# zgchen33/MCGaze

Measured on AMD Instinct MI355X. Metric: clips/sec (7x3x224x224), higher is better.
Workload: dtype f16x3; 1 GPU; full multiclue_gaze_r50 forward (R-50 + FPN + 4 decoder stages + gaze head), 64 clips/GPU x 7 frames x 3x224x224, 64 clips/step; clips_per_gpu=64, clip_length=7, global_clips=64, chunk_frames=0, parallelism=single GPU, trunk_streams=2

## Files before the change

### include/mcgaze_hip.h

```cpp
#ifndef MCGAZE_HIP_H
#define MCGAZE_HIP_H

#include <stddef.h>
#include <stdint.h>

#ifdef __cplusplus
extern "C" {
#endif

#define MCG_ABI_VERSION 14

enum { MCG_OK = 0, MCG_ERR_ARG = 1, MCG_ERR_HIP = 2, MCG_ERR_UNSUPPORTED = 3, MCG_ERR_WORKSPACE = 4 };
typedef enum { MCG_F32 = 0, MCG_BF16 = 1, MCG_F16X3 = 2, MCG_F16 = 3 } mcg_dtype;
#define MCG_ELEM_BYTES(dt) (((dt) == MCG_BF16 || (dt) == MCG_F16) ? 2 : 4)
typedef void* mcg_stream;

int mcg_abi_version(void);
const char* mcg_build_id(void);
const char* mcg_last_error(void);
int mcg_device_info(int* cu_count, size_t* hbm_bytes, char* arch, int arch_len);

int mcg_nchw_to_nhwc(mcg_stream s, mcg_dtype dt, const float* src, void* dst, int N, int C, int H, int W);
int mcg_nhwc_to_nchw(mcg_stream s, mcg_dtype dt, const void* src, float* dst, int N, int C, int H, int W);

enum { MCG_RES_NONE = 0, MCG_RES_ADD = 1, MCG_RES_UPSAMPLE_ADD = 2 };
enum {
  MCG_FLAG_STAGED_GEMM = 1,
  MCG_FLAG_NO_SPECIALISED = 2,
  MCG_FLAG_NO_ATTN_BLOCK = 4
};
typedef struct {
  const void* x;
  const void* w;
  const float* bias;
  const void* residual;
  void* y;
  int N, H, W, Cin, Cout, KH, KW, stride, pad;
  int relu;
  int residual_mode;
  int Hr, Wr;
  const void* x2;
  int Cin2, stride2, H2, W2;
  int tile;
  int flags;
  float wscale;
} mcg_conv_desc;
int mcg_conv2d(mcg_stream s, mcg_dtype dt, const mcg_conv_desc* d);

int mcg_bottleneck_x3(mcg_stream s, const float* x, const float* src2, const void* wstream, const float* bias, float* y, float* z,
                      int frames, int H, int W, int cm, int nsrc, int cn, void* trace);

size_t mcg_conv3x3_wino_x3_weight_bytes(int Cin, int Cout, int g);
int mcg_conv3x3_wino_x3(mcg_stream s, const float* x, const void* u, const float* bias, float* y, int frames, int H, int W,
                        int Cin, int Cout, int relu, int tile, float wscale, int g);

size_t mcg_stem_workspace_bytes(mcg_dtype dt, int N, int H, int W);
int mcg_stem_forward(mcg_stream s, mcg_dtype dt, const float* img, const void* w_stem, const float* bias,
                     void* y, int N, int H, int W, void* ws, size_t ws_bytes, int flags);

int mcg_roi_align(mcg_stream s, mcg_dtype dt, const void* const feats[4], const int feat_h[4], const int feat_w[4],
                  const int strides[4], int C, const float* boxes, int num_boxes, int boxes_per_frame,
                  void* out, int32_t* levels_out);
int mcg_roi_align_indexed(mcg_stream s, mcg_dtype dt, const void* const feats[4], const int feat_h[4], const int feat_w[4],
                          const int strides[4], int C, const float* boxes, int num_boxes, int boxes_per_frame,
                          const int32_t* frame_of, int pyramid_frames, void* out, int32_t* levels_out);

enum {
  MCG_SW_IN_PROJ_W = 0, MCG_SW_IN_PROJ_B, MCG_SW_OUT_PROJ_W, MCG_SW_OUT_PROJ_B, MCG_SW_ATTN_LN_G, MCG_SW_ATTN_LN_B,
  MCG_SW_DYN_W,
  MCG_SW_DYN_B,
  MCG_SW_NORM_IN_G, MCG_SW_NORM_IN_B, MCG_SW_NORM_OUT_G, MCG_SW_NORM_OUT_B,
  MCG_SW_FC_W, MCG_SW_FC_B, MCG_SW_FC_LN_G, MCG_SW_FC_LN_B, MCG_SW_IIC_LN_G, MCG_SW_IIC_LN_B,
  MCG_SW_FFN1_W, MCG_SW_FFN1_B, MCG_SW_FFN2_W, MCG_SW_FFN2_B, MCG_SW_FFN_LN_G, MCG_SW_FFN_LN_B,
  MCG_SW_CLS_FC_W, MCG_SW_CLS_LN_G, MCG_SW_CLS_LN_B,
  MCG_SW_REG_FC_W,
  MCG_SW_REG_LN_G,
  MCG_SW_REG_LN_B,
  MCG_SW_HEAD_CLS_W,
  MCG_SW_HEAD_CLS_B,
  MCG_SW_HEAD_REG_W,
  MCG_SW_HEAD_REG_B,
  MCG_SW_OUT_PROJ_WF, MCG_SW_CLS_FC_WF,
  MCG_SW_REG_FC_WF,
  MCG_SW_IN_PROJ_WF,
  MCG_SW_DYN_WF,
  MCG_SW_COUNT
};
enum {
  MCG_GW_FC_W = 0,
  MCG_GW_LN_G,
  MCG_GW_LN_B,
  MCG_GW_OUT_W,
  MCG_GW_OUT_B,
  MCG_GW_FUSE_W,
  MCG_GW_FUSE_B,
  MCG_GW_COUNT
};

size_t mcg_stage_workspace_bytes(mcg_dtype dt, int num_frames);
int mcg_stage_forward(mcg_stream s, mcg_dtype dt, const void* const weights[MCG_SW_COUNT], const void* roi_feat,
                      const void* obj_in, const float* boxes_in, int num_frames, int clip_length,
                      void* obj_out, float* boxes_out, float* cls_out, const float bbox_stds[4],
                      void* ws, size_t ws_bytes, int flags);

size_t mcg_gaze_head_workspace_bytes(mcg_dtype dt, int num_frames);
int mcg_gaze_head(mcg_stream s, mcg_dtype dt, const void* const weights[MCG_GW_COUNT], const void* obj,
                  int num_frames, float* gaze_out, void* ws, size_t ws_bytes);

typedef struct {
  const void* w;
  const float* bias;
  int cin, cout, k, stride, pad;
  const void* wf;
  float wscale;
  const void* wf4;
} mcg_conv_weights;

typedef struct {
  const void* wstream;
  const float* bias;
  int conv2_index;
  int cm, c, cn;
  int nsrc;
} mcg_fused_block;

typedef struct {
  int blocks[4];
  mcg_conv_weights stem;
  const mcg_conv_weights* convs;
  int num_convs;
  mcg_conv_weights lateral[4];
  mcg_conv_weights fpn_out[4];
  mcg_conv_weights c3_ds[4];
  const float* init_boxes;
  const void* init_feats;
  int num_stages;
  const void* const* stage_weights;
  const void* const* gaze_weights;
  float bbox_stds[4];
  const mcg_fused_block* fused;
  int num_fused;
} mcg_model_weights;

typedef struct mcg_engine mcg_engine;
int mcg_engine_create(mcg_engine** out, const mcg_model_weights* w, mcg_dtype dt);
void mcg_engine_destroy(mcg_engine* e);
int mcg_engine_set_option(mcg_engine* e, const char* name, int value);
int mcg_engine_range_audit(mcg_engine* e, unsigned long long* counts, const char** names, int capacity, int* n_out);
size_t mcg_engine_workspace_bytes(const mcg_engine* e, int num_frames, int H, int W, int chunk_frames);
int mcg_backbone_fpn_forward(mcg_engine* e, mcg_stream s, const float* img, int num_frames, int H, int W,
                             int chunk_frames, void* const pyramid[4], void* ws, size_t ws_bytes);
size_t mcg_trunk_workspace_bytes(const mcg_engine* e, int num_frames, int H, int W, int chunk_frames);
size_t mcg_decoder_workspace_bytes(const mcg_engine* e, int num_frames);
int mcg_decoder_forward(mcg_engine* e, mcg_stream s, const void* const pyramid[4], int num_frames, int clip_length, int H, int W,
                        const int* img_hw, float* gaze_out, float* boxes_out, float* scores_out, void* ws, size_t ws_bytes);
int mcg_decoder_forward_indexed(mcg_engine* e, mcg_stream s, const void* const pyramid[4], int pyramid_frames, const int32_t* frame_of,
                                int num_frames, int clip_length, int H, int W, const int* img_hw, float* gaze_out, float* boxes_out,
                                float* scores_out, void* ws, size_t ws_bytes);
int mcg_clip_forward(mcg_engine* e, mcg_stream s, const float* img, int num_frames, int clip_length, int H, int W,
                     const int* img_hw, int chunk_frames, float* gaze_out, float* boxes_out, float* scores_out,
                     void* ws, size_t ws_bytes);

typedef struct mcg_frame_desc {
  const void* src;
  int src_h, src_w, src_pitch;
  int crop_y, crop_x, crop_h, crop_w;
  int out_h, out_w;
} mcg_frame_desc;
int mcg_preprocess_frames(mcg_stream stream, const mcg_frame_desc* frames_dev, int num_frames, float* dst, int pad_h, int pad_w,
                          const float mean[3], const float stdinv[3], int to_rgb);

int mcg_engine_profile_start(mcg_engine* e, int capacity);
int mcg_engine_profile_stop(mcg_engine* e, int* count, float* ms, double* flops, double* algo_bytes, int* cfg, int* shape_mnk, int capacity);
int mcg_bench_backbone_forward(mcg_engine* e, mcg_stream s, const float* img, int num_frames, int H, int W, void* ws, size_t ws_bytes);
int mcg_bench_backbone_levels(const mcg_engine* e, void* ws, int num_frames, int H, int W, void* levels[4]);

#ifdef __cplusplus
}
#endif
#endif
```

### mcgaze_amd/csrc/check_resources.py

```python
#!/usr/bin/env python3
import re
import sys

RULES = {
    'wino_x3w_kernel': dict(scratch=0, vgpr_spill=0, unit='engine'),
}


def parse(path):
    kernels, cur = [], None
    for line in open(path, errors='replace'):
        m = re.search(r'remark: (?:\s*)Function Name: (\S+)', line)
        if m:
            cur = dict(name=m.group(1))
            kernels.append(cur)
            continue
        m = re.search(r'remark:\s+([A-Za-z \[\]/]+): (\S+) \[-Rpass-analysis', line)
        if m and cur is not None:
            cur[m.group(1).strip()] = m.group(2)
    return kernels


def main():
    path = sys.argv[1]
    kernels = parse(path)
    other = [l.rstrip() for l in open(path, errors='replace') if 'Rpass-analysis=kernel-resource-usage' not in l and not re.match(r'\s+\d* *\|', l) and l.strip()
             and not l.startswith('In file included from') and not re.match(r'\d+ (warning|remark)s? generated', l.strip())]
    for l in other:
        print(l, file=sys.stderr)
    bad = []
    import os
    unit = os.path.basename(path).split('.')[0]
    for prefix, lim in RULES.items():
        if lim.get('unit') == unit and not any(prefix in k['name'] and 'VGPRs Spill' in k and 'ScratchSize [bytes/lane]' in k for k in kernels):
            bad.append(f'{prefix}: no resource remarks found in {path} (expected -Rpass-analysis=kernel-resource-usage output for it)')
    for k in kernels:
        for prefix, lim in RULES.items():
            if prefix in k['name']:
                scratch = int(k.get('ScratchSize [bytes/lane]', '0'))
                spill = int(k.get('VGPRs Spill', '0'))
                if scratch > lim['scratch'] or spill > lim['vgpr_spill']:
                    bad.append(f"{k['name']}: scratch {scratch} B/lane, {spill} spilled VGPRs (limits {lim['scratch']}, {lim['vgpr_spill']})")
    if '--table' in sys.argv:
        print('| kernel | VGPRs | AGPRs | SGPRs | scratch B/lane | VGPR spill | waves/SIMD |\n|---|---|---|---|---|---|---|')
        for k in kernels:
            print(f"| `{k['name']}` | {k.get('VGPRs')} | {k.get('AGPRs')} | {k.get('TotalSGPRs')} | {k.get('ScratchSize [bytes/lane]')} | {k.get('VGPRs Spill')} | {k.get('Occupancy [waves/SIMD]')} |")
    if bad:
        print('check_resources: kernels with hand-issued loads must not spill:\n  ' + '\n  '.join(bad), file=sys.stderr)
        return 1
    return 0


if __name__ == '__main__':
    sys.exit(main())
```

### mcgaze_amd/csrc/engine.hip

```cpp
#include "igemm.hpp"
#include "pw_pair.hpp"
#include "pw_single.hpp"
#include "bneck_x3.hpp"
#include "pw_single_x3.hpp"
#include "wino_x3.hpp"

#include <stdlib.h>
#include <string.h>

#include <map>
#include <mutex>
#include <string>
#include <vector>

int launch_roi_align(hipStream_t s, mcg_dtype dt, const void* const feats[4], const int feat_h[4], const int feat_w[4],
                     const int strides[4], int C, const float* boxes, int num_boxes, int boxes_per_frame, const int32_t* frame_of,
                     int pyramid_frames, void* out, int32_t* levels_out);
int launch_init_queries(hipStream_t s, mcg_dtype dt, const float* init_boxes, const void* init_feats, const int* img_hw,
                        const int32_t* frame_of, int pyramid_frames, int H, int W, float* boxes, void* obj, int N);

struct mcg_engine {
  mcg_dtype dt;
  int blocks[4];
  mcg_conv_weights stem;
  std::vector<mcg_conv_weights> convs;
  mcg_conv_weights lateral[4], fpn_out[4], c3_ds[4];
  std::vector<mcg_fused_block> fused;
  bool bneck_fused = true;
  bool bneck_blocked = true;
  int winograd = 1;
  int wino_tile = -1;
  static constexpr int kAuditCap = 256;
  unsigned long long* audit_dev = nullptr;
  std::vector<std::string> audit_names;
  const float* init_boxes;
  const void* init_feats;
  int num_stages;
  std::vector<const void*> stage_w;
  const void* gaze_w[MCG_GW_COUNT];
  float stds[4];
  static constexpr int kMaxSplit = 4, kCandidates = 8;
  struct StreamPool* pool = nullptr;
  hipStream_t* cand = nullptr;
  hipEvent_t ev_fork = nullptr, ev_join[kMaxSplit - 1] = {};
  McgCtx ctx;
  Prof prof;
  int trunk_streams = 2;
  int max_range_frames = 0;
  bool pw_single = true;
  bool pw_pair = true;
  std::mutex mu;
};
struct StreamPool {
  hipStream_t cand[mcg_engine::kCandidates] = {};
  hipEvent_t ev_probe[3] = {};
  std::map<hipStream_t, std::vector<int>> side_of;
  std::mutex mu;
  bool ok = false;
};
static StreamPool* stream_pool_for_current_device() {
  static std::mutex g_mu;
  static std::map<int, StreamPool*> g_pools;
  int dev = 0;
  if (hipGetDevice(&dev) != hipSuccess) return nullptr;
  std::lock_guard<std::mutex> lock(g_mu);
  auto it = g_pools.find(dev);
  if (it != g_pools.end()) return it->second;
  StreamPool* p = new StreamPool();
  bool ok = true;
  for (int i = 0; i < mcg_engine::kCandidates; ++i) ok = ok && hipStreamCreateWithFlags(&p->cand[i], hipStreamNonBlocking) == hipSuccess;
  for (int i = 0; i < 3; ++i) ok = ok && hipEventCreate(&p->ev_probe[i]) == hipSuccess;
  p->ok = ok;
  g_pools[dev] = p;
  return p;
}
__global__ void probe_spin_kernel(long long ticks) {
  const long long t0 = wall_clock64();
  while (wall_clock64() - t0 < ticks) {}
}
static const std::vector<int>& side_streams_for(mcg_engine* e, hipStream_t s) {
  StreamPool* p = e->pool;
  std::lock_guard<std::mutex> lock(p->mu);
  auto it = p->side_of.find(s);
  if (it != p->side_of.end()) return it->second;
  std::vector<int> good, rest;
  const long long ticks = 15000;
  for (int c = 0; c < mcg_engine::kCandidates; ++c) {
    bool concurrent = false;
    if (hipEventRecord(p->ev_probe[0], s) == hipSuccess) {
      hipLaunchKernelGGL(probe_spin_kernel, dim3(1), dim3(64), 0, s, ticks);
      hipLaunchKernelGGL(probe_spin_kernel, dim3(1), dim3(64), 0, p->cand[c], ticks);
      float ms = 0.f;
      if (hipEventRecord(p->ev_probe[1], s) == hipSuccess && hipEventRecord(p->ev_probe[2], p->cand[c]) == hipSuccess &&
          hipEventSynchronize(p->ev_probe[1]) == hipSuccess && hipEventSynchronize(p->ev_probe[2]) == hipSuccess &&
          hipEventElapsedTime(&ms, p->ev_probe[0], p->ev_probe[2]) == hipSuccess)
        concurrent = ms < 0.15f * 1.6f;
    }
    (concurrent ? good : rest).push_back(c);
  }
  (void)hipGetLastError();
  good.insert(good.end(), rest.begin(), rest.end());
  return p->side_of.emplace(s, good).first->second;
}
static int range_frame_cap(const mcg_engine* e, int H, int W) {
  const long long per_frame = (long long)(H / 4) * (W / 4) * 256 * (mcg_is16(e->dt) ? 2 : 4);
  long long cap = 0x7FFFFF00ll / (per_frame > 0 ? per_frame : 1);
  if (e->max_range_frames > 0 && e->max_range_frames < cap) cap = e->max_range_frames;
  return cap < 1 ? 1 : (cap > 0x7fffffff ? 0x7fffffff : (int)cap);
}
static const int kMinFramesPerRange = 56;
static int trunk_ranges(const mcg_engine* e, int frames) {
  int k = e->trunk_streams;
  if (k > mcg_engine::kMaxSplit) k = mcg_engine::kMaxSplit;
  while (k > 1 && frames / k < kMinFramesPerRange) --k;
  return k < 1 ? 1 : k;
}

static inline size_t al256(size_t b) { return (b + 255) / 256 * 256; }
static inline size_t esize(mcg_dtype dt) { return mcg_is16(dt) ? 2 : 4; }

extern "C" void mcg_engine_destroy(mcg_engine* e);
extern "C" int mcg_engine_create(mcg_engine** out, const mcg_model_weights* w, mcg_dtype dt) {
  MCG_CHECK_ARG(out && w, "mcg_engine_create: null pointer");
  MCG_CHECK_ARG(dt == MCG_F32 || dt == MCG_BF16 || dt == MCG_F16X3 || dt == MCG_F16, "mcg_engine_create: unknown dtype %d", (int)dt);
  int expect = 0;
  for (int l = 0; l < 4; ++l) {
    MCG_CHECK_ARG(w->blocks[l] > 0, "mcg_engine_create: blocks[%d]=%d", l, w->blocks[l]);
    expect += 3 * w->blocks[l] + 1;
  }
  MCG_CHECK_ARG(w->num_convs == expect && w->convs, "mcg_engine_create: expected %d bottleneck convs, got %d", expect, w->num_convs);
  MCG_CHECK_ARG(w->num_stages > 0 && w->stage_weights && w->gaze_weights && w->init_boxes && w->init_feats, "mcg_engine_create: decoder tables missing");
  for (int i = 0; i < w->num_convs; ++i)
    MCG_CHECK_ARG(w->convs[i].w && w->convs[i].bias, "mcg_engine_create: conv %d has a null pointer", i);
  mcg_engine* e = new mcg_engine();
  e->dt = dt;
  memcpy(e->blocks, w->blocks, sizeof(e->blocks));
  e->stem = w->stem;
  e->convs.assign(w->convs, w->convs + w->num_convs);
  memcpy(e->lateral, w->lateral, sizeof(e->lateral));
  memcpy(e->fpn_out, w->fpn_out, sizeof(e->fpn_out));
  memcpy(e->c3_ds, w->c3_ds, sizeof(e->c3_ds));
  if (w->fused && w->num_fused > 0 && dt == MCG_F16X3) e->fused.assign(w->fused, w->fused + w->num_fused);
  e->init_boxes = w->init_boxes;
  e->init_feats = w->init_feats;
  e->num_stages = w->num_stages;
  e->stage_w.assign(w->stage_weights, w->stage_weights + (size_t)w->num_stages * MCG_SW_COUNT);
  memcpy(e->gaze_w, w->gaze_weights, sizeof(e->gaze_w));
  memcpy(e->stds, w->bbox_stds, sizeof(e->stds));
  bool ok = hipEventCreateWithFlags(&e->ev_fork, hipEventDisableTiming) == hipSuccess;
  e->pool = stream_pool_for_current_device();
  ok = ok && e->pool && e->pool->ok;
  if (e->pool) e->cand = e->pool->cand;
  for (int i = 0; i < mcg_engine::kMaxSplit - 1; ++i) ok = ok && hipEventCreateWithFlags(&e->ev_join[i], hipEventDisableTiming) == hipSuccess;
  if (!ok) {
    mcg_engine_destroy(e);
    mcg_set_error("mcg_engine_create: could not create the side streams / events");
    return MCG_ERR_HIP;
  }
  *out = e;
  return MCG_OK;
}

extern "C" int mcg_engine_set_option(mcg_engine* e, const char* name, int value) {
  MCG_CHECK_ARG(e && name, "mcg_engine_set_option: null pointer");
  std::lock_guard<std::mutex> lock(e->mu);
  if (!strcmp(name, "trunk_streams")) { MCG_CHECK_ARG(value >= 1 && value <= mcg_engine::kMaxSplit, "trunk_streams must be 1..%d", mcg_engine::kMaxSplit); e->trunk_streams = value; }
  else if (!strcmp(name, "max_range_frames")) { MCG_CHECK_ARG(value >= 0, "max_range_frames must be >= 0"); e->max_range_frames = value; }
  else if (!strcmp(name, "tile")) e->ctx.tile = value > 0 ? value : -1;
  else if (!strcmp(name, "staged_gemm")) e->ctx.staged = value != 0;
  else if (!strcmp(name, "conv3x3_c64")) e->ctx.c64 = value != 0;
  else if (!strcmp(name, "stem_fused")) e->ctx.stem_fused = value != 0;
  else if (!strcmp(name, "decoder_chain")) e->ctx.chain = value != 0;
  else if (!strcmp(name, "decoder_attn_block")) e->ctx.attn_block = value != 0;
  else if (!strcmp(name, "pointwise_pair")) e->pw_pair = value != 0;
  else if (!strcmp(name, "pointwise_stream")) e->pw_single = value != 0;
  else if (!strcmp(name, "bottleneck_fused")) e->bneck_fused = value != 0;
  else if (!strcmp(name, "bottleneck_blocked")) e->bneck_blocked = value != 0;
  else if (!strcmp(name, "winograd")) { MCG_CHECK_ARG(value >= 0 && value <= 2, "winograd must be 0, 1 or 2"); e->winograd = value; }
  else if (!strcmp(name, "wino_tile")) { MCG_CHECK_ARG(value >= -1 && value <= 3, "wino_tile must be -1 (by grid size) .. 3"); e->wino_tile = value; }
  else if (!strcmp(name, "range_audit")) {
    MCG_CHECK_ARG(!mcg_is16(e->dt) || !value, "range_audit: f32-storage engines only (MCG_F32, MCG_F16X3)");
    if (value && !e->audit_dev) {
      if (hipMalloc((void**)&e->audit_dev, sizeof(unsigned long long) * 2 * mcg_engine::kAuditCap) != hipSuccess) { e->audit_dev = nullptr; mcg_set_error("range_audit: hipMalloc failed"); return MCG_ERR_HIP; }
    }
    if (value && hipMemset(e->audit_dev, 0, sizeof(unsigned long long) * 2 * mcg_engine::kAuditCap) != hipSuccess) { mcg_set_error("range_audit: hipMemset failed"); return MCG_ERR_HIP; }
    if (!value && e->audit_dev) { (void)hipFree(e->audit_dev); e->audit_dev = nullptr; }
    e->audit_names.clear();
  }
  else { mcg_set_error("mcg_engine_set_option: unknown option '%s'", name); return MCG_ERR_ARG; }
  return MCG_OK;
}

extern "C" int mcg_engine_profile_start(mcg_engine* e, int capacity) {
  MCG_CHECK_ARG(e, "mcg_engine_profile_start: null engine");
  std::lock_guard<std::mutex> lock(e->mu);
  if (e->prof.recs) { mcg_set_error("mcg_engine_profile_start: already armed"); return MCG_ERR_ARG; }
  MCG_CHECK_ARG(capacity > 0 && capacity <= (1 << 20), "mcg_engine_profile_start: bad capacity %d", capacity);
  e->prof.recs = new ProfRec[capacity];
  for (int i = 0; i < capacity; ++i) { e->prof.recs[i].a = nullptr; e->prof.recs[i].b = nullptr; }
  for (int i = 0; i < capacity; ++i) {
    if (hipEventCreate(&e->prof.recs[i].a) != hipSuccess || hipEventCreate(&e->prof.recs[i].b) != hipSuccess) {
      for (int j = 0; j <= i; ++j) {
        if (e->prof.recs[j].a) (void)hipEventDestroy(e->prof.recs[j].a);
        if (e->prof.recs[j].b) (void)hipEventDestroy(e->prof.recs[j].b);
      }
      delete[] e->prof.recs;
      e->prof = Prof();
      mcg_set_error("mcg_engine_profile_start: hipEventCreate failed");
      return MCG_ERR_HIP;
    }
  }
  e->prof.cap = capacity; e->prof.n = 0;
  e->ctx.prof = &e->prof;
  return MCG_OK;
}
extern "C" int mcg_engine_profile_stop(mcg_engine* e, int* count, float* ms, double* flops, double* bytes, int* cfg, int* shape, int capacity) {
  MCG_CHECK_ARG(e, "mcg_engine_profile_stop: null engine");
  std::lock_guard<std::mutex> lock(e->mu);
  if (!e->prof.recs) { mcg_set_error("mcg_engine_profile_stop: not armed"); return MCG_ERR_ARG; }
  const int n = e->prof.n;
  int rc = MCG_OK;
  for (int i = 0; i < n; ++i) {
    const ProfRec& r = e->prof.recs[i];
    float t = 0.f;
    if (hipEventSynchronize(r.b) != hipSuccess || hipEventElapsedTime(&t, r.a, r.b) != hipSuccess) rc = MCG_ERR_HIP;
    if (i < capacity) {
      if (ms) ms[i] = t;
      if (flops) flops[i] = r.flops;
      if (bytes) bytes[i] = r.bytes;
      if (cfg) cfg[i] = r.cfg;
      if (shape) { shape[3 * i] = r.shape[0]; shape[3 * i + 1] = r.shape[1]; shape[3 * i + 2] = r.shape[2]; }
    }
  }
  for (int i = 0; i < e->prof.cap; ++i) { (void)hipEventDestroy(e->prof.recs[i].a); (void)hipEventDestroy(e->prof.recs[i].b); }
  delete[] e->prof.recs;
  e->prof = Prof();
  e->ctx.prof = nullptr;
  if (count) *count = n < capacity ? n : capacity;
  if (rc != MCG_OK) mcg_set_error("mcg_engine_profile_stop: event query failed");
  return rc;
}
extern "C" void mcg_engine_destroy(mcg_engine* e) {
  if (!e) return;
  if (e->ev_fork) (void)hipEventDestroy(e->ev_fork);
  for (int i = 0; i < mcg_engine::kMaxSplit - 1; ++i)
    if (e->ev_join[i]) (void)hipEventDestroy(e->ev_join[i]);
  if (e->prof.recs) {
    for (int i = 0; i < e->prof.cap; ++i) { (void)hipEventDestroy(e->prof.recs[i].a); (void)hipEventDestroy(e->prof.recs[i].b); }
    delete[] e->prof.recs;
  }
  if (e->audit_dev) (void)hipFree(e->audit_dev);
  delete e;
}

__global__ void range_audit_kernel(const float* __restrict__ x, long long n, unsigned long long* __restrict__ cnt) {
  unsigned long long big = 0, bad = 0;
  for (long long i = (long long)blockIdx.x * blockDim.x + threadIdx.x; i < n; i += (long long)gridDim.x * blockDim.x) {
    const float v = x[i];
    if (!(fabsf(v) <= 3.4028235e38f)) ++bad;
    else if (fabsf(v) > 65504.f) ++big;
  }
  big = (unsigned long long)wave_sum((float)big) ;
  bad = (unsigned long long)wave_sum((float)bad);
  if ((threadIdx.x & 63) == 0) {
    if (big) atomicAdd(cnt, big);
    if (bad) atomicAdd(cnt + 1, bad);
  }
}
struct AuditCursor { mcg_engine* e; hipStream_t s; int idx; bool naming; };
static void audit_tensor(AuditCursor& a, const char* name, const void* p, long long elements) {
  if (!a.e->audit_dev || a.idx >= mcg_engine::kAuditCap) return;
  if (a.naming) a.e->audit_names.push_back(name);
  const long long per_thread = 16;
  long long blocks = (elements + 256 * per_thread - 1) / (256 * per_thread);
  if (blocks > 4096) blocks = 4096;
  if (blocks < 1) blocks = 1;
  hipLaunchKernelGGL(range_audit_kernel, dim3((int)blocks), dim3(256), 0, a.s, (const float*)p, elements, a.e->audit_dev + 2 * a.idx);
  ++a.idx;
}

struct TrunkWs {
  char *stem_ws, *x0, *xa, *xb, *o1, *o2, *ds, *c[4], *l[4];
  size_t stem_bytes, total;
};
static TrunkWs trunk_layout(mcg_dtype dt, int n, int H, int W, char* base) {
  const size_t es = esize(dt);
  const size_t h2 = H / 4, w2 = W / 4;
  TrunkWs t;
  size_t off = 0;
  auto take = [&](size_t bytes) { char* p = base ? base + off : nullptr; off += al256(bytes); return p; };
  t.stem_bytes = mcg_stem_workspace_bytes(dt, n, H, W);
  t.stem_ws = take(t.stem_bytes);
  const size_t big = (size_t)n * h2 * w2 * 256 * es;
  t.x0 = take((size_t)n * h2 * w2 * 64 * es);
  t.xa = take(big); t.xb = take(big);
  t.o1 = take(big / 2); t.o2 = take(big / 2);
  t.ds = take(big);
  for (int i = 0; i < 4; ++i) {
    const size_t hi = (H / 4) >> i, wi = (W / 4) >> i;
    t.c[i] = take((size_t)n * hi * wi * (256u << i) * es);
    t.l[i] = take((size_t)n * hi * wi * 256 * es);
  }
  t.total = off;
  return t;
}

static int conv_call(const mcg_engine* e, hipStream_t s, mcg_dtype dt, const mcg_conv_weights& cw, const void* x, int n, int h, int w, void* y,
                     int relu, const void* res, int res_mode, int hr, int wr) {
  mcg_conv_desc d;
  memset(&d, 0, sizeof(d));
  d.x = x; d.w = cw.w; d.bias = cw.bias; d.residual = res; d.y = y;
  d.N = n; d.H = h; d.W = w; d.Cin = cw.cin; d.Cout = cw.cout; d.KH = cw.k; d.KW = cw.k; d.stride = cw.stride; d.pad = cw.pad;
  d.relu = relu; d.residual_mode = res_mode; d.Hr = hr; d.Wr = wr;
  d.wscale = dt == MCG_F16X3 ? cw.wscale : 0.f;
  const long long M = (long long)n * h * w;
  const int rm = res ? res_mode : MCG_RES_NONE;
  if (mcg_is16(dt) && e->pw_single && e->ctx.tile < 0 && !e->ctx.staged && cw.wf && cw.bias && cw.k == 1 && cw.stride == 1 && cw.pad == 0 &&
      pw_single_applicable(cw.cin, cw.cout, rm, M, rm == MCG_RES_UPSAMPLE_ADD ? (long long)n * hr * wr : M) && M < 0x7fffffffll) {
    PwSingleParams pp;
    memset(&pp, 0, sizeof(pp));
    pp.a = x; pp.res = res; pp.wf = cw.wf; pp.bias = cw.bias; pp.y = y;
    pp.M = (int)M; pp.relu = relu; pp.Ho = h; pp.Wo = w;
    if (rm == MCG_RES_UPSAMPLE_ADD) { pp.Hr = hr; pp.Wr = wr; pp.rscale_h = (float)hr / (float)h; pp.rscale_w = (float)wr / (float)w; }
    const double res_rows = rm == MCG_RES_NONE ? 0.0 : (rm == MCG_RES_ADD ? (double)M : (double)n * hr * wr);
    ProfRec* rec = prof_begin(e->ctx, s, 61, pp.M, cw.cout, cw.cin, 2.0 * M * cw.cin * cw.cout,
                              2.0 * ((double)M * (cw.cin + cw.cout) + res_rows * cw.cout + (double)cw.cin * cw.cout));
    const int prc = launch_pw_single(s, pp, cw.cin, cw.cout, rm == MCG_RES_NONE ? 0 : (rm == MCG_RES_ADD ? 1 : 2), dt == MCG_F16);
    prof_end(rec, s);
    if (prc) { mcg_set_error("pw_single launch failed"); return MCG_ERR_HIP; }
    return MCG_OK;
  }
  if (dt == MCG_F16X3 && e->pw_single && e->ctx.tile < 0 && cw.wf && cw.bias && cw.k == 1 && cw.stride == 1 && cw.pad == 0 &&
      pw_single_x3_applicable(cw.cin, cw.cout, rm, M, rm == MCG_RES_UPSAMPLE_ADD ? (long long)n * hr * wr : M) && M < 0x7fffffffll) {
    PwSingleParams pp;
    memset(&pp, 0, sizeof(pp));
    pp.a = x; pp.res = res; pp.wf = cw.wf; pp.bias = cw.bias; pp.y = y;
    pp.M = (int)M; pp.relu = relu; pp.Ho = h; pp.Wo = w; pp.wscale = cw.wscale;
    if (rm == MCG_RES_UPSAMPLE_ADD) { pp.Hr = hr; pp.Wr = wr; pp.rscale_h = (float)hr / (float)h; pp.rscale_w = (float)wr / (float)w; }
    const double res_rows = rm == MCG_RES_NONE ? 0.0 : (rm == MCG_RES_ADD ? (double)M : (double)n * hr * wr);
    ProfRec* rec = prof_begin(e->ctx, s, 71, pp.M, cw.cout, cw.cin, 2.0 * M * cw.cin * cw.cout,
                              4.0 * ((double)M * (cw.cin + cw.cout) + res_rows * cw.cout + (double)cw.cin * cw.cout));
    const int prc = launch_pw_single_x3(s, pp, cw.cout, rm == MCG_RES_NONE ? 0 : (rm == MCG_RES_ADD ? 1 : 2));
    prof_end(rec, s);
    if (prc) { mcg_set_error("pw_single_x3 launch failed"); return MCG_ERR_HIP; }
    return MCG_OK;
  }
  const int wg = (dt == MCG_F16X3 && e->winograd && e->ctx.tile < 0 && cw.k == 3 && cw.stride == 1 && cw.pad == 1 && rm == MCG_RES_NONE)
                     ? ((cw.wf4 && e->winograd >= 2 && wino_x3_applicable(n, h, w, cw.cin, cw.cout, 4)) ? 4 : ((cw.wf && wino_x3_applicable(n, h, w, cw.cin, cw.cout, 2)) ? 2 : 0))
                     : 0;
  if (wg) {
    WinoParams wp;
    memset(&wp, 0, sizeof(wp));
    wp.x = (const float*)x; wp.u = wg == 4 ? cw.wf4 : cw.wf; wp.bias = cw.bias; wp.y = (float*)y;
    wp.H = h; wp.W = w; wp.frames = n; wp.Cin = cw.cin; wp.Cout = cw.cout; wp.relu = relu; wp.wscale = cw.wscale;
    ProfRec* rec = prof_begin(e->ctx, s, 73, (int)M, cw.cout, 9 * cw.cin, 2.0 * M * 9.0 * cw.cin * cw.cout,
                              4.0 * ((double)M * (cw.cin + cw.cout) + 9.0 * cw.cin * cw.cout));
    const int wrc = launch_wino_x3(s, wp, e->wino_tile, wg);
    prof_end(rec, s);
    if (wrc) { mcg_set_error("wino_x3 launch failed"); return MCG_ERR_HIP; }
    return MCG_OK;
  }
  return conv2d_ctx(s, dt, &d, e->ctx);
}

static int trunk_chunk(mcg_engine* e, hipStream_t s, const float* img, int f0, int n, int H, int W, void* const pyr[4], char* wsbase,
                       bool backbone_only = false) {
  const mcg_dtype dt = e->dt;
  const size_t es = esize(dt);
  TrunkWs t = trunk_layout(dt, n, H, W, wsbase);
  MCG_TRY(stem_forward_ctx(s, dt, img + (size_t)f0 * 3 * H * W, e->stem.w, e->stem.bias, t.x0, n, H, W, t.stem_ws, t.stem_bytes, e->ctx));
  AuditCursor au{e, s, 0, e->audit_dev != nullptr && e->audit_names.empty()};
  char aname[64];
  audit_tensor(au, "stem", t.x0, (long long)n * (H / 4) * (W / 4) * 64);
  const void* x = t.x0;
  int h = H / 4, w = W / 4, ci = 0;
  bool x_blocked = false;
  bool o1_ready = false;
  char *o1 = t.o1, *o2 = t.o2;
  for (int l = 0; l < 4; ++l) {
    for (int b = 0; b < e->blocks[l]; ++b) {
      const mcg_conv_weights& c1 = e->convs[ci], &c2 = e->convs[ci + 1], &c3 = e->convs[ci + 2];
      const bool has_ds = b == 0;
      const int ho = (h + 2 * c2.pad - c2.k) / c2.stride + 1, wo = (w + 2 * c2.pad - c2.k) / c2.stride + 1;
      void* y = (b == e->blocks[l] - 1) ? (void*)t.c[l] : (x == t.xa ? (void*)t.xb : (void*)t.xa);
      if (!o1_ready) {
        MCG_TRY(conv_call(e, s, dt, c1, x, n, h, w, o1, 1, nullptr, MCG_RES_NONE, 0, 0));
        snprintf(aname, sizeof(aname), "layer%d.%d.conv1", l + 1, b);
        audit_tensor(au, aname, o1, (long long)n * h * w * c1.cout);
      }
      o1_ready = false;
      auto fused_at = [&](int cj, int bj) -> const mcg_fused_block* {
        if (!(dt == MCG_F16X3 && e->bneck_fused && e->ctx.tile < 0) || cj + 2 >= (int)e->convs.size()) return nullptr;
        const mcg_fused_block* f = nullptr;
        for (const mcg_fused_block& q : e->fused)
          if (q.conv2_index == cj + 1) f = &q;
        if (!f) return nullptr;
        const bool ds = bj == 0;
        const mcg_conv_weights &d2 = e->convs[cj + 1], &d3 = e->convs[cj + 2];
        const int kk = ds ? e->convs[cj + 3].cin : 0, ss = ds ? e->convs[cj + 3].stride : 1;
        const int cn_i = cj + (ds ? 4 : 3);
        const bool nx = f->cn == 0 || (cn_i < (int)e->convs.size() && e->convs[cn_i].k == 1 && e->convs[cn_i].stride == 1 && e->convs[cn_i].cout == f->cn && e->convs[cn_i].cin == f->c);
        return (d2.k == 3 && d2.stride == 1 && d2.pad == 1 && d2.cin == f->cm && d2.cout == f->cm && d3.cout == f->c && f->nsrc == (ds ? 2 : 1) && nx &&
                bneck_x3_applicable(f->cm, f->c, f->cn, f->nsrc, kk, ss)) ? f : nullptr;
      };
      const mcg_fused_block* fb = fused_at(ci, b);
      if (x_blocked && !(fb && fb->nsrc == 1)) { mcg_set_error("trunk: a blocked tensor reached a kernel that does not read that layout"); return MCG_ERR_UNSUPPORTED; }
      if (fb) {
        const int k2 = has_ds ? e->convs[ci + 3].cin : 0;
        const int ci_nx = ci + (has_ds ? 4 : 3);
        {
          BneckParams bp;
          memset(&bp, 0, sizeof(bp));
          bp.x = (const float*)o1; bp.res = (const float*)x; bp.wstream = (const char*)fb->wstream; bp.bias = fb->bias;
          bp.y = (float*)y; bp.z = (float*)o2; bp.H = h; bp.W = w;
          const long long blk_bytes = (long long)n * ((h + bnx::TH - 1) / bnx::TH) * ((w + bnx::TW - 1) / bnx::TW) * bnx::NPIX * fb->c * (long long)es;
          const mcg_fused_block* fnext = (b + 1 < e->blocks[l]) ? fused_at(ci_nx, b + 1) : nullptr;
          bp.res_blocked = x_blocked ? 1 : 0;
          bp.y_blocked = (e->bneck_blocked && !e->audit_dev && y != (void*)t.c[l] && fb->cn > 0 && fnext && fnext->nsrc == 1 && fnext->c == fb->c &&
                          blk_bytes <= (long long)((size_t)n * (H / 4) * (W / 4) * 256 * es)) ? 1 : 0;
          const double M = (double)n * h * w;
          ProfRec* rec = prof_begin(e->ctx, s, 70, n * h * w, fb->c + fb->cn, 9 * fb->cm + fb->cm + k2 + fb->c,
                                    2.0 * M * (9.0 * fb->cm * fb->cm + (double)(fb->cm + k2) * fb->c + (double)fb->c * fb->cn),
                                    4.0 * (M * (fb->cm + (has_ds ? k2 : fb->c) + fb->c + fb->cn) + 9.0 * fb->cm * fb->cm + (double)(fb->cm + k2) * fb->c + (double)fb->c * fb->cn));
          const int frc = launch_bneck_x3(s, bp, n, fb->cm, fb->nsrc, fb->cn);
          prof_end(rec, s);
          if (frc) { mcg_set_error("bneck_x3 launch failed"); return MCG_ERR_HIP; }
          snprintf(aname, sizeof(aname), "layer%d.%d.out (fused tail)", l + 1, b);
          audit_tensor(au, aname, y, (long long)n * h * w * fb->c);
          if (fb->cn > 0) {
            snprintf(aname, sizeof(aname), "layer%d.%d.next_conv1 (fused tail)", l + 1, b);
            audit_tensor(au, aname, o2, (long long)n * h * w * fb->cn);
          }
          if (fb->cn > 0) { char* tmp = o1; o1 = o2; o2 = tmp; o1_ready = true; }
          x = y; h = ho; w = wo;
          x_blocked = bp.y_blocked != 0;
          ci = ci_nx;
          continue;
        }
      }
      MCG_TRY(conv_call(e, s, dt, c2, o1, n, h, w, o2, 1, nullptr, MCG_RES_NONE, 0, 0));
      snprintf(aname, sizeof(aname), "layer%d.%d.conv2", l + 1, b);
      audit_tensor(au, aname, o2, (long long)n * ho * wo * c2.cout);
      const int ci_next = ci + (has_ds ? 4 : 3);
      const mcg_conv_weights* c3w = has_ds ? (e->c3_ds[l].w ? &e->c3_ds[l] : nullptr) : &c3;
      const mcg_conv_weights* c1n = ci_next < (int)e->convs.size() ? &e->convs[ci_next] : nullptr;
      const int k2 = has_ds ? e->convs[ci + 3].cin : 0;
      if (mcg_is16(dt) && e->pw_pair && l == 0 && c3w && c1n && c3w->wf && c1n->wf && c3w->bias && c1n->bias && c1n->k == 1 && c1n->stride == 1 &&
          c1n->cin == c3.cout && pw_pair_applicable(c3.cin, k2, has_ds ? e->convs[ci + 3].stride : 1, c3.cout, c1n->cout, (long long)n * ho * wo) && (long long)n * ho * wo < 0x7fffffffll) {
        PwPairParams pp;
        memset(&pp, 0, sizeof(pp));
        pp.a1 = o2; pp.K1 = c3.cin;
        if (has_ds) { pp.a2 = x; pp.K2 = k2; pp.stride2 = e->convs[ci + 3].stride; pp.H2 = h; pp.W2 = w; }
        else pp.res = x;
        pp.w3f = c3w->wf; pp.b3 = c3w->bias; pp.y = y;
        pp.w1f = c1n->wf; pp.b1 = c1n->bias; pp.z = o1;
        pp.M = n * ho * wo; pp.C = c3.cout; pp.C2 = c1n->cout; pp.Ho = ho; pp.Wo = wo;
        ProfRec* rec = prof_begin(e->ctx, s, 60, pp.M, pp.C + pp.C2, pp.K1 + pp.K2, 2.0 * pp.M * ((double)(pp.K1 + pp.K2) * pp.C + (double)pp.C * pp.C2),
                                  2.0 * ((double)pp.M * (pp.K1 + pp.K2 + (has_ds ? 0 : pp.C) + pp.C + pp.C2) + (double)(pp.K1 + pp.K2) * pp.C + (double)pp.C * pp.C2));
        const int prc = launch_pw_pair(s, pp, dt == MCG_F16);
        prof_end(rec, s);
        if (prc) { mcg_set_error("pw_pair launch failed"); return MCG_ERR_HIP; }
        o1_ready = true;
        x = y; h = ho; w = wo;
        ci = ci_next;
        continue;
      }
      if (has_ds && e->c3_ds[l].w) {
        const mcg_conv_weights& f = e->c3_ds[l];
        mcg_conv_desc d;
        memset(&d, 0, sizeof(d));
        d.x = o2; d.w = f.w; d.bias = f.bias; d.y = y;
        d.wscale = dt == MCG_F16X3 ? f.wscale : 0.f;
        d.N = n; d.H = ho; d.W = wo; d.Cin = c3.cin; d.Cout = c3.cout; d.KH = 1; d.KW = 1; d.stride = 1; d.pad = 0; d.relu = 1;
        d.x2 = x; d.Cin2 = e->convs[ci + 3].cin; d.stride2 = e->convs[ci + 3].stride; d.H2 = h; d.W2 = w;
        MCG_TRY(conv2d_ctx(s, dt, &d, e->ctx));
      } else {
        const void* identity = x;
        if (has_ds) {
          MCG_TRY(conv_call(e, s, dt, e->convs[ci + 3], x, n, h, w, t.ds, 0, nullptr, MCG_RES_NONE, 0, 0));
          identity = t.ds;
        }
        MCG_TRY(conv_call(e, s, dt, c3, o2, n, ho, wo, y, 1, identity, MCG_RES_ADD, 0, 0));
      }
      snprintf(aname, sizeof(aname), "layer%d.%d.out", l + 1, b);
      audit_tensor(au, aname, y, (long long)n * ho * wo * c3.cout);
      x = y; h = ho; w = wo;
      ci += has_ds ? 4 : 3;
    }
  }
  if (backbone_only) return MCG_OK;
  int hs[4], wsz[4];
  for (int i = 0; i < 4; ++i) { hs[i] = (H / 4) >> i; wsz[i] = (W / 4) >> i; }
  for (int i = 3; i >= 0; --i) {
    const void* res = i == 3 ? nullptr : t.l[i + 1];
    MCG_TRY(conv_call(e, s, dt, e->lateral[i], t.c[i], n, hs[i], wsz[i], t.l[i], 0, res, res ? MCG_RES_UPSAMPLE_ADD : MCG_RES_NONE,
                      i == 3 ? 0 : hs[i + 1], i == 3 ? 0 : wsz[i + 1]));
    snprintf(aname, sizeof(aname), "fpn.lateral%d (+ top-down)", i);
    audit_tensor(au, aname, t.l[i], (long long)n * hs[i] * wsz[i] * 256);
  }
  for (int i = 0; i < 4; ++i) {
    char* dst = (char*)pyr[i] + (size_t)f0 * hs[i] * wsz[i] * 256 * es;
    MCG_TRY(conv_call(e, s, dt, e->fpn_out[i], t.l[i], n, hs[i], wsz[i], dst, 0, nullptr, MCG_RES_NONE, 0, 0));
    snprintf(aname, sizeof(aname), "fpn.P%d", i + 2);
    audit_tensor(au, aname, dst, (long long)n * hs[i] * wsz[i] * 256);
  }
  return MCG_OK;
}

extern "C" int mcg_engine_range_audit(mcg_engine* e, unsigned long long* counts, const char** names, int capacity, int* n_out) {
  MCG_CHECK_ARG(e && counts && n_out && capacity > 0, "mcg_engine_range_audit: bad argument");
  std::lock_guard<std::mutex> lock(e->mu);
  if (!e->audit_dev) { mcg_set_error("mcg_engine_range_audit: the range_audit option is off"); return MCG_ERR_ARG; }
  const int n = (int)e->audit_names.size() < capacity ? (int)e->audit_names.size() : capacity;
  if (hipDeviceSynchronize() != hipSuccess ||
      hipMemcpy(counts, e->audit_dev, sizeof(unsigned long long) * 2 * n, hipMemcpyDeviceToHost) != hipSuccess ||
      hipMemset(e->audit_dev, 0, sizeof(unsigned long long) * 2 * mcg_engine::kAuditCap) != hipSuccess) {
    mcg_set_error("mcg_engine_range_audit: device read failed");
    return MCG_ERR_HIP;
  }
  if (names) for (int i = 0; i < n; ++i) names[i] = e->audit_names[i].c_str();
  *n_out = n;
  return MCG_OK;
}

struct DecWs {
  char *roi, *obj_a, *obj_b, *stage_ws, *gaze_ws;
  float *boxes_a, *boxes_b, *cls;
  size_t stage_bytes, gaze_bytes, total;
};
static DecWs dec_layout(mcg_dtype dt, int N, char* base) {
  const size_t es = esize(dt), R = (size_t)N * 3;
  DecWs c;
  memset(&c, 0, sizeof(c));
  size_t off = 0;
  auto take = [&](size_t bytes) { char* p = base ? base + off : nullptr; off += al256(bytes); return p; };
  c.roi = take(R * 49 * 256 * es);
  c.obj_a = take(R * 256 * es); c.obj_b = take(R * 256 * es);
  c.boxes_a = (float*)take(R * 4 * 4); c.boxes_b = (float*)take(R * 4 * 4); c.cls = (float*)take(R * 4);
  c.stage_bytes = mcg_stage_workspace_bytes(dt, N); c.stage_ws = take(c.stage_bytes);
  c.gaze_bytes = mcg_gaze_head_workspace_bytes(dt, N); c.gaze_ws = take(c.gaze_bytes);
  c.total = off;
  return c;
}
static size_t pyramid_bytes(mcg_dtype dt, int N, int H, int W, int level) {
  return al256((size_t)N * ((H / 4) >> level) * ((W / 4) >> level) * 256 * esize(dt));
}

extern "C" size_t mcg_trunk_workspace_bytes(const mcg_engine* e, int N, int H, int W, int chunk) {
  if (!e || N <= 0) return 0;
  if (chunk <= 0 || chunk > N) chunk = N;
  if (chunk < N) return trunk_layout(e->dt, chunk, H, W, nullptr).total;
  size_t total = 0;
  const int cap = range_frame_cap(e, H, W);
  for (int k = 1; k <= mcg_engine::kMaxSplit; ++k) {
    const int per = (N + k - 1) / k < cap ? (N + k - 1) / k : cap;
    const size_t t = (size_t)k * al256(trunk_layout(e->dt, per, H, W, nullptr).total);
    if (t > total) total = t;
  }
  return total;
}
extern "C" size_t mcg_decoder_workspace_bytes(const mcg_engine* e, int N) {
  if (!e || N <= 0) return 0;
  return dec_layout(e->dt, N, nullptr).total;
}
extern "C" size_t mcg_engine_workspace_bytes(const mcg_engine* e, int N, int H, int W, int chunk) {
  if (!e || N <= 0) return 0;
  size_t total = mcg_trunk_workspace_bytes(e, N, H, W, chunk) + mcg_decoder_workspace_bytes(e, N);
  for (int i = 0; i < 4; ++i) total += pyramid_bytes(e->dt, N, H, W, i);
  return total;
}

static int check_shape(int N, int H, int W) {
  MCG_CHECK_ARG(N > 0, "num_frames must be positive (got %d)", N);
  MCG_CHECK_ARG(H >= 32 && W >= 32 && H % 32 == 0 && W % 32 == 0, "frame size %dx%d must be a multiple of 32 (Pad(size_divisor=32))", H, W);
  return MCG_OK;
}

static int trunk_forward(mcg_engine* e, mcg_stream s_, const float* img, int N, int H, int W, int chunk,
                         void* const pyramid[4], void* ws, size_t ws_bytes, bool backbone_only) {
  MCG_CHECK_ARG(e && img && (pyramid || backbone_only) && ws, "mcg_backbone_fpn_forward: null pointer");
  MCG_TRY(check_shape(N, H, W));
  std::lock_guard<std::mutex> lock(e->mu);
  if (chunk <= 0 || chunk > N) chunk = N;
  const size_t need = mcg_trunk_workspace_bytes(e, N, H, W, chunk);
  if (ws_bytes < need) { mcg_set_error("mcg_backbone_fpn_forward: workspace too small (%zu < %zu)", ws_bytes, need); return MCG_ERR_WORKSPACE; }
  hipStream_t s = (hipStream_t)s_;
  if (chunk < N) {
    for (int f0 = 0; f0 < N; f0 += chunk) MCG_TRY(trunk_chunk(e, s, img, f0, (N - f0) < chunk ? (N - f0) : chunk, H, W, pyramid, (char*)ws, backbone_only));
    return MCG_OK;
  }
  const int k = trunk_ranges(e, N);
  const int cap = range_frame_cap(e, H, W);
  const int per = (N + k - 1) / k < cap ? (N + k - 1) / k : cap;
  if (k == 1) {
    for (int f0 = 0; f0 < N; f0 += per) MCG_TRY(trunk_chunk(e, s, img, f0, (N - f0) < per ? (N - f0) : per, H, W, pyramid, (char*)ws, backbone_only));
    return MCG_OK;
  }
  const std::vector<int>& sides = side_streams_for(e, s);
  const size_t part_ws = al256(trunk_layout(e->dt, per, H, W, nullptr).total);
  if (hipEventRecord(e->ev_fork, s) != hipSuccess) { mcg_set_error("mcg_backbone_fpn_forward: hipEventRecord failed"); return MCG_ERR_HIP; }
  int rc = MCG_OK;
  for (int i = 1; i < k; ++i)
    if (hipStreamWaitEvent(e->cand[sides[i - 1]], e->ev_fork, 0) != hipSuccess) { mcg_set_error("mcg_backbone_fpn_forward: hipStreamWaitEvent failed"); return MCG_ERR_HIP; }
  for (int f0 = 0, i = 0; f0 < N && rc == MCG_OK; f0 += per, i = (i + 1) % k) {
    hipStream_t si = i == 0 ? s : e->cand[sides[i - 1]];
    rc = trunk_chunk(e, si, img, f0, (N - f0) < per ? (N - f0) : per, H, W, pyramid, (char*)ws + (size_t)i * part_ws, backbone_only);
  }
  for (int i = 1; i < k; ++i) {
    hipStream_t si = e->cand[sides[i - 1]];
    if (hipEventRecord(e->ev_join[i - 1], si) != hipSuccess || hipStreamWaitEvent(s, e->ev_join[i - 1], 0) != hipSuccess) {
      mcg_set_error("mcg_backbone_fpn_forward: join failed");
      rc = rc == MCG_OK ? MCG_ERR_HIP : rc;
    }
  }
  return rc;
}

extern "C" int mcg_bottleneck_x3(mcg_stream s, const float* x, const float* src2, const void* wstream, const float* bias, float* y, float* z,
                                 int frames, int H, int W, int cm, int nsrc, int cn, void* trace) {
  MCG_CHECK_ARG(x && src2 && wstream && bias && y && (z || cn == 0), "mcg_bottleneck_x3: null pointer");
  MCG_CHECK_ARG(frames > 0 && H > 0 && W > 0, "mcg_bottleneck_x3: empty problem");
  MCG_CHECK_ARG(bneck_x3_applicable(cm, 4 * cm, cn, nsrc, 64, 1), "mcg_bottleneck_x3: unsupported shape (cm=%d nsrc=%d cn=%d)", cm, nsrc, cn);
  BneckParams bp;
  memset(&bp, 0, sizeof(bp));
  bp.x = x; bp.res = src2; bp.wstream = (const char*)wstream; bp.bias = bias; bp.y = y; bp.z = z; bp.H = H; bp.W = W; bp.trace = (unsigned long long*)trace;
  if (launch_bneck_x3((hipStream_t)s, bp, frames, cm, nsrc, cn)) { mcg_set_error("mcg_bottleneck_x3: launch failed"); return MCG_ERR_HIP; }
  return MCG_OK;
}

extern "C" size_t mcg_conv3x3_wino_x3_weight_bytes(int Cin, int Cout, int g) {
  return (Cin > 0 && Cout > 0 && Cin % 32 == 0 && Cout % wnx::UNT == 0 && (g == 2 || g == 4)) ? wino_x3_weight_bytes(Cin, Cout, g) : 0;
}
extern "C" int mcg_conv3x3_wino_x3(mcg_stream s, const float* x, const void* u, const float* bias, float* y, int frames, int H, int W,
                                   int Cin, int Cout, int relu, int tile, float wscale, int g) {
  MCG_CHECK_ARG(x && u && y, "mcg_conv3x3_wino_x3: null pointer");
  MCG_CHECK_ARG(tile >= 0 && tile <= 4, "mcg_conv3x3_wino_x3: tile must be 0 (by grid size) .. 4");
  if (!wino_x3_applicable(frames, H, W, Cin, Cout, g)) {
    mcg_set_error("mcg_conv3x3_wino_x3: unsupported shape (frames=%d %dx%d, %d -> %d channels, F(%d,3)): Cin %% 32, Cout %% 128, W <= 62 (F(4,3): W %% 4 == 0, W >= 16), a tile's window within its buffer", frames, H, W, Cin, Cout, g);
    return MCG_ERR_UNSUPPORTED;
  }
  WinoParams wp;
  memset(&wp, 0, sizeof(wp));
  wp.x = x; wp.u = u; wp.bias = bias; wp.y = y; wp.H = H; wp.W = W; wp.frames = frames; wp.Cin = Cin; wp.Cout = Cout; wp.relu = relu;
  wp.wscale = wscale;
  if (launch_wino_x3((hipStream_t)s, wp, tile - 1, g)) { mcg_set_error("mcg_conv3x3_wino_x3: launch failed"); return MCG_ERR_HIP; }
  return MCG_OK;
}

extern "C" int mcg_backbone_fpn_forward(mcg_engine* e, mcg_stream s, const float* img, int N, int H, int W, int chunk,
                                        void* const pyramid[4], void* ws, size_t ws_bytes) {
  return trunk_forward(e, s, img, N, H, W, chunk, pyramid, ws, ws_bytes, false);
}
extern "C" int mcg_bench_backbone_forward(mcg_engine* e, mcg_stream s, const float* img, int N, int H, int W, void* ws, size_t ws_bytes) {
  return trunk_forward(e, s, img, N, H, W, 0, nullptr, ws, ws_bytes, true);
}

extern "C" int mcg_bench_backbone_levels(const mcg_engine* e, void* ws, int N, int H, int W, void* levels[4]) {
  MCG_CHECK_ARG(e && ws && levels, "mcg_bench_backbone_levels: null pointer");
  MCG_TRY(check_shape(N, H, W));
  MCG_CHECK_ARG(trunk_ranges(e, N) == 1 && N <= range_frame_cap(e, H, W), "mcg_bench_backbone_levels: the batch runs as several frame ranges (set trunk_streams = 1)");
  const TrunkWs t = trunk_layout(e->dt, N, H, W, (char*)ws);
  for (int i = 0; i < 4; ++i) levels[i] = t.c[i];
  return MCG_OK;
}

static int decoder_forward(mcg_engine* e, hipStream_t s, const void* const pyramid[4], int pyramid_frames, const int32_t* frame_of, int N,
                           int clip_length, int H, int W, const int* img_hw, float* gaze_out, float* boxes_out, float* scores_out, void* ws,
                           size_t ws_bytes) {
  MCG_CHECK_ARG(e && pyramid && gaze_out && boxes_out && scores_out && ws, "mcg_decoder_forward: null pointer");
  MCG_TRY(check_shape(N, H, W));
  MCG_CHECK_ARG(clip_length > 0 && N % clip_length == 0, "num_frames=%d is not a multiple of clip_length=%d", N, clip_length);
  DecWs c = dec_layout(e->dt, N, (char*)ws);
  if (ws_bytes < c.total) { mcg_set_error("mcg_decoder_forward: workspace too small (%zu < %zu)", ws_bytes, c.total); return MCG_ERR_WORKSPACE; }
  MCG_TRY(launch_init_queries(s, e->dt, e->init_boxes, e->init_feats, img_hw, frame_of, pyramid_frames, H, W, c.boxes_a, c.obj_a, N));
  int fh[4], fw[4];
  const int strides[4] = {4, 8, 16, 32};
  for (int i = 0; i < 4; ++i) { fh[i] = (H / 4) >> i; fw[i] = (W / 4) >> i; }
  char* obj_in = c.obj_a; char* obj_out = c.obj_b;
  float* b_in = c.boxes_a; float* b_out = c.boxes_b;
  for (int st = 0; st < e->num_stages; ++st) {
    MCG_TRY(launch_roi_align(s, e->dt, pyramid, fh, fw, strides, 256, b_in, N * 3, 3, frame_of, pyramid_frames, c.roi, nullptr));
    float* bdst = (st == e->num_stages - 1) ? boxes_out : b_out;
    MCG_TRY(stage_forward_ctx(s, e->dt, &e->stage_w[(size_t)st * MCG_SW_COUNT], c.roi, obj_in, b_in, N, clip_length, obj_out, bdst,
                              c.cls, e->stds, c.stage_ws, c.stage_bytes, e->ctx));
    char* t = obj_in; obj_in = obj_out; obj_out = t;
    if (st != e->num_stages - 1) { float* tb = b_in; b_in = b_out; b_out = tb; }
  }
  MCG_TRY(gaze_head_ctx(s, e->dt, e->gaze_w, obj_in, N, gaze_out, c.gaze_ws, c.gaze_bytes, e->ctx, c.cls, scores_out));
  return MCG_OK;
}

extern "C" int mcg_decoder_forward(mcg_engine* e, mcg_stream s_, const void* const pyramid[4], int N, int clip_length, int H, int W,
                                   const int* img_hw, float* gaze_out, float* boxes_out, float* scores_out, void* ws, size_t ws_bytes) {
  return decoder_forward(e, (hipStream_t)s_, pyramid, N, nullptr, N, clip_length, H, W, img_hw, gaze_out, boxes_out, scores_out, ws, ws_bytes);
}

extern "C" int mcg_decoder_forward_indexed(mcg_engine* e, mcg_stream s_, const void* const pyramid[4], int pyramid_frames, const int32_t* frame_of,
                                           int N, int clip_length, int H, int W, const int* img_hw, float* gaze_out, float* boxes_out,
                                           float* scores_out, void* ws, size_t ws_bytes) {
  MCG_CHECK_ARG(frame_of, "mcg_decoder_forward_indexed: null frame_of (mcg_decoder_forward is the plain path)");
  MCG_CHECK_ARG(pyramid_frames > 0, "mcg_decoder_forward_indexed: empty pyramid store (pyramid_frames=%d)", pyramid_frames);
  return decoder_forward(e, (hipStream_t)s_, pyramid, pyramid_frames, frame_of, N, clip_length, H, W, img_hw, gaze_out, boxes_out, scores_out,
                         ws, ws_bytes);
}

extern "C" int mcg_clip_forward(mcg_engine* e, mcg_stream s_, const float* img, int N, int clip_length, int H, int W,
                                const int* img_hw, int chunk, float* gaze_out, float* boxes_out, float* scores_out,
                                void* ws, size_t ws_bytes) {
  MCG_CHECK_ARG(e && img && gaze_out && boxes_out && scores_out && ws, "mcg_clip_forward: null pointer");
  MCG_TRY(check_shape(N, H, W));
  MCG_CHECK_ARG(clip_length > 0 && N % clip_length == 0, "mcg_clip_forward: num_frames=%d is not a multiple of clip_length=%d", N, clip_length);
  const size_t need = mcg_engine_workspace_bytes(e, N, H, W, chunk);
  if (ws_bytes < need) { mcg_set_error("mcg_clip_forward: workspace too small (%zu < %zu)", ws_bytes, need); return MCG_ERR_WORKSPACE; }
  char* base = (char*)ws;
  const size_t trunk_bytes = mcg_trunk_workspace_bytes(e, N, H, W, chunk);
  void* pyr[4];
  size_t off = trunk_bytes;
  for (int i = 0; i < 4; ++i) { pyr[i] = base + off; off += pyramid_bytes(e->dt, N, H, W, i); }
  MCG_TRY(mcg_backbone_fpn_forward(e, s_, img, N, H, W, chunk, pyr, base, trunk_bytes));
  return mcg_decoder_forward(e, s_, pyr, N, clip_length, H, W, img_hw, gaze_out, boxes_out, scores_out, base + off, ws_bytes - off);
}
```

### mcgaze_amd/csrc/roi_align.hip

```cpp
#include "common.hpp"

struct RoiLevels {
  const void* feat[4];
  int h[4], w[4];
  float scale[4];
};

template <typename T>
__global__ __launch_bounds__(256) void roi_align_kernel(RoiLevels lv, int C, const float* __restrict__ boxes, int boxes_per_frame,
                                                        const int32_t* __restrict__ frame_of, int pyramid_frames,
                                                        T* __restrict__ out, int32_t* __restrict__ levels_out, float finest_scale) {
  constexpr int EPC = Elem<T>::kPerChunk;
  constexpr int P = 7, S = 2, NS = P * S;
  __shared__ int s_lo[2][NS], s_hi[2][NS];
  __shared__ float s_l[2][NS], s_h[2][NS];
  __shared__ int s_valid[2][NS];
  const int box = blockIdx.x, tid = threadIdx.x;
  const float x1 = boxes[box * 4 + 0], y1 = boxes[box * 4 + 1], x2 = boxes[box * 4 + 2], y2 = boxes[box * 4 + 3];
  const float sc = sqrtf((x2 - x1) * (y2 - y1));
  int level = (int)fminf(fmaxf(floorf(log2f(sc / finest_scale + 1e-6f)), 0.f), 3.f);
  if (!(sc == sc)) level = 0;
  const int H = lv.h[level], W = lv.w[level];
  const float ss = lv.scale[level];
  if (tid < 2 * NS) {
    const int axis = tid / NS, i = tid % NS;
    const float start = (axis == 0 ? y1 : x1) * ss - 0.5f, end = (axis == 0 ? y2 : x2) * ss - 0.5f;
    const float bin = (end - start) / (float)P;
    const int L = axis == 0 ? H : W;
    float c = start + (float)(i / S) * bin + ((float)(i % S) + 0.5f) * bin / (float)S;
    const int valid = !(c < -1.0f || c > (float)L);
    c = fmaxf(c, 0.f);
    int lo = (int)c, hi;
    if (lo >= L - 1) {
      lo = hi = L - 1;
      c = (float)lo;
    } else {
      hi = lo + 1;
    }
    const float l = c - (float)lo;
    s_lo[axis][i] = lo; s_hi[axis][i] = hi; s_l[axis][i] = l; s_h[axis][i] = 1.f - l; s_valid[axis][i] = valid && (c == c);
  }
  if (tid == 0) {
    if (levels_out) levels_out[box] = level;
  }
  __syncthreads();
  int frame = box / boxes_per_frame;
  bool bad_row = false;
  if (frame_of) {
    frame = __builtin_amdgcn_readfirstlane(frame_of[frame]);
    bad_row = frame < 0 || frame >= pyramid_frames;
    if (bad_row) frame = 0;
  }
  const T* __restrict__ F = (const T*)lv.feat[level] + (long long)frame * H * W * C;
  const int groups = C / EPC, bins_per_pass = 256 / groups;
  const int cg = tid % groups, slot = tid / groups;
  if (bad_row) {
    float nan[EPC];
#pragma unroll
    for (int e = 0; e < EPC; ++e) nan[e] = __builtin_nanf("");
    for (int bin = slot; bin < P * P; bin += bins_per_pass)
      *(uint4*)(out + ((long long)box * (P * P) + bin) * C + cg * EPC) = f32_to_chunk(nan, (T*)nullptr);
    return;
  }
  for (int bin = slot; bin < P * P; bin += bins_per_pass) {
    const int ph = bin / P, pw = bin % P;
    float acc[EPC];
#pragma unroll
    for (int e = 0; e < EPC; ++e) acc[e] = 0.f;
#pragma unroll
    for (int iy = 0; iy < S; ++iy) {
      const int yi = ph * S + iy;
#pragma unroll
      for (int ix = 0; ix < S; ++ix) {
        const int xi = pw * S + ix;
        if (!(s_valid[0][yi] && s_valid[1][xi])) continue;
        const int yl = s_lo[0][yi], yh = s_hi[0][yi], xl = s_lo[1][xi], xh = s_hi[1][xi];
        const float ly = s_l[0][yi], hy = s_h[0][yi], lx = s_l[1][xi], hx = s_h[1][xi];
        const float w1 = hy * hx, w2 = hy * lx, w3 = ly * hx, w4 = ly * lx;
        float v1[EPC], v2[EPC], v3[EPC], v4[EPC];
        chunk_to_f32(*(const uint4*)(F + ((long long)yl * W + xl) * C + cg * EPC), v1, (T*)nullptr);
        chunk_to_f32(*(const uint4*)(F + ((long long)yl * W + xh) * C + cg * EPC), v2, (T*)nullptr);
        chunk_to_f32(*(const uint4*)(F + ((long long)yh * W + xl) * C + cg * EPC), v3, (T*)nullptr);
        chunk_to_f32(*(const uint4*)(F + ((long long)yh * W + xh) * C + cg * EPC), v4, (T*)nullptr);
#pragma unroll
        for (int e = 0; e < EPC; ++e) acc[e] += w1 * v1[e] + w2 * v2[e] + w3 * v3[e] + w4 * v4[e];
      }
    }
#pragma unroll
    for (int e = 0; e < EPC; ++e) acc[e] *= (1.0f / (float)(S * S));
    *(uint4*)(out + ((long long)box * (P * P) + bin) * C + cg * EPC) = f32_to_chunk(acc, (T*)nullptr);
  }
}

int launch_roi_align(hipStream_t s, mcg_dtype dt, const void* const feats[4], const int feat_h[4], const int feat_w[4],
                     const int strides[4], int C, const float* boxes, int num_boxes, int boxes_per_frame, const int32_t* frame_of,
                     int pyramid_frames, void* out, int32_t* levels_out) {
  RoiLevels lv;
  for (int i = 0; i < 4; ++i) {
    lv.feat[i] = feats[i]; lv.h[i] = feat_h[i]; lv.w[i] = feat_w[i];
    lv.scale[i] = 1.0f / (float)strides[i];
  }
  const int epc = mcg_is16(dt) ? 8 : 4;
  MCG_CHECK_ARG(C % epc == 0 && C / epc <= 256 && 256 % (C / epc) == 0, "roi_align: unsupported channel count %d", C);
  if (dt == MCG_BF16)
    hipLaunchKernelGGL(roi_align_kernel<bf16_t>, dim3(num_boxes), dim3(256), 0, s, lv, C, boxes, boxes_per_frame, frame_of, pyramid_frames,
                       (bf16_t*)out, levels_out, 56.f);
  else if (dt == MCG_F16)
    hipLaunchKernelGGL(roi_align_kernel<f16_t>, dim3(num_boxes), dim3(256), 0, s, lv, C, boxes, boxes_per_frame, frame_of, pyramid_frames,
                       (f16_t*)out, levels_out, 56.f);
  else
    hipLaunchKernelGGL(roi_align_kernel<float>, dim3(num_boxes), dim3(256), 0, s, lv, C, boxes, boxes_per_frame, frame_of, pyramid_frames,
                       (float*)out, levels_out, 56.f);
  MCG_CHECK_LAUNCH("roi_align");
  return MCG_OK;
}

extern "C" int mcg_roi_align(mcg_stream s, mcg_dtype dt, const void* const feats[4], const int feat_h[4], const int feat_w[4],
                             const int strides[4], int C, const float* boxes, int num_boxes, int boxes_per_frame,
                             void* out, int32_t* levels_out) {
  MCG_CHECK_ARG(feats && feat_h && feat_w && strides && boxes && out, "mcg_roi_align: null pointer");
  MCG_CHECK_ARG(num_boxes > 0 && boxes_per_frame > 0, "mcg_roi_align: empty box set");
  for (int i = 0; i < 4; ++i) MCG_CHECK_ARG(feats[i] && feat_h[i] > 0 && feat_w[i] > 0 && strides[i] > 0, "mcg_roi_align: bad level %d", i);
  return launch_roi_align((hipStream_t)s, dt, feats, feat_h, feat_w, strides, C, boxes, num_boxes, boxes_per_frame, nullptr, 0, out, levels_out);
}

extern "C" int mcg_roi_align_indexed(mcg_stream s, mcg_dtype dt, const void* const feats[4], const int feat_h[4], const int feat_w[4],
                                     const int strides[4], int C, const float* boxes, int num_boxes, int boxes_per_frame,
                                     const int32_t* frame_of, int pyramid_frames, void* out, int32_t* levels_out) {
  MCG_CHECK_ARG(feats && feat_h && feat_w && strides && boxes && out && frame_of, "mcg_roi_align_indexed: null pointer");
  MCG_CHECK_ARG(num_boxes > 0 && boxes_per_frame > 0 && pyramid_frames > 0, "mcg_roi_align_indexed: empty box set or pyramid");
  for (int i = 0; i < 4; ++i) MCG_CHECK_ARG(feats[i] && feat_h[i] > 0 && feat_w[i] > 0 && strides[i] > 0, "mcg_roi_align_indexed: bad level %d", i);
  return launch_roi_align((hipStream_t)s, dt, feats, feat_h, feat_w, strides, C, boxes, num_boxes, boxes_per_frame, frame_of, pyramid_frames,
                          out, levels_out);
}
```

### mcgaze_amd/csrc/wino_x3.hpp

```cpp
#pragma once
#include "igemm_dma.hpp"

namespace wnx {
constexpr int KS = 16;
constexpr int UNT = 128;
constexpr int ustage(int g) { return (g + 2) * 4 * 2 * 1024; }
constexpr int wcap(int g, int ct) { return (g == 4 && ct == 4) ? 32 * 1024 : 48 * 1024; }
}

struct WinoParams {
  const float* x;
  const void* u;
  const float* bias;
  float* y;
  int H, W, PW, frames, Cin, Cout, relu;
  int total_pairs, n_tiles;
  int tpf, gpf;
  float wscale;
};

template <int NB, int RH, int RT, int CT, int G>
__global__ __launch_bounds__(64 * (G + 2) * RH, 1) void wino_x3_kernel(const WinoParams p) {
  using namespace wnx;
  constexpr int NV = G + 2, NW = NV * RH, NTHREADS = 64 * NW, MT = 32 * RH * RT, NT = 32 * CT;
  constexpr int ROWB = NB * 1024, WIN_CAP = wcap(G, CT), USTAGE = ustage(G);
  constexpr int BSTAGE = NV * CT * 2 * 1024;
  constexpr int BPW = 2 * NV * CT / NW;
  constexpr int MAXP = (WIN_CAP / 1024 + NW - 1) / NW;
  constexpr int NTERM = G == 2 ? 2 : 4;
  static_assert((2 * NV * CT) % NW == 0 && UNT % NT == 0 && (G == 2 || G == 4), "tile shape");
  extern __shared__ __attribute__((aligned(16))) char smem[];
  char* const s_win = smem;
  char* const s_b = smem + 2 * WIN_CAP;
  const int tid = threadIdx.x, lane = tid & 63;
  const int wave = __builtin_amdgcn_readfirstlane(tid >> 6);
  const int nu = wave % NV, rh = wave / NV;
  const int logical = xcd_remap(blockIdx.x, gridDim.x);
  const int mt = logical / p.n_tiles, ntile = logical - mt * p.n_tiles;
  int q0, q_end;
  if (p.tpf > 0) {
    const int f = mt / p.tpf, t = mt - f * p.tpf;
    q0 = f * p.gpf + t * MT;
    q_end = min(q0 + MT, (f + 1) * p.gpf);
  } else {
    q0 = mt * MT;
    q_end = min(q0 + MT, p.total_pairs);
  }
  const int q_last = q_end - 1;
  const int H1 = p.H + 1;
  auto slot_of = [&](int q) { const int R = q / p.PW; return R + R / p.H + 1; };
  const int sig_b = __builtin_amdgcn_readfirstlane(slot_of(q0) - 1);
  const int NP = __builtin_amdgcn_readfirstlane((slot_of(q_last) - sig_b + 2) * NB);
  const int NSL = p.Cin / KS, KT = 3 * NSL;

  const int n0 = ntile * NT;
  const u32x4 srd_x = make_srd(p.x);
  const u32x4 srd_u = make_srd((const char*)p.u + (size_t)(n0 / UNT) * KT * USTAGE + (size_t)((n0 % UNT) / 32) * 2048);
  const uint32_t lds_win = (uint32_t)(uintptr_t)(__attribute__((address_space(3))) char*)s_win;
  const uint32_t lds_b = (uint32_t)(uintptr_t)(__attribute__((address_space(3))) char*)s_b;

  uint32_t prow[MAXP];
  int pblk[MAXP];
  bool pok[MAXP], prowok[MAXP];
  static_for<MAXP>([&](auto nc) {
    constexpr int n = decltype(nc)::value;
    const int pi = wave + NW * n, j = pi / NB, b = pi - j * NB;
    const int sg = sig_b + j, f = sg / H1, r = sg - f * H1;
    pok[n] = pi < NP;
    prowok[n] = __builtin_amdgcn_readfirstlane((r != 0 && f < p.frames) ? 1 : 0) != 0;
    prow[n] = __builtin_amdgcn_readfirstlane((uint32_t)(((long long)(f * p.H + r - 1) * p.W) * p.Cin * 4));
    pblk[n] = b;
  });
  const int l_ph = lane >> 5, l_i = (lane >> 2) & 7, l_cs = lane & 3;
  auto win_voff = [&](int pc) -> uint32_t {
    const int b = pc / (G / 2), hph = pc - b * (G / 2);
    const int x = (8 * b + l_i) * G + 2 * hph + l_ph - 1;
    const int c = l_cs ^ ((2 * b + (l_i >> 2)) & 3);
    return (unsigned)x < (unsigned)p.W ? (uint32_t)((x * p.Cin + 4 * c) * 4) : MCG_OOB_OFFSET;
  };
  auto issue_window = [&](int cs, uint32_t dst) {
    static_for<MAXP>([&](auto nc) {
      constexpr int n = decltype(nc)::value;
      if (pok[n]) {
        const uint32_t v = prowok[n] ? win_voff(pblk[n]) : MCG_OOB_OFFSET;
        lds_dma16<0>(v, srd_x, prow[n] + (uint32_t)cs * (KS * 4), dst + (uint32_t)(wave + NW * n) * 1024u);
      }
    });
  };
  const uint32_t b_voff = (uint32_t)lane * 16u;
  auto issue_b = [&](int k, uint32_t dst) {
    static_for<BPW>([&](auto ic) {
      constexpr int i = decltype(ic)::value;
      const int pc = wave * BPW + i, pnu = pc / (2 * CT), rest = pc - pnu * (2 * CT);
      lds_dma16<i * 1024>(b_voff, srd_u, (uint32_t)k * USTAGE + (uint32_t)pnu * 8192u + (uint32_t)rest * 1024u, dst + (uint32_t)wave * (BPW * 1024u));
    });
  };

  int toff[NTERM];
  float tco[NTERM];
  if constexpr (G == 2) {
    toff[0] = nu == 0 ? 0 : 1; toff[1] = nu == 3 ? 3 : 2;
    tco[0] = 1.f; tco[1] = nu == 1 ? 1.f : -1.f;
  } else {
    const int o4[6][4] = {{0, 2, 4, 4}, {1, 2, 3, 4}, {1, 2, 3, 4}, {1, 2, 3, 4}, {1, 2, 3, 4}, {1, 3, 5, 5}};
    const float c4[6][4] = {{4.f, -5.f, 1.f, 0.f}, {-4.f, -4.f, 1.f, 1.f}, {4.f, -4.f, -1.f, 1.f}, {-2.f, -1.f, 2.f, 1.f}, {2.f, -1.f, -2.f, 1.f}, {4.f, -5.f, 1.f, 0.f}};
#pragma unroll
    for (int t = 0; t < 4; ++t) {
      toff[t] = o4[0][t]; tco[t] = c4[0][t];
#pragma unroll
      for (int v = 1; v < 6; ++v)
        if (nu == v) { toff[t] = o4[v][t]; tco[t] = c4[v][t]; }
    }
  }
  const int pl = lane & 31, h = lane >> 5;
  const char* ap[RT][NTERM][2];
#pragma unroll
  for (int rt = 0; rt < RT; ++rt) {
    const int q = min(q0 + (RT * rh + rt) * 32 + pl, q_last);
    const int R = q / p.PW, xg = q - R * p.PW;
    const int jrow = (R + R / p.H + 1) - sig_b - 1;
#pragma unroll
    for (int t = 0; t < NTERM; ++t) {
      const int wx = G * xg + toff[t];
      const int pp = wx / G, ph = wx - pp * G, swz = (pp >> 2) & 3;
      const int off = jrow * ROWB + (pp >> 3) * (G * 512) + ph * 512 + (pp & 7) * 64;
#pragma unroll
      for (int ch = 0; ch < 2; ++ch) ap[rt][t][ch] = s_win + off + (((2 * h + ch) ^ swz) << 4);
    }
  }
  const char* const bp = s_b + nu * (CT * 2 * 1024) + lane * 16;

  f32x16 acc[RT][CT];
#pragma unroll
  for (int i = 0; i < RT; ++i)
#pragma unroll
    for (int j = 0; j < CT; ++j)
#pragma unroll
      for (int r = 0; r < 16; ++r) acc[i][j][r] = 0.f;

  struct Raw { uint4 d[RT][NTERM][2]; };
  auto load_raw = [&](auto wbc, auto kyc, Raw& r) {
    constexpr int AOFF = decltype(wbc)::value * WIN_CAP + decltype(kyc)::value * ROWB;
#pragma unroll
    for (int rt = 0; rt < RT; ++rt)
#pragma unroll
      for (int t = 0; t < NTERM; ++t) { r.d[rt][t][0] = *(const uint4*)(ap[rt][t][0] + AOFF); r.d[rt][t][1] = *(const uint4*)(ap[rt][t][1] + AOFF); }
  };
  auto transform = [&](const Raw& r, bf16x8 (&ah)[RT], bf16x8 (&al)[RT]) {
#pragma unroll
    for (int rt = 0; rt < RT; ++rt) {
      float v[8];
#pragma unroll
      for (int c = 0; c < 2; ++c) {
        const uint32_t e0[4] = {r.d[rt][0][c].x, r.d[rt][0][c].y, r.d[rt][0][c].z, r.d[rt][0][c].w};
        const uint32_t e1[4] = {r.d[rt][1][c].x, r.d[rt][1][c].y, r.d[rt][1][c].z, r.d[rt][1][c].w};
        if constexpr (G == 2) {
#pragma unroll
          for (int e = 0; e < 4; ++e) v[4 * c + e] = fmaf(tco[1], __uint_as_float(e1[e]), __uint_as_float(e0[e]));
        } else {
          const uint32_t e2[4] = {r.d[rt][2][c].x, r.d[rt][2][c].y, r.d[rt][2][c].z, r.d[rt][2][c].w};
          const uint32_t e3[4] = {r.d[rt][3][c].x, r.d[rt][3][c].y, r.d[rt][3][c].z, r.d[rt][3][c].w};
#pragma unroll
          for (int e = 0; e < 4; ++e)
            v[4 * c + e] = fmaf(tco[3], __uint_as_float(e3[e]), fmaf(tco[2], __uint_as_float(e2[e]), fmaf(tco[1], __uint_as_float(e1[e]), tco[0] * __uint_as_float(e0[e]))));
        }
      }
      const uint4 v0 = make_uint4(__float_as_uint(v[0]), __float_as_uint(v[1]), __float_as_uint(v[2]), __float_as_uint(v[3]));
      const uint4 v1 = make_uint4(__float_as_uint(v[4]), __float_as_uint(v[5]), __float_as_uint(v[6]), __float_as_uint(v[7]));
      split_f32x8(v0, v1, ah[rt], al[rt]);
    }
  };

  issue_window(0, lds_win);
  issue_b(0, lds_b);
  bf16x8 fh[2][RT], fl[2][RT];
  asm volatile("s_waitcnt vmcnt(0)" ::: "memory");
  __builtin_amdgcn_s_barrier();
  {
    Raw r0;
    load_raw(std::integral_constant<int, 0>{}, std::integral_constant<int, 0>{}, r0);
    transform(r0, fh[0], fl[0]);
  }
  constexpr int NM1 = RT * CT;
  constexpr int PVALU = (G == 2 ? 32 : 56) * RT, VPM = (PVALU + 2 * NM1 - 1) / (2 * NM1);
#pragma nounroll
  for (int s2 = 0; s2 < NSL / 2; ++s2) {
    static_for<6>([&](auto uc) {
      constexpr int U = decltype(uc)::value, KY = U % 3, SL = U & 1, WB = U / 3;
      constexpr int U1 = (U + 1) % 6, KY1 = U1 % 3, WB1 = U1 / 3;
      constexpr int BOFF = SL * BSTAGE;
      const int k = 6 * s2 + U, cs = 2 * s2 + WB;
      asm volatile("s_waitcnt vmcnt(0) lgkmcnt(0)" ::: "memory");
      __builtin_amdgcn_s_barrier();
      bf16x8 bh[CT], bl[CT];
#pragma unroll
      for (int ct = 0; ct < CT; ++ct) {
        bh[ct] = __builtin_bit_cast(bf16x8, *(const uint4*)(bp + BOFF + ct * 2048));
        bl[ct] = __builtin_bit_cast(bf16x8, *(const uint4*)(bp + BOFF + ct * 2048 + 1024));
      }
      Raw raw;
      load_raw(std::integral_constant<int, WB1>{}, std::integral_constant<int, KY1>{}, raw);
      __builtin_amdgcn_sched_barrier(0);
      const uint32_t kn = (uint32_t)min(k + 1, KT - 1) * USTAGE, bdst = lds_b + (SL ^ 1) * BSTAGE + (uint32_t)wave * (BPW * 1024u);
      static_for<NM1>([&](auto mc) {
        constexpr int M = decltype(mc)::value, I = M / CT, J = M % CT;
        acc[I][J] = x3_mfma(fl[SL][I], bh[J], acc[I][J]);
        if constexpr (M < BPW) {
          const int pc = wave * BPW + M, pnu = pc / (2 * CT), rest = pc - pnu * (2 * CT);
          lds_dma16<M * 1024>(b_voff, srd_u, kn + (uint32_t)pnu * 8192u + (uint32_t)rest * 1024u, bdst);
        }
        __builtin_amdgcn_sched_barrier(0);
      });
      if constexpr (NM1 < BPW) {
        static_for<BPW - NM1>([&](auto mc) {
          constexpr int M = NM1 + decltype(mc)::value;
          const int pc = wave * BPW + M, pnu = pc / (2 * CT), rest = pc - pnu * (2 * CT);
          lds_dma16<M * 1024>(b_voff, srd_u, kn + (uint32_t)pnu * 8192u + (uint32_t)rest * 1024u, bdst);
        });
      }
      if (KY == 0 && cs + 1 < NSL) issue_window(cs + 1, lds_win + (WB ^ 1) * WIN_CAP);
      transform(raw, fh[SL ^ 1], fl[SL ^ 1]);
#pragma unroll
      for (int i2 = 0; i2 < RT; ++i2)
#pragma unroll
        for (int j2 = 0; j2 < CT; ++j2) acc[i2][j2] = x3_mfma(fh[SL][i2], bl[j2], acc[i2][j2]);
#pragma unroll
      for (int i2 = 0; i2 < RT; ++i2)
#pragma unroll
        for (int j2 = 0; j2 < CT; ++j2) acc[i2][j2] = x3_mfma(fh[SL][i2], bh[j2], acc[i2][j2]);
      static_for<2 * NM1 - 1>([&](auto) {
        __builtin_amdgcn_sched_group_barrier(0x008, 1, 0);
        __builtin_amdgcn_sched_group_barrier(0x002, VPM, 0);
      });
      __builtin_amdgcn_sched_group_barrier(0x008, 1, 0);
      __builtin_amdgcn_sched_group_barrier(0x002, 8, 0);
    });
  }
  asm volatile("s_waitcnt vmcnt(0) lgkmcnt(0)" ::: "memory");
  __syncthreads();

  constexpr int PP = 32 * RT, CPR = NT / 4;
  static_assert(NV * PP * NT * 4 <= 2 * WIN_CAP + 2 * BSTAGE, "epilogue staging");
  float* const C = (float*)smem;
  const float wsc = p.wscale > 0.f ? p.wscale : 1.f;
#pragma unroll 1
  for (int pass = 0; pass < RH; ++pass) {
    if (rh == pass) {
#pragma unroll
      for (int rt = 0; rt < RT; ++rt)
#pragma unroll
        for (int ct = 0; ct < CT; ++ct)
#pragma unroll
          for (int r = 0; r < 16; ++r)
            C[(nu * PP + rt * 32 + mfma32_row(r, lane)) * NT + ct * 32 + (lane & 31)] = acc[rt][ct][r];
    }
    __syncthreads();
    for (int item = tid; item < PP * CPR; item += NTHREADS) {
      const int prl = item / CPR, ch4 = (item - prl * CPR) * 4;
      const int q = q0 + pass * PP + prl;
      if (q >= q_end) continue;
      float4 bv = make_float4(0.f, 0.f, 0.f, 0.f);
      if (p.bias) bv = *(const float4*)(p.bias + n0 + ch4);
      float4 m[NV];
#pragma unroll
      for (int v = 0; v < NV; ++v) m[v] = *(const float4*)(C + (v * PP + prl) * NT + ch4);
      float4 y[G];
      if constexpr (G == 2) {
        y[0] = make_float4(((m[0].x + m[1].x) + m[2].x) * wsc + bv.x, ((m[0].y + m[1].y) + m[2].y) * wsc + bv.y, ((m[0].z + m[1].z) + m[2].z) * wsc + bv.z, ((m[0].w + m[1].w) + m[2].w) * wsc + bv.w);
        y[1] = make_float4(((m[1].x - m[2].x) - m[3].x) * wsc + bv.x, ((m[1].y - m[2].y) - m[3].y) * wsc + bv.y, ((m[1].z - m[2].z) - m[3].z) * wsc + bv.z, ((m[1].w - m[2].w) - m[3].w) * wsc + bv.w);
      } else {
#define MCG_W4(F)                                                                                                            \
        {                                                                                                                    \
          const float s12 = m[1].F + m[2].F, d12 = m[1].F - m[2].F, s34 = m[3].F + m[4].F, d34 = m[3].F - m[4].F;            \
          y[0].F = ((m[0].F + s12) + s34) * wsc + bv.F;                                                                      \
          y[1].F = fmaf(2.f, d34, d12) * wsc + bv.F;                                                                         \
          y[2].F = fmaf(4.f, s34, s12) * wsc + bv.F;                                                                         \
          y[3].F = (fmaf(8.f, d34, d12) + m[5].F) * wsc + bv.F;                                                              \
        }
        MCG_W4(x) MCG_W4(y) MCG_W4(z) MCG_W4(w)
#undef MCG_W4
      }
      const int R = q / p.PW, xo = G * (q - R * p.PW);
      float* yp = p.y + ((long long)R * p.W + xo) * p.Cout + n0 + ch4;
#pragma unroll
      for (int j = 0; j < G; ++j) {
        if (xo + j >= p.W) break;
        float4 o = y[j];
        if (p.relu) { o.x = fmaxf(o.x, 0.f); o.y = fmaxf(o.y, 0.f); o.z = fmaxf(o.z, 0.f); o.w = fmaxf(o.w, 0.f); }
        *(float4*)(yp + (long long)j * p.Cout) = o;
      }
    }
    __syncthreads();
  }
}

typedef uint32_t u32x4v __attribute__((ext_vector_type(4)));
template <int IMM>
__device__ __forceinline__ void buf_load16(u32x4v& dst, uint32_t voffset, const u32x4& srd, uint32_t soffset_uniform) {
  asm volatile("buffer_load_dwordx4 %0, %1, %2, %3 offen offset:%4" : "=&v"(dst) : "v"(voffset), "s"(srd), "s"(soffset_uniform), "n"(IMM) : "memory");
}
template <int NB>
__global__ __launch_bounds__(256, 1) void wino_x3w_kernel(const WinoParams p) {
  using namespace wnx;
  constexpr int G = 2, NV = 4, NW = 4, RT = 4, CT = 4, MT = 128, NT = 128;
  constexpr int ROWB = NB * 1024, WIN_CAP = 48 * 1024, USTAGE = ustage(2);
  constexpr int MAXP = WIN_CAP / 1024 / NW;
  constexpr int HB = MAXP / 2;
  extern __shared__ __attribute__((aligned(16))) char smem[];
  char* const s_win = smem;
  const int tid = threadIdx.x, lane = tid & 63;
  const int wave = __builtin_amdgcn_readfirstlane(tid >> 6);
  const int nu = wave;
  const int logical = xcd_remap(blockIdx.x, gridDim.x);
  const int mt = logical / p.n_tiles, ntile = logical - mt * p.n_tiles;
  int q0, q_end;
  if (p.tpf > 0) {
    const int f = mt / p.tpf, t = mt - f * p.tpf;
    q0 = f * p.gpf + t * MT;
    q_end = min(q0 + MT, (f + 1) * p.gpf);
  } else {
    q0 = mt * MT;
    q_end = min(q0 + MT, p.total_pairs);
  }
  const int q_last = q_end - 1;
  const int H1 = p.H + 1;
  auto slot_of = [&](int q) { const int R = q / p.PW; return R + R / p.H + 1; };
  const int sig_b = __builtin_amdgcn_readfirstlane(slot_of(q0) - 1);
  const int NP = __builtin_amdgcn_readfirstlane((slot_of(q_last) - sig_b + 2) * NB);
  const int NSL = p.Cin / KS, KT = 3 * NSL;
  const int n0 = ntile * NT;
  const u32x4 srd_x = make_srd(p.x);
  const u32x4 srd_u = make_srd((const char*)p.u + (size_t)(n0 / UNT) * KT * USTAGE);
  const uint32_t lds_win = (uint32_t)(uintptr_t)(__attribute__((address_space(3))) char*)s_win;

  uint32_t prow[MAXP];
  uint32_t pokm = 0, prowokm = 0;
  static_for<MAXP>([&](auto nc) {
    constexpr int n = decltype(nc)::value;
    const int pi = wave + NW * n, j = pi / NB;
    const int sg = sig_b + j, f = sg / H1, r = sg - f * H1;
    if (pi < NP) pokm |= 1u << n;
    if (r != 0 && f < p.frames) prowokm |= 1u << n;
    prow[n] = __builtin_amdgcn_readfirstlane((uint32_t)(((long long)(f * p.H + r - 1) * p.W) * p.Cin * 4));
  });
  pokm = __builtin_amdgcn_readfirstlane(pokm);
  prowokm = __builtin_amdgcn_readfirstlane(prowokm);
  uint32_t w_voff;
  {
    const int l_ph = lane >> 5, l_i = (lane >> 2) & 7, l_cs = lane & 3, b = wave & (NB - 1);
    const int x = (8 * b + l_i) * G + l_ph - 1;
    const int c = l_cs ^ ((2 * b + (l_i >> 2)) & 3);
    w_voff = (unsigned)x < (unsigned)p.W ? (uint32_t)((x * p.Cin + 4 * c) * 4) : MCG_OOB_OFFSET;
  }
  auto issue_window = [&](auto hc, int cs, uint32_t dst) {
    constexpr int h0 = decltype(hc)::value * HB;
    static_for<HB>([&](auto nc) {
      constexpr int n = h0 + decltype(nc)::value;
      if (pokm & (1u << n)) {
        const uint32_t v = (prowokm & (1u << n)) ? w_voff : MCG_OOB_OFFSET;
        lds_dma16<0>(v, srd_x, prow[n] + (uint32_t)cs * (KS * 4), dst + (uint32_t)(wave + NW * n) * 1024u);
      }
    });
  };
  const uint32_t b_voff = (uint32_t)lane * 16u + (uint32_t)nu * 8192u;
  u32x4v bh[2][CT], bl[2][CT];
  auto issue_b1 = [&](auto slc, auto jc, uint32_t koff) {
    constexpr int SLX = decltype(slc)::value, J = decltype(jc)::value;
    if constexpr (J & 1) buf_load16<(J & 3) * 1024>(bl[SLX][J >> 1], b_voff, srd_u, koff + (J >> 2) * 4096u);
    else buf_load16<(J & 3) * 1024>(bh[SLX][J >> 1], b_voff, srd_u, koff + (J >> 2) * 4096u);
  };

  const int toff0 = nu == 0 ? 0 : 1, toff1 = nu == 3 ? 3 : 2;
  const float tsg = nu == 1 ? 1.f : -1.f;
  const int pl = lane & 31, h = lane >> 5;
  const char* ap[RT][2][2];
#pragma unroll
  for (int rt = 0; rt < RT; ++rt) {
    const int q = min(q0 + rt * 32 + pl, q_last);
    const int R = q / p.PW, xg = q - R * p.PW;
    const int jrow = (R + R / p.H + 1) - sig_b - 1;
#pragma unroll
    for (int t = 0; t < 2; ++t) {
      const int wx = G * xg + (t == 0 ? toff0 : toff1);
      const int pp = wx / G, ph = wx - pp * G, swz = (pp >> 2) & 3;
      const int off = jrow * ROWB + (pp >> 3) * (G * 512) + ph * 512 + (pp & 7) * 64;
#pragma unroll
      for (int ch = 0; ch < 2; ++ch) ap[rt][t][ch] = s_win + off + (((2 * h + ch) ^ swz) << 4);
    }
  }

  f32x16 acc[RT][CT];
#pragma unroll
  for (int i = 0; i < RT; ++i)
#pragma unroll
    for (int j = 0; j < CT; ++j)
#pragma unroll
      for (int r = 0; r < 16; ++r) acc[i][j][r] = 0.f;

  struct Raw { uint4 d[RT][2][2]; };
  auto load_raw = [&](auto wbc, auto kyc, Raw& r) {
    constexpr int AOFF = decltype(wbc)::value * WIN_CAP + decltype(kyc)::value * ROWB;
#pragma unroll
    for (int rt = 0; rt < RT; ++rt)
#pragma unroll
      for (int t = 0; t < 2; ++t) { r.d[rt][t][0] = *(const uint4*)(ap[rt][t][0] + AOFF); r.d[rt][t][1] = *(const uint4*)(ap[rt][t][1] + AOFF); }
  };
  auto transform = [&](const Raw& r, bf16x8 (&ah)[RT], bf16x8 (&al)[RT]) {
#pragma unroll
    for (int rt = 0; rt < RT; ++rt) {
      float v[8];
#pragma unroll
      for (int c = 0; c < 2; ++c) {
        const uint32_t e0[4] = {r.d[rt][0][c].x, r.d[rt][0][c].y, r.d[rt][0][c].z, r.d[rt][0][c].w};
        const uint32_t e1[4] = {r.d[rt][1][c].x, r.d[rt][1][c].y, r.d[rt][1][c].z, r.d[rt][1][c].w};
#pragma unroll
        for (int e = 0; e < 4; ++e) v[4 * c + e] = fmaf(tsg, __uint_as_float(e1[e]), __uint_as_float(e0[e]));
      }
      const uint4 v0 = make_uint4(__float_as_uint(v[0]), __float_as_uint(v[1]), __float_as_uint(v[2]), __float_as_uint(v[3]));
      const uint4 v1 = make_uint4(__float_as_uint(v[4]), __float_as_uint(v[5]), __float_as_uint(v[6]), __float_as_uint(v[7]));
      split_f32x8(v0, v1, ah[rt], al[rt]);
    }
  };

  issue_window(std::integral_constant<int, 0>{}, 0, lds_win);
  issue_window(std::integral_constant<int, 1>{}, 0, lds_win);
  static_for<8>([&](auto jc) { issue_b1(std::integral_constant<int, 0>{}, jc, 0u); });
  if (NSL > 1) issue_window(std::integral_constant<int, 0>{}, 1, lds_win + WIN_CAP);
  bf16x8 fh[2][RT], fl[2][RT];
  asm volatile("s_waitcnt vmcnt(0)" ::: "memory");
  __builtin_amdgcn_s_barrier();
  {
    Raw r0;
    load_raw(std::integral_constant<int, 0>{}, std::integral_constant<int, 0>{}, r0);
    transform(r0, fh[0], fl[0]);
  }
  constexpr int NM1 = RT * CT;
  uint32_t nh[RT][4], nl[RT][4];
#pragma nounroll
  for (int s2 = 0; s2 < NSL / 2; ++s2) {
    static_for<6>([&](auto uc) {
      constexpr int U = decltype(uc)::value, KY = U % 3, SL = U & 1, WB = U / 3;
      constexpr int U1 = (U + 1) % 6, KY1 = U1 % 3, WB1 = U1 / 3;
      const int k = 6 * s2 + U, cs = 2 * s2 + WB;
      asm volatile("s_waitcnt vmcnt(0)"
                   : "+v"(bh[SL][0]), "+v"(bh[SL][1]), "+v"(bh[SL][2]), "+v"(bh[SL][3]), "+v"(bl[SL][0]), "+v"(bl[SL][1]), "+v"(bl[SL][2]), "+v"(bl[SL][3])
                   :
                   : "memory");
      if constexpr (KY == 2) __builtin_amdgcn_s_barrier();
      Raw raw;
      load_raw(std::integral_constant<int, WB1>{}, std::integral_constant<int, KY1>{}, raw);
      __builtin_amdgcn_sched_barrier(0);
      const uint32_t kn = (uint32_t)min(k + 1, KT - 1) * USTAGE;
      auto vmem_slot = [&](auto vc) {
        constexpr int V = decltype(vc)::value;
        if constexpr (V < 8) {
          issue_b1(std::integral_constant<int, SL ^ 1>{}, std::integral_constant<int, V>{}, kn);
        } else if constexpr (KY != 1 && V < 8 + HB) {
          constexpr int n = (KY == 0 ? HB : 0) + (V - 8);
          const int csn = KY == 0 ? cs + 1 : cs + 2;
          if (csn < NSL && (pokm & (1u << n))) {
            const uint32_t v = (prowokm & (1u << n)) ? w_voff : MCG_OOB_OFFSET;
            lds_dma16<0>(v, srd_x, prow[n] + (uint32_t)csn * (KS * 4), lds_win + (KY == 0 ? (WB ^ 1) : WB) * WIN_CAP + (uint32_t)(wave + NW * n) * 1024u);
          }
        }
      };
      static_for<NM1>([&](auto mc) {
        constexpr int M = decltype(mc)::value, I = M / CT, J = M % CT;
        acc[I][J] = x3_mfma(fl[SL][I], __builtin_bit_cast(bf16x8, bh[SL][J]), acc[I][J]);
        if constexpr (M % 3 == 0) {
          __builtin_amdgcn_sched_barrier(0);
          vmem_slot(std::integral_constant<int, M / 3>{});
          __builtin_amdgcn_sched_barrier(0);
        }
      });
      __builtin_amdgcn_sched_barrier(0);
      static_for<8>([&](auto qc) {
        constexpr int Q = decltype(qc)::value, I = Q & 3, TERM3 = Q >> 2;
        constexpr int XR = Q >> 1, XC = Q & 1;
        {
          const uint32_t e0[4] = {raw.d[XR][0][XC].x, raw.d[XR][0][XC].y, raw.d[XR][0][XC].z, raw.d[XR][0][XC].w};
          const uint32_t e1[4] = {raw.d[XR][1][XC].x, raw.d[XR][1][XC].y, raw.d[XR][1][XC].z, raw.d[XR][1][XC].w};
          float v[4];
#pragma unroll
          for (int e = 0; e < 4; ++e) v[e] = fmaf(tsg, __uint_as_float(e1[e]), __uint_as_float(e0[e]));
          split_pair(v[0], v[1], nh[XR][2 * XC], nl[XR][2 * XC]);
          split_pair(v[2], v[3], nh[XR][2 * XC + 1], nl[XR][2 * XC + 1]);
        }
#pragma unroll
        for (int j2 = 0; j2 < CT; ++j2)
          acc[I][j2] = x3_mfma(fh[SL][I], __builtin_bit_cast(bf16x8, TERM3 ? bh[SL][j2] : bl[SL][j2]), acc[I][j2]);
        asm volatile("" : "+v"(nh[XR][2 * XC]), "+v"(nh[XR][2 * XC + 1]), "+v"(nl[XR][2 * XC]), "+v"(nl[XR][2 * XC + 1]));
        static_for<4>([&](auto) {
          __builtin_amdgcn_sched_group_barrier(0x008, 1, 0);
          __builtin_amdgcn_sched_group_barrier(0x002, 4, 0);
        });
        __builtin_amdgcn_sched_barrier(0);
        vmem_slot(std::integral_constant<int, 6 + Q>{});
        __builtin_amdgcn_sched_barrier(0);
      });
#pragma unroll
      for (int rt = 0; rt < RT; ++rt) {
        fh[SL ^ 1][rt] = __builtin_bit_cast(bf16x8, make_uint4(nh[rt][0], nh[rt][1], nh[rt][2], nh[rt][3]));
        fl[SL ^ 1][rt] = __builtin_bit_cast(bf16x8, make_uint4(nl[rt][0], nl[rt][1], nl[rt][2], nl[rt][3]));
      }
    });
  }
  asm volatile("s_waitcnt vmcnt(0) lgkmcnt(0)"
               : "+v"(bh[0][0]), "+v"(bh[0][1]), "+v"(bh[0][2]), "+v"(bh[0][3]), "+v"(bl[0][0]), "+v"(bl[0][1]), "+v"(bl[0][2]), "+v"(bl[0][3]),
                 "+v"(bh[1][0]), "+v"(bh[1][1]), "+v"(bh[1][2]), "+v"(bh[1][3]), "+v"(bl[1][0]), "+v"(bl[1][1]), "+v"(bl[1][2]), "+v"(bl[1][3])
               :
               : "memory");
  __syncthreads();

  constexpr int PP = 64, CPR = NT / 4;
  float* const C = (float*)smem;
  const float wsc = p.wscale > 0.f ? p.wscale : 1.f;
#pragma unroll
  for (int pass = 0; pass < 2; ++pass) {
#pragma unroll
    for (int rt = 0; rt < 2; ++rt)
#pragma unroll
      for (int ct = 0; ct < CT; ++ct)
#pragma unroll
        for (int r = 0; r < 16; ++r)
          C[(nu * PP + rt * 32 + mfma32_row(r, lane)) * NT + ct * 32 + (lane & 31)] = acc[2 * pass + rt][ct][r];
    __syncthreads();
    for (int item = tid; item < PP * CPR; item += 256) {
      const int prl = item / CPR, ch4 = (item - prl * CPR) * 4;
      const int q = q0 + pass * PP + prl;
      if (q >= q_end) continue;
      float4 bv = make_float4(0.f, 0.f, 0.f, 0.f);
      if (p.bias) bv = *(const float4*)(p.bias + n0 + ch4);
      float4 m[NV];
#pragma unroll
      for (int v = 0; v < NV; ++v) m[v] = *(const float4*)(C + (v * PP + prl) * NT + ch4);
      float4 y[2];
      y[0] = make_float4(((m[0].x + m[1].x) + m[2].x) * wsc + bv.x, ((m[0].y + m[1].y) + m[2].y) * wsc + bv.y, ((m[0].z + m[1].z) + m[2].z) * wsc + bv.z, ((m[0].w + m[1].w) + m[2].w) * wsc + bv.w);
      y[1] = make_float4(((m[1].x - m[2].x) - m[3].x) * wsc + bv.x, ((m[1].y - m[2].y) - m[3].y) * wsc + bv.y, ((m[1].z - m[2].z) - m[3].z) * wsc + bv.z, ((m[1].w - m[2].w) - m[3].w) * wsc + bv.w);
      const int R = q / p.PW, xo = G * (q - R * p.PW);
      float* yp = p.y + ((long long)R * p.W + xo) * p.Cout + n0 + ch4;
#pragma unroll
      for (int j = 0; j < 2; ++j) {
        if (xo + j >= p.W) break;
        float4 o = y[j];
        if (p.relu) { o.x = fmaxf(o.x, 0.f); o.y = fmaxf(o.y, 0.f); o.z = fmaxf(o.z, 0.f); o.w = fmaxf(o.w, 0.f); }
        *(float4*)(yp + (long long)j * p.Cout) = o;
      }
    }
    __syncthreads();
  }
}

static inline int wino_x3_tile_groups(int g, int shape) { return g == 2 ? ((shape == 0 || shape == 3) ? 128 : (shape == 1 ? 64 : 32)) : (shape == 0 ? 64 : 32); }
static inline int wino_x3_tile_channels(int shape) { return (shape == 0 || shape == 3) ? 128 : 64; }
static inline int wino_x3_pieces(int W, int g) { return (g * ((W + g - 1) / g) + 2 + 8 * g - 1) / (8 * g) * (g / 2); }
static inline int wino_x3_max_rows(int H, int W, int mt, int g, bool cross) {
  const int PW = (W + g - 1) / g;
  int rows = (PW - 1 + mt - 1) / PW + 1;
  if (!cross && rows > H) rows = H;
  const int nz = cross ? (rows >= 2 ? (rows - 2) / H + 1 : 0) : 0;
  return rows + nz + 2;
}
static inline int wino_x3_nb_template(int pieces) { return pieces <= 1 ? 1 : (pieces <= 2 ? 2 : 4); }
static inline int wino_x3_mode(int frames, int H, int W, int Cin, int Cout, int g) {
  if (Cin % 32 != 0 || Cout % wnx::UNT != 0 || H < 1 || W < 2 || frames < 1 || (g != 2 && g != 4)) return 0;
  if (g == 4 && (W % 4 != 0 || W < 16)) return 0;
  const int pcs = wino_x3_pieces(W, g);
  if (pcs > 4) return 0;
  const int nb = wino_x3_nb_template(pcs);
  const long long px = (long long)frames * H * W;
  if (!(px * Cin * 4 < MCG_DMA_MAX_BYTES && px * Cout * 4 < MCG_DMA_MAX_BYTES && px < 0x7fffffffLL)) return 0;
  const int mt = wino_x3_tile_groups(g, 0), cap = wnx::wcap(g, 4);
  if (wino_x3_max_rows(H, W, mt, g, true) * nb * 1024 <= cap) return 1;
  if (wino_x3_max_rows(H, W, mt, g, false) * nb * 1024 <= cap) return 2;
  return 0;
}
static inline bool wino_x3_applicable(int frames, int H, int W, int Cin, int Cout, int g = 2) { return wino_x3_mode(frames, H, W, Cin, Cout, g) != 0; }
static inline size_t wino_x3_weight_bytes(int Cin, int Cout, int g = 2) { return (size_t)(Cout / wnx::UNT) * (3 * Cin / wnx::KS) * wnx::ustage(g); }

template <int NB, int RH, int RT, int CT, int G>
static inline int launch_wino_x3_t(hipStream_t s, const WinoParams& p, int grid) {
  constexpr int kLds = 2 * wnx::wcap(G, CT) + 2 * ((G + 2) * CT * 2 * 1024);
  static bool raised[MCG_MAX_DEVICES] = {false};
  int dev = 0;
  if (hipGetDevice(&dev) != hipSuccess || dev < 0 || dev >= MCG_MAX_DEVICES) dev = 0;
  if (!raised[dev]) {
    if (hipFuncSetAttribute((const void*)wino_x3_kernel<NB, RH, RT, CT, G>, hipFuncAttributeMaxDynamicSharedMemorySize, kLds) != hipSuccess) return 1;
    raised[dev] = true;
  }
  hipLaunchKernelGGL((wino_x3_kernel<NB, RH, RT, CT, G>), dim3(grid), dim3(64 * (G + 2) * RH), kLds, s, p);
  return hipGetLastError() == hipSuccess ? 0 : 1;
}
template <int NB>
static inline int launch_wino_x3w(hipStream_t s, const WinoParams& p, int grid) {
  constexpr int kLds = 4 * 64 * 128 * 4;
  static bool raised[MCG_MAX_DEVICES] = {false};
  int dev = 0;
  if (hipGetDevice(&dev) != hipSuccess || dev < 0 || dev >= MCG_MAX_DEVICES) dev = 0;
  if (!raised[dev]) {
    if (hipFuncSetAttribute((const void*)wino_x3w_kernel<NB>, hipFuncAttributeMaxDynamicSharedMemorySize, kLds) != hipSuccess) return 1;
    raised[dev] = true;
  }
  hipLaunchKernelGGL((wino_x3w_kernel<NB>), dim3(grid), dim3(256), kLds, s, p);
  return hipGetLastError() == hipSuccess ? 0 : 1;
}
template <int NB>
static inline int launch_wino_x3_nb(hipStream_t s, const WinoParams& p, int g, int shape, int grid) {
  if (g == 2 && shape == 3) return launch_wino_x3w<NB>(s, p, grid);
  if (g == 4) return shape == 0 ? launch_wino_x3_t<NB, 2, 1, 4, 4>(s, p, grid) : launch_wino_x3_t<NB, 1, 1, 2, 4>(s, p, grid);
  if (shape == 0) return launch_wino_x3_t<NB, 2, 2, 4, 2>(s, p, grid);
  if (shape == 1) return launch_wino_x3_t<NB, 2, 1, 2, 2>(s, p, grid);
  return launch_wino_x3_t<NB, 1, 1, 2, 2>(s, p, grid);
}
static const int kWinoMinGrid = 130;
static inline int launch_wino_x3(hipStream_t s, WinoParams p, int shape = -1, int g = 2) {
  const int mode = wino_x3_mode(p.frames, p.H, p.W, p.Cin, p.Cout, g);
  if (mode == 0) return 1;
  p.PW = (p.W + g - 1) / g;
  p.gpf = p.H * p.PW;
  p.total_pairs = p.frames * p.gpf;
  auto mtiles = [&](int sh) {
    const int mt = wino_x3_tile_groups(g, sh);
    return mode == 2 ? p.frames * ((p.gpf + mt - 1) / mt) : (p.total_pairs + mt - 1) / mt;
  };
  auto grid_of = [&](int sh) { return mtiles(sh) * (p.Cout / wino_x3_tile_channels(sh)); };
  if (shape < 0) shape = grid_of(0) >= kWinoMinGrid ? (g == 2 ? 3 : 0) : ((g == 2 && grid_of(1) >= kWinoMinGrid) ? 1 : 2);
  if (g == 4 && (shape == 1 || shape == 3)) shape = 2;
  p.n_tiles = p.Cout / wino_x3_tile_channels(shape);
  p.tpf = mode == 2 ? (p.gpf + wino_x3_tile_groups(g, shape) - 1) / wino_x3_tile_groups(g, shape) : 0;
  const int grid = grid_of(shape);
  const int nb = wino_x3_nb_template(wino_x3_pieces(p.W, g));
  if (nb == 1) return launch_wino_x3_nb<1>(s, p, g, shape, grid);
  if (nb == 2) return launch_wino_x3_nb<2>(s, p, g, shape, grid);
  return launch_wino_x3_nb<4>(s, p, g, shape, grid);
}
```

### mcgaze_amd/engine.py

```python
import ctypes as C
import os

import numpy as np
import torch

from . import lib as L
from .packing import PackedWeights

_TORCH_DT = {'bf16': torch.bfloat16, 'f16': torch.float16, 'fp16': torch.float16, 'fp32': torch.float32, 'f32': torch.float32, 'f16x3': torch.float32, 'bf16x3': torch.float32}
_CODE = {'bf16': L.MCG_BF16, 'f16': L.MCG_F16, 'fp16': L.MCG_F16, 'fp32': L.MCG_F32, 'f32': L.MCG_F32, 'f16x3': L.MCG_F16X3,
         'bf16x3': L.MCG_F16X3}


def _code(dtype):
    return L.MCG_BF16 if dtype == torch.bfloat16 else (L.MCG_F16 if dtype == torch.float16 else L.MCG_F32)


def _ptr(t):
    return C.c_void_p(t.data_ptr()) if t is not None else C.c_void_p(0)


def _stream(device=None):
    return C.c_void_p(torch.cuda.current_stream(device).cuda_stream)


def _require_gpu():
    if not torch.cuda.is_available():
        raise L.McgError('mcgaze_amd needs a HIP device (MI355X / gfx950); there is no CPU fallback path')


def _ws(nbytes, device):
    return torch.empty(max(int(nbytes), 256), dtype=torch.uint8, device=device)


def to_nhwc(x_nchw, dtype):
    _require_gpu()
    lib = L.load()
    N, Cc, H, W = x_nchw.shape
    x = x_nchw.contiguous().float()
    out = torch.empty(N, H, W, Cc, dtype=dtype, device=x.device)
    L.check(lib.mcg_nchw_to_nhwc(_stream(), _code(dtype), _ptr(x), _ptr(out), N, Cc, H, W), 'mcg_nchw_to_nhwc')
    return out


def to_nchw(x_nhwc):
    _require_gpu()
    lib = L.load()
    N, H, W, Cc = x_nhwc.shape
    out = torch.empty(N, Cc, H, W, dtype=torch.float32, device=x_nhwc.device)
    L.check(lib.mcg_nhwc_to_nchw(_stream(), _code(x_nhwc.dtype), _ptr(x_nhwc.contiguous()), _ptr(out), N, Cc, H, W), 'mcg_nhwc_to_nchw')
    return out


def conv2d(x, w, bias=None, stride=1, pad=0, relu=False, residual=None, residual_mode=L.RES_NONE, x2=None, stride2=1, split=False,
           tile=0, flags=0, prescale=True):
    _require_gpu()
    lib = L.load()
    N, H, W, Cin = x.shape
    Cout, KH, KW, _ = w.shape
    wscale = 0.0
    if split:
        from .packing import pow2_prescale, split_pack
        assert x.dtype == torch.float32 and w.dtype == torch.float32
        ws, wscale = pow2_prescale(w.reshape(Cout, -1).cpu()) if prescale else (w.reshape(Cout, -1).cpu(), 0.0)
        w = split_pack(ws).to(x.device)
    Cin2 = x2.shape[3] if x2 is not None else 0
    Ho, Wo = (H + 2 * pad - KH) // stride + 1, (W + 2 * pad - KW) // stride + 1
    y = torch.empty(N, Ho, Wo, Cout, dtype=x.dtype, device=x.device)
    d = L.ConvDesc(x.data_ptr(), w.data_ptr(), bias.data_ptr() if bias is not None else None,
                   residual.data_ptr() if residual is not None else None, y.data_ptr(),
                   N, H, W, Cin, Cout, KH, KW, stride, pad, int(relu), residual_mode if residual is not None else L.RES_NONE,
                   residual.shape[1] if residual is not None else 0, residual.shape[2] if residual is not None else 0,
                   x2.data_ptr() if x2 is not None else None, Cin2, stride2, x2.shape[1] if x2 is not None else 0,
                   x2.shape[2] if x2 is not None else 0, tile, flags, wscale)
    L.check(lib.mcg_conv2d(_stream(), L.MCG_F16X3 if split else _code(x.dtype), C.byref(d)), 'mcg_conv2d')
    return y


def conv3x3_wino(x, w, bias=None, relu=False, tile=0, g=2):
    _require_gpu()
    lib = L.load()
    from .packing import pow2_prescale, wino_pack
    N, H, W, Cin = x.shape
    Cout = w.shape[0]
    ws, wscale = pow2_prescale(w.cpu())
    u = wino_pack(ws, g=g).to(x.device)
    assert u.numel() * 2 == lib.mcg_conv3x3_wino_x3_weight_bytes(Cin, Cout, g), (u.numel(), Cin, Cout)
    y = torch.empty(N, H, W, Cout, dtype=torch.float32, device=x.device)
    L.check(lib.mcg_conv3x3_wino_x3(_stream(), _ptr(x.contiguous()), _ptr(u), _ptr(bias), _ptr(y), N, H, W, Cin, Cout, int(relu), tile, wscale, g), 'mcg_conv3x3_wino_x3')
    return y


def bottleneck_x3(x, src2, wstream, bias, cn, nsrc, trace=None):
    _require_gpu()
    lib = L.load()
    N, H, W, cm = x.shape
    y = torch.empty(N, H, W, 4 * cm, dtype=torch.float32, device=x.device)
    z = torch.empty(N, H, W, cn, dtype=torch.float32, device=x.device) if cn else None
    L.check(lib.mcg_bottleneck_x3(_stream(), _ptr(x.contiguous()), _ptr(src2.contiguous()), _ptr(wstream), _ptr(bias), _ptr(y), _ptr(z),
                                  N, H, W, cm, nsrc, cn, _ptr(trace)), 'mcg_bottleneck_x3')
    return y, z


def stem(img, w_stem, bias, dtype, flags=0, split=False):
    _require_gpu()
    lib = L.load()
    N, _, H, W = img.shape
    code = L.MCG_F16X3 if split else _code(dtype)
    ws = _ws(lib.mcg_stem_workspace_bytes(code, N, H, W), img.device)
    y = torch.empty(N, H // 4, W // 4, 64, dtype=dtype, device=img.device)
    L.check(lib.mcg_stem_forward(_stream(), code, _ptr(img.contiguous()), _ptr(w_stem), _ptr(bias), _ptr(y), N, H, W,
                                 _ptr(ws), ws.numel(), flags), 'mcg_stem_forward')
    return y


def roi_align(feats, boxes, strides=(4, 8, 16, 32)):
    _require_gpu()
    lib = L.load()
    N, P = boxes.shape[:2]
    Cc = feats[0].shape[-1]
    out = torch.empty(N * P, 49, Cc, dtype=feats[0].dtype, device=boxes.device)
    lv = torch.empty(N * P, dtype=torch.int32, device=boxes.device)
    fp = (C.c_void_p * 4)(*[f.data_ptr() for f in feats])
    fh = (C.c_int * 4)(*[f.shape[1] for f in feats])
    fw = (C.c_int * 4)(*[f.shape[2] for f in feats])
    st = (C.c_int * 4)(*strides)
    b = boxes.contiguous().float()
    L.check(lib.mcg_roi_align(_stream(), _code(feats[0].dtype), fp, fh, fw, st, Cc, _ptr(b), N * P, P, _ptr(out), _ptr(lv)), 'mcg_roi_align')
    return out, lv


def roi_align_indexed(feats, boxes, frame_of, strides=(4, 8, 16, 32)):
    _require_gpu()
    lib = L.load()
    N, P = boxes.shape[:2]
    K, Cc = feats[0].shape[0], feats[0].shape[-1]
    table = torch.from_numpy(check_frame_table(frame_of, K, 1)).to(boxes.device)
    if table.numel() != N:
        raise L.McgError(f'frame_of holds {table.numel()} entries for {N} frames of boxes')
    out = torch.empty(N * P, 49, Cc, dtype=feats[0].dtype, device=boxes.device)
    lv = torch.empty(N * P, dtype=torch.int32, device=boxes.device)
    fp = (C.c_void_p * 4)(*[f.data_ptr() for f in feats])
    fh = (C.c_int * 4)(*[f.shape[1] for f in feats])
    fw = (C.c_int * 4)(*[f.shape[2] for f in feats])
    st = (C.c_int * 4)(*strides)
    b = boxes.contiguous().float()
    L.check(lib.mcg_roi_align_indexed(_stream(), _code(feats[0].dtype), fp, fh, fw, st, Cc, _ptr(b), N * P, P, _ptr(table), K, _ptr(out), _ptr(lv)),
            'mcg_roi_align_indexed')
    return out, lv


def check_frame_table(frame_of, pyramid_frames, clip_length):
    t = frame_of.numpy() if isinstance(frame_of, torch.Tensor) else frame_of
    try:
        a = np.asarray(t)
    except Exception as ex:
        raise L.McgError(f'frame_of must be a flat sequence of row indices ({ex})')
    if a.ndim != 1 or (a.size and not np.issubdtype(a.dtype, np.integer)):
        raise L.McgError(f'frame_of must be a flat sequence of integer row indices (got {a.dtype} of shape {a.shape})')
    if clip_length < 1 or a.size == 0 or a.size % clip_length:
        raise L.McgError(f'frame_of holds {a.size} entries, not a positive multiple of clip_length={clip_length}')
    if pyramid_frames < 1 or int(a.min()) < 0 or int(a.max()) >= pyramid_frames:
        raise L.McgError(f'frame_of entries must lie in [0, {pyramid_frames}) (got {int(a.min())} .. {int(a.max())})')
    return a.astype(np.int32)


def _table(d, keys):
    return (C.c_void_p * len(keys))(*[d[k].data_ptr() for k in keys])


def stage_forward(stage_w, roi_feat, obj, boxes, clip_length, stds=(0.5, 0.5, 1.0, 1.0), split=False, flags=0):
    _require_gpu()
    lib = L.load()
    N = obj.shape[0]
    dt = L.MCG_F16X3 if split else _code(obj.dtype)
    ws = _ws(lib.mcg_stage_workspace_bytes(dt, N), obj.device)
    obj_out = torch.empty_like(obj)
    boxes_out = torch.empty(N, 3, 4, dtype=torch.float32, device=obj.device)
    cls = torch.empty(N, 3, dtype=torch.float32, device=obj.device)
    sd = (C.c_float * 4)(*stds)
    L.check(lib.mcg_stage_forward(_stream(), dt, _table(stage_w, L.STAGE_KEYS), _ptr(roi_feat.contiguous()), _ptr(obj.contiguous()),
                                  _ptr(boxes.contiguous().float()), N, clip_length, _ptr(obj_out), _ptr(boxes_out), _ptr(cls), sd,
                                  _ptr(ws), ws.numel(), flags), 'mcg_stage_forward')
    return obj_out, boxes_out, cls


def gaze_head(gaze_w, obj, split=False):
    _require_gpu()
    lib = L.load()
    N = obj.shape[0]
    dt = L.MCG_F16X3 if split else _code(obj.dtype)
    ws = _ws(lib.mcg_gaze_head_workspace_bytes(dt, N), obj.device)
    out = torch.empty(4, N, 3, dtype=torch.float32, device=obj.device)
    L.check(lib.mcg_gaze_head(_stream(), dt, _table(gaze_w, L.GAZE_KEYS), _ptr(obj.contiguous()), N, _ptr(out), _ptr(ws), ws.numel()), 'mcg_gaze_head')
    return out


class HipEngine:

    def __init__(self, state_dict, depth=50, num_stages=4, precision='f16x3', device='cuda:0', bbox_stds=(0.5, 0.5, 1.0, 1.0), fuse_downsample=True):
        _require_gpu()
        self.lib = L.load()
        self.device = torch.device(device)
        self.dtype = _TORCH_DT[precision]
        self.code = _CODE[precision]
        self.precision = precision
        self.weights = PackedWeights(state_dict, depth=depth, num_stages=num_stages, dtype=self.dtype, device=self.device,
                                     fuse_downsample=fuse_downsample, split=self.code == L.MCG_F16X3)
        w = self.weights
        mk = lambda c: L.ConvWeights(c['w'].data_ptr(), c['bias'].data_ptr(), c['cin'], c['cout'], c['k'], c['stride'], c['pad'],
                                     c['wf'].data_ptr() if c.get('wf') is not None else None, float(c.get('wscale', 0.0)),
                                     c['wf4'].data_ptr() if c.get('wf4') is not None else None)
        self._convs = (L.ConvWeights * len(w.convs))(*[mk(c) for c in w.convs])
        self._stage_tab = (C.c_void_p * (num_stages * L.SW_COUNT))(*[st[k].data_ptr() for st in w.stages for k in L.STAGE_KEYS])
        self._gaze_tab = _table(w.gaze, L.GAZE_KEYS)
        mw = L.ModelWeights()
        mw.blocks = (C.c_int * 4)(*w.blocks)
        mw.stem = mk(w.stem)
        mw.convs = C.cast(self._convs, C.POINTER(L.ConvWeights))
        mw.num_convs = len(w.convs)
        mw.lateral = (L.ConvWeights * 4)(*[mk(c) for c in w.lateral])
        mw.fpn_out = (L.ConvWeights * 4)(*[mk(c) for c in w.fpn_out])
        if len(w.c3_ds) == 4:
            mw.c3_ds = (L.ConvWeights * 4)(*[mk(c) for c in w.c3_ds])
        mw.init_boxes = w.init_boxes.data_ptr()
        mw.init_feats = w.init_feats.data_ptr()
        mw.num_stages = num_stages
        mw.stage_weights = C.cast(self._stage_tab, C.POINTER(C.c_void_p))
        mw.gaze_weights = C.cast(self._gaze_tab, C.POINTER(C.c_void_p))
        mw.bbox_stds = (C.c_float * 4)(*bbox_stds)
        if w.fused:
            self._fused = (L.FusedBlock * len(w.fused))(*[L.FusedBlock(f['wstream'].data_ptr(), f['bias'].data_ptr(), f['conv2_index'], f['cm'], f['c'],
                                                                      f['cn'], f['nsrc']) for f in w.fused])
            mw.fused, mw.num_fused = C.cast(self._fused, C.POINTER(L.FusedBlock)), len(w.fused)
        self._handle = C.c_void_p()
        with torch.cuda.device(self.device):
            L.check(self.lib.mcg_engine_create(C.byref(self._handle), C.byref(mw), self.code), 'mcg_engine_create')
        self._ws = None
        self._ws_key = None
        self._dec_ws = None

    def set_option(self, name, value):
        L.check(self.lib.mcg_engine_set_option(self._handle, name.encode(), int(value)), f'mcg_engine_set_option({name})')

    def range_audit(self, capacity=256):
        counts = (C.c_ulonglong * (2 * capacity))()
        names = (C.c_char_p * capacity)()
        n = C.c_int()
        L.check(self.lib.mcg_engine_range_audit(self._handle, counts, names, capacity, C.byref(n)), 'mcg_engine_range_audit')
        return [(names[i].decode(), int(counts[2 * i]), int(counts[2 * i + 1])) for i in range(n.value)]

    def profile_start(self, capacity=4096):
        L.check(self.lib.mcg_engine_profile_start(self._handle, capacity), 'mcg_engine_profile_start')

    def profile_stop(self, capacity=4096):
        cnt = C.c_int()
        ms = (C.c_float * capacity)(); fl = (C.c_double * capacity)(); by = (C.c_double * capacity)()
        cf = (C.c_int * capacity)(); sh = (C.c_int * (3 * capacity))()
        L.check(self.lib.mcg_engine_profile_stop(self._handle, C.byref(cnt), ms, fl, by, cf, sh, capacity), 'mcg_engine_profile_stop')
        return [(ms[i], fl[i], cf[i], (sh[3 * i], sh[3 * i + 1], sh[3 * i + 2]), by[i]) for i in range(cnt.value)]

    def backbone_only(self, img, return_levels=False):
        self._check_img(img)
        N, _, H, W = img.shape
        with torch.cuda.device(self.device):
            ws = self._workspace(N, H, W, 0)
            L.check(self.lib.mcg_bench_backbone_forward(self._handle, _stream(self.device), _ptr(img), N, H, W, _ptr(ws), ws.numel()), 'mcg_bench_backbone_forward')
            if not return_levels:
                return None
            tab = (C.c_void_p * 4)()
            L.check(self.lib.mcg_bench_backbone_levels(self._handle, _ptr(ws), N, H, W, tab), 'mcg_bench_backbone_levels')
            es = ws.element_size() * (2 if self.dtype in (torch.bfloat16, torch.float16) else 4)
            out = []
            for i in range(4):
                shape = (N, (H // 4) >> i, (W // 4) >> i, 256 << i)
                n = shape[0] * shape[1] * shape[2] * shape[3]
                off = tab[i] - ws.data_ptr()
                out.append(ws[off:off + n * es].view(self.dtype).view(shape))
            return out

    def __del__(self):
        h = getattr(self, '_handle', None)
        if h is not None and h.value:
            self.lib.mcg_engine_destroy(h)
            self._handle = None

    def _workspace(self, N, H, W, chunk):
        key = (N, H, W, chunk)
        need = self.lib.mcg_engine_workspace_bytes(self._handle, N, H, W, chunk)
        if self._ws is None or self._ws.numel() < need or self._ws_key != key:
            if self._ws is None or self._ws.numel() < need:
                self._ws = None
                self._ws = _ws(need, self.device)
            self._ws_key = key
        return self._ws

    def _check_img(self, img):
        if not (img.is_cuda and img.device == self.device and img.dtype == torch.float32 and img.is_contiguous() and img.dim() == 4):
            raise L.McgError(f'img must be a contiguous float32 [N,3,H,W] tensor on {self.device} (got {img.dtype} {tuple(img.shape)} on {img.device})')

    def backbone_fpn(self, img, chunk_frames=0, out=None, row=0):
        self._check_img(img)
        N, _, H, W = img.shape
        shapes = [((H // 4) >> i, (W // 4) >> i, 256) for i in range(4)]
        if out is not None:
            K = self._check_pyramid(out, shapes)
            if not (0 <= row and row + N <= K):
                raise L.McgError(f'backbone_fpn: rows [{row}, {row + N}) do not fit a pyramid store of {K} rows')
        with torch.cuda.device(self.device):
            ws = self._workspace(N, H, W, chunk_frames)
            if out is None:
                pyr, row = [torch.empty((N,) + s, dtype=self.dtype, device=self.device) for s in shapes], 0
            else:
                pyr = out
            es = pyr[0].element_size()
            tab = (C.c_void_p * 4)(*[p.data_ptr() + row * s[0] * s[1] * s[2] * es for p, s in zip(pyr, shapes)])
            L.check(self.lib.mcg_backbone_fpn_forward(self._handle, _stream(self.device), _ptr(img), N, H, W, chunk_frames, tab, _ptr(ws), ws.numel()),
                    'mcg_backbone_fpn_forward')
        return pyr

    def _check_pyramid(self, pyramid, shapes=None):
        if len(pyramid) != 4:
            raise L.McgError(f'a pyramid is four levels (got {len(pyramid)})')
        K = pyramid[0].shape[0]
        if shapes is None:
            h, w = pyramid[0].shape[1], pyramid[0].shape[2]
            shapes = [(h >> i, w >> i, 256) for i in range(4)]
        for i, (p, s) in enumerate(zip(pyramid, shapes)):
            if not (p.dtype == self.dtype and p.device == self.device and p.is_contiguous() and tuple(p.shape) == (K,) + tuple(s)):
                raise L.McgError(f'pyramid level {i} must be a contiguous {self.dtype} [{K},{s[0]},{s[1]},256] tensor on {self.device} '
                                 f'(got {p.dtype} {tuple(p.shape)} on {p.device})')
        return K

    def decode(self, pyramid, frame_of, clip_length, img_hw=None, out=None):
        K = pyramid[0].shape[0] if len(pyramid) else 0
        H, W = (pyramid[0].shape[1] * 4, pyramid[0].shape[2] * 4) if len(pyramid) else (0, 0)
        dev_table = isinstance(frame_of, torch.Tensor) and frame_of.device.type != 'cpu'
        host = None if dev_table else check_frame_table(frame_of, K, clip_length)
        self._check_pyramid(pyramid)
        with torch.cuda.device(self.device):
            if dev_table:
                if not (frame_of.dtype == torch.int32 and frame_of.device == self.device and frame_of.dim() == 1):
                    raise L.McgError(f'a device frame_of must be a 1-D int32 tensor on {self.device} (got {frame_of.dtype} {tuple(frame_of.shape)} on {frame_of.device})')
                table = frame_of.contiguous()
                if table.numel() == 0 or table.numel() % clip_length:
                    raise L.McgError(f'frame_of holds {table.numel()} entries, not a positive multiple of clip_length={clip_length}')
            else:
                table = torch.from_numpy(host).pin_memory().to(self.device, non_blocking=True)
            N = table.numel()
            if out is None:
                out = dict(gaze=torch.empty(4, N, 3, dtype=torch.float32, device=self.device),
                           boxes=torch.empty(N, 3, 4, dtype=torch.float32, device=self.device),
                           scores=torch.empty(N, 3, dtype=torch.float32, device=self.device))
            hw = self.img_hw_tensor(img_hw, K)
            need = self.lib.mcg_decoder_workspace_bytes(self._handle, N)
            if self._dec_ws is None or self._dec_ws.numel() < need:
                self._dec_ws = None
                self._dec_ws = _ws(need, self.device)
            ws = self._dec_ws
            tab = (C.c_void_p * 4)(*[p.data_ptr() for p in pyramid])
            L.check(self.lib.mcg_decoder_forward_indexed(self._handle, _stream(self.device), tab, K, _ptr(table), N, clip_length, H, W, _ptr(hw),
                                                         _ptr(out['gaze']), _ptr(out['boxes']), _ptr(out['scores']), _ptr(ws), ws.numel()),
                    'mcg_decoder_forward_indexed')
        return out

    def forward(self, img, clip_length, img_hw=None, chunk_frames=0, out=None):
        self._check_img(img)
        N, _, H, W = img.shape
        with torch.cuda.device(self.device):
            ws = self._workspace(N, H, W, chunk_frames)
            if out is None:
                out = dict(gaze=torch.empty(4, N, 3, dtype=torch.float32, device=self.device),
                           boxes=torch.empty(N, 3, 4, dtype=torch.float32, device=self.device),
                           scores=torch.empty(N, 3, dtype=torch.float32, device=self.device))
            hw = self.img_hw_tensor(img_hw, N)
            L.check(self.lib.mcg_clip_forward(self._handle, _stream(self.device), _ptr(img), N, clip_length, H, W, _ptr(hw), chunk_frames,
                                              _ptr(out['gaze']), _ptr(out['boxes']), _ptr(out['scores']), _ptr(ws), ws.numel()),
                    'mcg_clip_forward')
        return out

    def img_hw_tensor(self, img_hw, N):
        if img_hw is None:
            return None
        if not isinstance(img_hw, torch.Tensor):
            img_hw = torch.as_tensor(np.asarray(img_hw, dtype=np.int32).reshape(N, 2))
        hw = img_hw.to(device=self.device, dtype=torch.int32).contiguous()
        if hw.numel() != 2 * N:
            raise L.McgError(f'img_hw must hold {N} (h, w) pairs, got {tuple(hw.shape)}')
        return hw


class GraphedForward:

    def __init__(self, engine, num_frames, H, W, clip_length, with_img_hw=False):
        e = self.e = engine
        self.N, self.T = num_frames, clip_length
        dev = e.device
        with torch.cuda.device(dev):
            self.img = torch.zeros(num_frames, 3, H, W, dtype=torch.float32, device=dev)
            self.hw = torch.zeros(num_frames, 2, dtype=torch.int32, device=dev) if with_img_hw else None
            if self.hw is not None:
                self.hw[:, 0], self.hw[:, 1] = H, W
            self.out = dict(gaze=torch.zeros(4, num_frames, 3, device=dev), boxes=torch.zeros(num_frames, 3, 4, device=dev),
                            scores=torch.zeros(num_frames, 3, device=dev))
            side = torch.cuda.Stream(device=dev)
            side.wait_stream(torch.cuda.current_stream(dev))
            with torch.cuda.stream(side):
                for _ in range(2):
                    e.forward(self.img, clip_length, img_hw=self.hw, out=self.out)
            torch.cuda.current_stream(dev).wait_stream(side)
            torch.cuda.synchronize(dev)
            self.graph = torch.cuda.CUDAGraph()
            with torch.cuda.graph(self.graph, stream=side):
                e.forward(self.img, clip_length, img_hw=self.hw, out=self.out)

    def __call__(self, img, img_hw=None):
        self.e._check_img(img)
        if tuple(img.shape) != tuple(self.img.shape):
            raise L.McgError(f'GraphedForward was captured for {tuple(self.img.shape)}, got {tuple(img.shape)}')
        self.img.copy_(img, non_blocking=True)
        if img_hw is not None:
            if self.hw is None:
                raise L.McgError('GraphedForward was captured without img_hw (with_img_hw=True to enable)')
            self.hw.copy_(self.e.img_hw_tensor(img_hw, self.N), non_blocking=True)
        self.graph.replay()
        return self.out


_PIPELINE_STREAMS = {}


def pipeline_streams(device, decoder_priority=-1):
    dev = torch.device(device)
    key = (dev.index if dev.index is not None else torch.cuda.current_device(), decoder_priority)
    if key not in _PIPELINE_STREAMS:
        _PIPELINE_STREAMS[key] = (torch.cuda.Stream(device=dev), torch.cuda.Stream(device=dev, priority=decoder_priority))
    return _PIPELINE_STREAMS[key]


class PipelinedRunner:

    def __init__(self, engine, num_frames, H, W, clip_length, chunk_frames=0, decoder_priority=-1):
        self.e, self.N, self.H, self.W, self.T, self.chunk = engine, num_frames, H, W, clip_length, chunk_frames
        dev, lib, h = engine.device, engine.lib, engine._handle
        self.sa, self.sb = pipeline_streams(dev, decoder_priority)
        self.pyr = [[torch.empty(num_frames, (H // 4) >> i, (W // 4) >> i, 256, dtype=engine.dtype, device=dev) for i in range(4)] for _ in range(2)]
        self.tabs = [(C.c_void_p * 4)(*[p.data_ptr() for p in lvl]) for lvl in self.pyr]
        self.trunk_ws = _ws(lib.mcg_trunk_workspace_bytes(h, num_frames, H, W, chunk_frames), dev)
        self.dec_ws = _ws(lib.mcg_decoder_workspace_bytes(h, num_frames), dev)
        self.trunk_done = [torch.cuda.Event() for _ in range(2)]
        self.dec_done = [torch.cuda.Event() for _ in range(2)]
        self.used = [False, False]
        self._hw_keep = [None, None]
        self.k = 0

    def submit(self, img, out, img_hw=None):
        with torch.cuda.device(self.e.device):
            return self._submit(img, out, img_hw)

    def _submit(self, img, out, img_hw):
        e, lib, slot = self.e, self.e.lib, self.k & 1
        e._check_img(img)
        img_hw = e.img_hw_tensor(img_hw, self.N)
        if img_hw is not None:
            img_hw.record_stream(self.sb)
        self._hw_keep[slot] = img_hw
        cur = torch.cuda.current_stream(e.device)
        self.sa.wait_stream(cur)
        if self.used[slot]:
            self.sa.wait_event(self.dec_done[slot])
        L.check(lib.mcg_backbone_fpn_forward(e._handle, C.c_void_p(self.sa.cuda_stream), _ptr(img), self.N, self.H, self.W, self.chunk,
                                             self.tabs[slot], _ptr(self.trunk_ws), self.trunk_ws.numel()), 'mcg_backbone_fpn_forward')
        self.trunk_done[slot].record(self.sa)
        self.sb.wait_event(self.trunk_done[slot])
        L.check(lib.mcg_decoder_forward(e._handle, C.c_void_p(self.sb.cuda_stream), self.tabs[slot], self.N, self.T, self.H, self.W,
                                        _ptr(img_hw), _ptr(out['gaze']), _ptr(out['boxes']), _ptr(out['scores']),
                                        _ptr(self.dec_ws), self.dec_ws.numel()), 'mcg_decoder_forward')
        self.dec_done[slot].record(self.sb)
        self.used[slot] = True
        self.k += 1
        return self.dec_done[slot]

    def flush(self):
        cur = torch.cuda.current_stream(self.e.device)
        for slot in range(2):
            if self.used[slot]:
                cur.wait_event(self.dec_done[slot])
```

### mcgaze_amd/lib.py

```python
import ctypes as C
import os

_HERE = os.path.dirname(os.path.abspath(__file__))
LIB_PATH = os.environ.get('MCGAZE_LIB') or os.path.join(_HERE, 'libmcgaze_hip.so')

MCG_OK = 0
MCG_F32, MCG_BF16, MCG_F16X3, MCG_F16 = 0, 1, 2, 3
ABI_VERSION = 14
RES_NONE, RES_ADD, RES_UPSAMPLE_ADD = 0, 1, 2
FLAG_STAGED_GEMM, FLAG_NO_SPECIALISED, FLAG_NO_ATTN_BLOCK = 1, 2, 4

STAGE_KEYS = [
    'IN_PROJ_W', 'IN_PROJ_B', 'OUT_PROJ_W', 'OUT_PROJ_B', 'ATTN_LN_G', 'ATTN_LN_B', 'DYN_W', 'DYN_B',
    'NORM_IN_G', 'NORM_IN_B', 'NORM_OUT_G', 'NORM_OUT_B', 'FC_W', 'FC_B', 'FC_LN_G', 'FC_LN_B', 'IIC_LN_G', 'IIC_LN_B',
    'FFN1_W', 'FFN1_B', 'FFN2_W', 'FFN2_B', 'FFN_LN_G', 'FFN_LN_B', 'CLS_FC_W', 'CLS_LN_G', 'CLS_LN_B',
    'REG_FC_W', 'REG_LN_G', 'REG_LN_B', 'HEAD_CLS_W', 'HEAD_CLS_B', 'HEAD_REG_W', 'HEAD_REG_B', 'OUT_PROJ_WF', 'CLS_FC_WF', 'REG_FC_WF', 'IN_PROJ_WF', 'DYN_WF']
GAZE_KEYS = ['FC_W', 'LN_G', 'LN_B', 'OUT_W', 'OUT_B', 'FUSE_W', 'FUSE_B']
SW_COUNT, GW_COUNT = len(STAGE_KEYS), len(GAZE_KEYS)

EXPORTS = ['mcg_abi_version', 'mcg_build_id', 'mcg_last_error', 'mcg_device_info', 'mcg_nchw_to_nhwc', 'mcg_nhwc_to_nchw', 'mcg_conv2d',
           'mcg_stem_workspace_bytes', 'mcg_stem_forward', 'mcg_roi_align', 'mcg_stage_workspace_bytes', 'mcg_stage_forward',
           'mcg_gaze_head_workspace_bytes', 'mcg_gaze_head', 'mcg_engine_create', 'mcg_engine_destroy',
           'mcg_engine_workspace_bytes', 'mcg_trunk_workspace_bytes', 'mcg_decoder_workspace_bytes', 'mcg_backbone_fpn_forward',
           'mcg_decoder_forward', 'mcg_clip_forward', 'mcg_preprocess_frames', 'mcg_engine_set_option', 'mcg_engine_profile_start',
           'mcg_engine_profile_stop', 'mcg_bench_backbone_forward', 'mcg_bottleneck_x3', 'mcg_bench_backbone_levels', 'mcg_conv3x3_wino_x3',
           'mcg_conv3x3_wino_x3_weight_bytes', 'mcg_engine_range_audit', 'mcg_roi_align_indexed', 'mcg_decoder_forward_indexed']


class ConvDesc(C.Structure):
    _fields_ = [('x', C.c_void_p), ('w', C.c_void_p), ('bias', C.c_void_p), ('residual', C.c_void_p), ('y', C.c_void_p),
                ('N', C.c_int), ('H', C.c_int), ('W', C.c_int), ('Cin', C.c_int), ('Cout', C.c_int), ('KH', C.c_int),
                ('KW', C.c_int), ('stride', C.c_int), ('pad', C.c_int), ('relu', C.c_int), ('residual_mode', C.c_int),
                ('Hr', C.c_int), ('Wr', C.c_int), ('x2', C.c_void_p), ('Cin2', C.c_int), ('stride2', C.c_int), ('H2', C.c_int),
                ('W2', C.c_int), ('tile', C.c_int), ('flags', C.c_int), ('wscale', C.c_float)]


class ConvWeights(C.Structure):
    _fields_ = [('w', C.c_void_p), ('bias', C.c_void_p), ('cin', C.c_int), ('cout', C.c_int), ('k', C.c_int),
                ('stride', C.c_int), ('pad', C.c_int), ('wf', C.c_void_p), ('wscale', C.c_float), ('wf4', C.c_void_p)]


class FusedBlock(C.Structure):
    _fields_ = [('wstream', C.c_void_p), ('bias', C.c_void_p), ('conv2_index', C.c_int), ('cm', C.c_int), ('c', C.c_int), ('cn', C.c_int),
                ('nsrc', C.c_int)]


class ModelWeights(C.Structure):
    _fields_ = [('blocks', C.c_int * 4), ('stem', ConvWeights), ('convs', C.POINTER(ConvWeights)), ('num_convs', C.c_int),
                ('lateral', ConvWeights * 4), ('fpn_out', ConvWeights * 4), ('c3_ds', ConvWeights * 4), ('init_boxes', C.c_void_p),
                ('init_feats', C.c_void_p), ('num_stages', C.c_int), ('stage_weights', C.POINTER(C.c_void_p)),
                ('gaze_weights', C.POINTER(C.c_void_p)), ('bbox_stds', C.c_float * 4), ('fused', C.POINTER(FusedBlock)), ('num_fused', C.c_int)]


class FrameDesc(C.Structure):
    _fields_ = [('src', C.c_void_p), ('src_h', C.c_int), ('src_w', C.c_int), ('src_pitch', C.c_int), ('crop_y', C.c_int),
                ('crop_x', C.c_int), ('crop_h', C.c_int), ('crop_w', C.c_int), ('out_h', C.c_int), ('out_w', C.c_int)]


class McgError(RuntimeError):
    pass


_lib = None


def load():
    global _lib
    if _lib is not None:
        return _lib
    if not os.path.exists(LIB_PATH):
        raise McgError(f'{LIB_PATH} not found: build it with `python -c "import __graft_entry__ as g; g.build()"` '
                       f'(or `make -C mcgaze_amd/csrc`); mcgaze_amd has no CPU fallback')
    lib = C.CDLL(LIB_PATH)
    vp, i, sz = C.c_void_p, C.c_int, C.c_size_t
    lib.mcg_abi_version.restype = i
    lib.mcg_last_error.restype = C.c_char_p
    lib.mcg_build_id.restype = C.c_char_p
    lib.mcg_device_info.argtypes = [C.POINTER(i), C.POINTER(sz), C.c_char_p, i]
    lib.mcg_nchw_to_nhwc.argtypes = [vp, i, vp, vp, i, i, i, i]
    lib.mcg_nhwc_to_nchw.argtypes = [vp, i, vp, vp, i, i, i, i]
    lib.mcg_conv2d.argtypes = [vp, i, C.POINTER(ConvDesc)]
    lib.mcg_stem_workspace_bytes.restype = sz
    lib.mcg_stem_workspace_bytes.argtypes = [i, i, i, i]
    lib.mcg_stem_forward.argtypes = [vp, i, vp, vp, vp, vp, i, i, i, vp, sz, i]
    lib.mcg_roi_align.argtypes = [vp, i, C.POINTER(vp), C.POINTER(i), C.POINTER(i), C.POINTER(i), i, vp, i, i, vp, vp]
    lib.mcg_roi_align_indexed.argtypes = [vp, i, C.POINTER(vp), C.POINTER(i), C.POINTER(i), C.POINTER(i), i, vp, i, i, vp, i, vp, vp]
    lib.mcg_stage_workspace_bytes.restype = sz
    lib.mcg_stage_workspace_bytes.argtypes = [i, i]
    lib.mcg_stage_forward.argtypes = [vp, i, C.POINTER(vp), vp, vp, vp, i, i, vp, vp, vp, C.POINTER(C.c_float), vp, sz, i]
    lib.mcg_gaze_head_workspace_bytes.restype = sz
    lib.mcg_gaze_head_workspace_bytes.argtypes = [i, i]
    lib.mcg_gaze_head.argtypes = [vp, i, C.POINTER(vp), vp, i, vp, vp, sz]
    lib.mcg_engine_create.argtypes = [C.POINTER(vp), C.POINTER(ModelWeights), i]
    lib.mcg_engine_destroy.argtypes = [vp]
    lib.mcg_engine_destroy.restype = None
    lib.mcg_engine_workspace_bytes.restype = sz
    lib.mcg_engine_workspace_bytes.argtypes = [vp, i, i, i, i]
    lib.mcg_trunk_workspace_bytes.restype = sz
    lib.mcg_trunk_workspace_bytes.argtypes = [vp, i, i, i, i]
    lib.mcg_decoder_workspace_bytes.restype = sz
    lib.mcg_decoder_workspace_bytes.argtypes = [vp, i]
    lib.mcg_decoder_forward.argtypes = [vp, vp, C.POINTER(vp), i, i, i, i, vp, vp, vp, vp, vp, sz]
    lib.mcg_decoder_forward_indexed.argtypes = [vp, vp, C.POINTER(vp), i, vp, i, i, i, i, vp, vp, vp, vp, vp, sz]
    lib.mcg_backbone_fpn_forward.argtypes = [vp, vp, vp, i, i, i, i, C.POINTER(vp), vp, sz]
    lib.mcg_clip_forward.argtypes = [vp, vp, vp, i, i, i, i, vp, i, vp, vp, vp, vp, sz]
    lib.mcg_preprocess_frames.argtypes = [vp, vp, i, vp, i, i, C.POINTER(C.c_float), C.POINTER(C.c_float), i]
    lib.mcg_engine_set_option.argtypes = [vp, C.c_char_p, i]
    lib.mcg_engine_profile_start.argtypes = [vp, i]
    lib.mcg_engine_profile_stop.argtypes = [vp, C.POINTER(i), C.POINTER(C.c_float), C.POINTER(C.c_double), C.POINTER(C.c_double), C.POINTER(i), C.POINTER(i), i]
    lib.mcg_bench_backbone_forward.argtypes = [vp, vp, vp, i, i, i, vp, sz]
    lib.mcg_bench_backbone_levels.argtypes = [vp, vp, i, i, i, C.POINTER(vp)]
    lib.mcg_bottleneck_x3.argtypes = [vp, vp, vp, vp, vp, vp, vp, i, i, i, i, i, i, vp]
    lib.mcg_conv3x3_wino_x3.argtypes = [vp, vp, vp, vp, vp, i, i, i, i, i, i, i, C.c_float, i]
    lib.mcg_conv3x3_wino_x3_weight_bytes.restype = sz
    lib.mcg_engine_range_audit.argtypes = [vp, C.POINTER(C.c_ulonglong), C.POINTER(C.c_char_p), i, C.POINTER(i)]
    lib.mcg_conv3x3_wino_x3_weight_bytes.argtypes = [i, i, i]
    for name in EXPORTS:
        fn = getattr(lib, name)
        if fn.restype is C.c_int and name not in ('mcg_abi_version',):
            fn.restype = i
    if lib.mcg_abi_version() != ABI_VERSION:
        raise McgError(f'ABI mismatch: library reports {lib.mcg_abi_version()}, binding expects {ABI_VERSION}')
    _lib = lib
    return lib


def build_id():
    return load().mcg_build_id().decode()


def source_id():
    import hashlib
    src = os.path.join(_HERE, 'csrc')
    names = sorted(n for n in os.listdir(src) if n.endswith('.hip') or n.endswith('.hpp'))
    h = hashlib.sha256()
    for n in names:
        h.update(open(os.path.join(src, n), 'rb').read())
    h.update(open(os.path.join(_HERE, '..', 'include', 'mcgaze_hip.h'), 'rb').read())
    return h.hexdigest()[:16]


def check(rc, what):
    if rc != MCG_OK:
        msg = load().mcg_last_error().decode(errors='replace')
        raise McgError(f'{what} failed (code {rc}): {msg}')
```

Before: 3323 clips/s.

## Defer P2 FPN output conv to decoder and compute only ROI-touched blocks

The trunk now skips the 3x3 fpn_out conv for the finest pyramid level and keeps the lateral inner map in a slot buffer. Before each decoder stage, a mark kernel finds which 8x8 spatial blocks the current boxes touch, and a new Winograd block kernel computes P2 only for those blocks not already done. This targets the largest FPN output conv, most of whose output ROI-align never reads. In exchange it adds per-stage launches, state clearing and a separate slot layout, and it changes the pipelined engine and clip_forward APIs.

```diff
diff --git a/include/mcgaze_hip.h b/include/mcgaze_hip.h
--- a/include/mcgaze_hip.h
+++ b/include/mcgaze_hip.h
@@ -8,7 +8,7 @@
 extern "C" {
 #endif
 
-#define MCG_ABI_VERSION 14
+#define MCG_ABI_VERSION 15
 
 enum { MCG_OK = 0, MCG_ERR_ARG = 1, MCG_ERR_HIP = 2, MCG_ERR_UNSUPPORTED = 3, MCG_ERR_WORKSPACE = 4 };
 typedef enum { MCG_F32 = 0, MCG_BF16 = 1, MCG_F16X3 = 2, MCG_F16 = 3 } mcg_dtype;
@@ -157,6 +157,12 @@
 int mcg_decoder_forward_indexed(mcg_engine* e, mcg_stream s, const void* const pyramid[4], int pyramid_frames, const int32_t* frame_of,
                                 int num_frames, int clip_length, int H, int W, const int* img_hw, float* gaze_out, float* boxes_out,
                                 float* scores_out, void* ws, size_t ws_bytes);
+size_t mcg_deferred_pyramid_bytes(const mcg_engine* e, int num_frames, int H, int W);
+int mcg_deferred_pyramid_levels(const mcg_engine* e, void* slot, int num_frames, int H, int W, void* levels[4], int* deferred);
+int mcg_backbone_fpn_forward_deferred(mcg_engine* e, mcg_stream s, const float* img, int num_frames, int H, int W, int chunk_frames,
+                                      void* slot, size_t slot_bytes, void* ws, size_t ws_bytes);
+int mcg_decoder_forward_deferred(mcg_engine* e, mcg_stream s, void* slot, size_t slot_bytes, int num_frames, int clip_length, int H, int W,
+                                 const int* img_hw, float* gaze_out, float* boxes_out, float* scores_out, void* ws, size_t ws_bytes);
 int mcg_clip_forward(mcg_engine* e, mcg_stream s, const float* img, int num_frames, int clip_length, int H, int W,
                      const int* img_hw, int chunk_frames, float* gaze_out, float* boxes_out, float* scores_out,
                      void* ws, size_t ws_bytes);
diff --git a/mcgaze_amd/csrc/check_resources.py b/mcgaze_amd/csrc/check_resources.py
--- a/mcgaze_amd/csrc/check_resources.py
+++ b/mcgaze_amd/csrc/check_resources.py
@@ -4,6 +4,7 @@
 
 RULES = {
     'wino_x3w_kernel': dict(scratch=0, vgpr_spill=0, unit='engine'),
+    'wino_x3w_blocks_kernel': dict(scratch=0, vgpr_spill=0, unit='engine'),
 }
 
 
diff --git a/mcgaze_amd/csrc/engine.hip b/mcgaze_amd/csrc/engine.hip
--- a/mcgaze_amd/csrc/engine.hip
+++ b/mcgaze_amd/csrc/engine.hip
@@ -18,6 +18,10 @@
                      int pyramid_frames, void* out, int32_t* levels_out);
 int launch_init_queries(hipStream_t s, mcg_dtype dt, const float* init_boxes, const void* init_feats, const int* img_hw,
                         const int32_t* frame_of, int pyramid_frames, int H, int W, float* boxes, void* obj, int N);
+bool roi_mark_supported(int H, int W);
+int launch_defer_clear(hipStream_t s, int* p, int n);
+int launch_roi_mark(hipStream_t s, const float* boxes, int num_boxes, int boxes_per_frame, int level, int H, int W, int stride, int* state,
+                    int* list, int* count);
 
 struct mcg_engine {
   mcg_dtype dt;
@@ -30,6 +34,7 @@
   bool bneck_blocked = true;
   int winograd = 1;
   int wino_tile = -1;
+  int fpn_deferred = 1;
   static constexpr int kAuditCap = 256;
   unsigned long long* audit_dev = nullptr;
   std::vector<std::string> audit_names;
@@ -177,6 +182,7 @@
   else if (!strcmp(name, "bottleneck_fused")) e->bneck_fused = value != 0;
   else if (!strcmp(name, "bottleneck_blocked")) e->bneck_blocked = value != 0;
   else if (!strcmp(name, "winograd")) { MCG_CHECK_ARG(value >= 0 && value <= 2, "winograd must be 0, 1 or 2"); e->winograd = value; }
+  else if (!strcmp(name, "fpn_deferred")) e->fpn_deferred = value != 0;
   else if (!strcmp(name, "wino_tile")) { MCG_CHECK_ARG(value >= -1 && value <= 3, "wino_tile must be -1 (by grid size) .. 3"); e->wino_tile = value; }
   else if (!strcmp(name, "range_audit")) {
     MCG_CHECK_ARG(!mcg_is16(e->dt) || !value, "range_audit: f32-storage engines only (MCG_F32, MCG_F16X3)");
@@ -303,6 +309,12 @@
   }
   t.total = off;
   return t;
+}
+
+static int wino_kind(const mcg_engine* e, mcg_dtype dt, const mcg_conv_weights& cw, int n, int h, int w, int rm) {
+  return (dt == MCG_F16X3 && e->winograd && e->ctx.tile < 0 && cw.k == 3 && cw.stride == 1 && cw.pad == 1 && rm == MCG_RES_NONE)
+             ? ((cw.wf4 && e->winograd >= 2 && wino_x3_applicable(n, h, w, cw.cin, cw.cout, 4)) ? 4 : ((cw.wf && wino_x3_applicable(n, h, w, cw.cin, cw.cout, 2)) ? 2 : 0))
+             : 0;
 }
 
 static int conv_call(const mcg_engine* e, hipStream_t s, mcg_dtype dt, const mcg_conv_weights& cw, const void* x, int n, int h, int w, void* y,
@@ -345,9 +357,7 @@
     if (prc) { mcg_set_error("pw_single_x3 launch failed"); return MCG_ERR_HIP; }
     return MCG_OK;
   }
-  const int wg = (dt == MCG_F16X3 && e->winograd && e->ctx.tile < 0 && cw.k == 3 && cw.stride == 1 && cw.pad == 1 && rm == MCG_RES_NONE)
-                     ? ((cw.wf4 && e->winograd >= 2 && wino_x3_applicable(n, h, w, cw.cin, cw.cout, 4)) ? 4 : ((cw.wf && wino_x3_applicable(n, h, w, cw.cin, cw.cout, 2)) ? 2 : 0))
-                     : 0;
+  const int wg = wino_kind(e, dt, cw, n, h, w, rm);
   if (wg) {
     WinoParams wp;
     memset(&wp, 0, sizeof(wp));
@@ -364,10 +374,11 @@
 }
 
 static int trunk_chunk(mcg_engine* e, hipStream_t s, const float* img, int f0, int n, int H, int W, void* const pyr[4], char* wsbase,
-                       bool backbone_only = false) {
+                       bool backbone_only = false, char* inner0 = nullptr) {
   const mcg_dtype dt = e->dt;
   const size_t es = esize(dt);
   TrunkWs t = trunk_layout(dt, n, H, W, wsbase);
+  if (inner0) t.l[0] = inner0 + (size_t)f0 * (H / 4) * (W / 4) * 256 * es;
   MCG_TRY(stem_forward_ctx(s, dt, img + (size_t)f0 * 3 * H * W, e->stem.w, e->stem.bias, t.x0, n, H, W, t.stem_ws, t.stem_bytes, e->ctx));
   AuditCursor au{e, s, 0, e->audit_dev != nullptr && e->audit_names.empty()};
   char aname[64];
@@ -498,7 +509,7 @@
     snprintf(aname, sizeof(aname), "fpn.lateral%d (+ top-down)", i);
     audit_tensor(au, aname, t.l[i], (long long)n * hs[i] * wsz[i] * 256);
   }
-  for (int i = 0; i < 4; ++i) {
+  for (int i = inner0 ? 1 : 0; i < 4; ++i) {
     char* dst = (char*)pyr[i] + (size_t)f0 * hs[i] * wsz[i] * 256 * es;
     MCG_TRY(conv_call(e, s, dt, e->fpn_out[i], t.l[i], n, hs[i], wsz[i], dst, 0, nullptr, MCG_RES_NONE, 0, 0));
     snprintf(aname, sizeof(aname), "fpn.P%d", i + 2);
@@ -542,8 +553,41 @@
   c.total = off;
   return c;
 }
+static bool check_shape_ok(int N, int H, int W) { return N > 0 && H >= 32 && W >= 32 && H % 32 == 0 && W % 32 == 0; }
 static size_t pyramid_bytes(mcg_dtype dt, int N, int H, int W, int level) {
   return al256((size_t)N * ((H / 4) >> level) * ((W / 4) >> level) * 256 * esize(dt));
+}
+
+struct DeferSlot {
+  void* p[4];
+  char* inner;
+  int *state, *count, *list;
+  int nblk;
+  bool deferred;
+  size_t total;
+};
+static bool fpn_deferred_on(const mcg_engine* e, int N, int H, int W) {
+  const mcg_conv_weights& cw = e->fpn_out[0];
+  const int h = H / 4, w = W / 4;
+  return e->fpn_deferred && e->dt == MCG_F16X3 && !e->audit_dev && e->num_stages > 0 && wino_kind(e, e->dt, cw, N, h, w, MCG_RES_NONE) == 2 &&
+         wino_x3_blocks_applicable(N, h, w, cw.cin, cw.cout) && roi_mark_supported(h, w);
+}
+static DeferSlot defer_layout(const mcg_engine* e, int N, int H, int W, char* base) {
+  DeferSlot d;
+  memset(&d, 0, sizeof(d));
+  size_t off = 0;
+  auto take = [&](size_t bytes) { char* p = base ? base + off : nullptr; off += al256(bytes); return p; };
+  for (int i = 0; i < 4; ++i) d.p[i] = take(pyramid_bytes(e->dt, N, H, W, i));
+  d.deferred = fpn_deferred_on(e, N, H, W);
+  if (d.deferred) {
+    d.inner = take((size_t)N * (H / 4) * (W / 4) * 256 * esize(e->dt));
+    d.nblk = N * wino_x3_blocks_per_frame(H / 4, W / 4);
+    d.state = (int*)take(sizeof(int) * ((size_t)d.nblk + e->num_stages));
+    d.count = d.state ? d.state + d.nblk : nullptr;
+    d.list = (int*)take(sizeof(int) * (size_t)d.nblk * e->num_stages);
+  }
+  d.total = off;
+  return d;
 }
 
 extern "C" size_t mcg_trunk_workspace_bytes(const mcg_engine* e, int N, int H, int W, int chunk) {
@@ -565,9 +609,11 @@
 }
 extern "C" size_t mcg_engine_workspace_bytes(const mcg_engine* e, int N, int H, int W, int chunk) {
   if (!e || N <= 0) return 0;
-  size_t total = mcg_trunk_workspace_bytes(e, N, H, W, chunk) + mcg_decoder_workspace_bytes(e, N);
-  for (int i = 0; i < 4; ++i) total += pyramid_bytes(e->dt, N, H, W, i);
-  return total;
+  return mcg_trunk_workspace_bytes(e, N, H, W, chunk) + mcg_decoder_workspace_bytes(e, N) + defer_layout(e, N, H, W, nullptr).total;
+}
+extern "C" size_t mcg_deferred_pyramid_bytes(const mcg_engine* e, int N, int H, int W) {
+  if (!e || N <= 0 || check_shape_ok(N, H, W) == false) return 0;
+  return defer_layout(e, N, H, W, nullptr).total;
 }
 
 static int check_shape(int N, int H, int W) {
@@ -577,7 +623,7 @@
 }
 
 static int trunk_forward(mcg_engine* e, mcg_stream s_, const float* img, int N, int H, int W, int chunk,
-                         void* const pyramid[4], void* ws, size_t ws_bytes, bool backbone_only) {
+                         void* const pyramid[4], void* ws, size_t ws_bytes, bool backbone_only, char* inner0 = nullptr) {
   MCG_CHECK_ARG(e && img && (pyramid || backbone_only) && ws, "mcg_backbone_fpn_forward: null pointer");
   MCG_TRY(check_shape(N, H, W));
   std::lock_guard<std::mutex> lock(e->mu);
@@ -586,14 +632,14 @@
   if (ws_bytes < need) { mcg_set_error("mcg_backbone_fpn_forward: workspace too small (%zu < %zu)", ws_bytes, need); return MCG_ERR_WORKSPACE; }
   hipStream_t s = (hipStream_t)s_;
   if (chunk < N) {
-    for (int f0 = 0; f0 < N; f0 += chunk) MCG_TRY(trunk_chunk(e, s, img, f0, (N - f0) < chunk ? (N - f0) : chunk, H, W, pyramid, (char*)ws, backbone_only));
+    for (int f0 = 0; f0 < N; f0 += chunk) MCG_TRY(trunk_chunk(e, s, img, f0, (N - f0) < chunk ? (N - f0) : chunk, H, W, pyramid, (char*)ws, backbone_only, inner0));
     return MCG_OK;
   }
   const int k = trunk_ranges(e, N);
   const int cap = range_frame_cap(e, H, W);
   const int per = (N + k - 1) / k < cap ? (N + k - 1) / k : cap;
   if (k == 1) {
-    for (int f0 = 0; f0 < N; f0 += per) MCG_TRY(trunk_chunk(e, s, img, f0, (N - f0) < per ? (N - f0) : per, H, W, pyramid, (char*)ws, backbone_only));
+    for (int f0 = 0; f0 < N; f0 += per) MCG_TRY(trunk_chunk(e, s, img, f0, (N - f0) < per ? (N - f0) : per, H, W, pyramid, (char*)ws, backbone_only, inner0));
     return MCG_OK;
   }
   const std::vector<int>& sides = side_streams_for(e, s);
@@ -604,7 +650,7 @@
     if (hipStreamWaitEvent(e->cand[sides[i - 1]], e->ev_fork, 0) != hipSuccess) { mcg_set_error("mcg_backbone_fpn_forward: hipStreamWaitEvent failed"); return MCG_ERR_HIP; }
   for (int f0 = 0, i = 0; f0 < N && rc == MCG_OK; f0 += per, i = (i + 1) % k) {
     hipStream_t si = i == 0 ? s : e->cand[sides[i - 1]];
-    rc = trunk_chunk(e, si, img, f0, (N - f0) < per ? (N - f0) : per, H, W, pyramid, (char*)ws + (size_t)i * part_ws, backbone_only);
+    rc = trunk_chunk(e, si, img, f0, (N - f0) < per ? (N - f0) : per, H, W, pyramid, (char*)ws + (size_t)i * part_ws, backbone_only, inner0);
   }
   for (int i = 1; i < k; ++i) {
     hipStream_t si = e->cand[sides[i - 1]];
@@ -666,7 +712,7 @@
 
 static int decoder_forward(mcg_engine* e, hipStream_t s, const void* const pyramid[4], int pyramid_frames, const int32_t* frame_of, int N,
                            int clip_length, int H, int W, const int* img_hw, float* gaze_out, float* boxes_out, float* scores_out, void* ws,
-                           size_t ws_bytes) {
+                           size_t ws_bytes, const DeferSlot* d = nullptr) {
   MCG_CHECK_ARG(e && pyramid && gaze_out && boxes_out && scores_out && ws, "mcg_decoder_forward: null pointer");
   MCG_TRY(check_shape(N, H, W));
   MCG_CHECK_ARG(clip_length > 0 && N % clip_length == 0, "num_frames=%d is not a multiple of clip_length=%d", N, clip_length);
@@ -678,7 +724,23 @@
   for (int i = 0; i < 4; ++i) { fh[i] = (H / 4) >> i; fw[i] = (W / 4) >> i; }
   char* obj_in = c.obj_a; char* obj_out = c.obj_b;
   float* b_in = c.boxes_a; float* b_out = c.boxes_b;
+  const bool defer = d && d->deferred;
+  if (defer) MCG_TRY(launch_defer_clear(s, d->state, d->nblk + e->num_stages));
   for (int st = 0; st < e->num_stages; ++st) {
+    if (defer) {
+      const mcg_conv_weights& cw = e->fpn_out[0];
+      MCG_TRY(launch_roi_mark(s, b_in, N * 3, 3, 0, fh[0], fw[0], strides[0], d->state, d->list + (size_t)st * d->nblk, d->count + st));
+      WinoParams wp;
+      memset(&wp, 0, sizeof(wp));
+      wp.x = (const float*)d->inner; wp.u = cw.wf; wp.bias = cw.bias; wp.y = (float*)d->p[0];
+      wp.H = fh[0]; wp.W = fw[0]; wp.frames = N; wp.Cin = cw.cin; wp.Cout = cw.cout; wp.relu = 0; wp.wscale = cw.wscale;
+      const double M = (double)N * fh[0] * fw[0];
+      ProfRec* rec = prof_begin(e->ctx, s, 73, (int)M, cw.cout, 9 * cw.cin, st == 0 ? 2.0 * M * 9.0 * cw.cin * cw.cout : 0.0,
+                                st == 0 ? 4.0 * (M * (cw.cin + cw.cout) + 9.0 * cw.cin * cw.cout) : 0.0);
+      const int wrc = launch_wino_x3_blocks(s, wp, d->list + (size_t)st * d->nblk, d->count + st, d->nblk);
+      prof_end(rec, s);
+      if (wrc) { mcg_set_error("wino_x3 block launch failed"); return MCG_ERR_HIP; }
+    }
     MCG_TRY(launch_roi_align(s, e->dt, pyramid, fh, fw, strides, 256, b_in, N * 3, 3, frame_of, pyramid_frames, c.roi, nullptr));
     float* bdst = (st == e->num_stages - 1) ? boxes_out : b_out;
     MCG_TRY(stage_forward_ctx(s, e->dt, &e->stage_w[(size_t)st * MCG_SW_COUNT], c.roi, obj_in, b_in, N, clip_length, obj_out, bdst,
@@ -702,6 +764,33 @@
   MCG_CHECK_ARG(pyramid_frames > 0, "mcg_decoder_forward_indexed: empty pyramid store (pyramid_frames=%d)", pyramid_frames);
   return decoder_forward(e, (hipStream_t)s_, pyramid, pyramid_frames, frame_of, N, clip_length, H, W, img_hw, gaze_out, boxes_out, scores_out,
                          ws, ws_bytes);
+}
+
+extern "C" int mcg_deferred_pyramid_levels(const mcg_engine* e, void* slot, int N, int H, int W, void* levels[4], int* deferred) {
+  MCG_CHECK_ARG(e && slot && levels, "mcg_deferred_pyramid_levels: null pointer");
+  MCG_TRY(check_shape(N, H, W));
+  const DeferSlot d = defer_layout(e, N, H, W, (char*)slot);
+  for (int i = 0; i < 4; ++i) levels[i] = d.p[i];
+  if (deferred) *deferred = d.deferred ? 1 : 0;
+  return MCG_OK;
+}
+
+extern "C" int mcg_backbone_fpn_forward_deferred(mcg_engine* e, mcg_stream s, const float* img, int N, int H, int W, int chunk, void* slot,
+                                                 size_t slot_bytes, void* ws, size_t ws_bytes) {
+  MCG_CHECK_ARG(e && slot, "mcg_backbone_fpn_forward_deferred: null pointer");
+  MCG_TRY(check_shape(N, H, W));
+  const DeferSlot d = defer_layout(e, N, H, W, (char*)slot);
+  if (slot_bytes < d.total) { mcg_set_error("mcg_backbone_fpn_forward_deferred: slot too small (%zu < %zu)", slot_bytes, d.total); return MCG_ERR_WORKSPACE; }
+  return trunk_forward(e, s, img, N, H, W, chunk, d.p, ws, ws_bytes, false, d.deferred ? d.inner : nullptr);
+}
+
+extern "C" int mcg_decoder_forward_deferred(mcg_engine* e, mcg_stream s, void* slot, size_t slot_bytes, int N, int clip_length, int H, int W,
+                                            const int* img_hw, float* gaze_out, float* boxes_out, float* scores_out, void* ws, size_t ws_bytes) {
+  MCG_CHECK_ARG(e && slot, "mcg_decoder_forward_deferred: null pointer");
+  MCG_TRY(check_shape(N, H, W));
+  const DeferSlot d = defer_layout(e, N, H, W, (char*)slot);
+  if (slot_bytes < d.total) { mcg_set_error("mcg_decoder_forward_deferred: slot too small (%zu < %zu)", slot_bytes, d.total); return MCG_ERR_WORKSPACE; }
+  return decoder_forward(e, (hipStream_t)s, d.p, N, nullptr, N, clip_length, H, W, img_hw, gaze_out, boxes_out, scores_out, ws, ws_bytes, &d);
 }
 
 extern "C" int mcg_clip_forward(mcg_engine* e, mcg_stream s_, const float* img, int N, int clip_length, int H, int W,
@@ -714,9 +803,9 @@
   if (ws_bytes < need) { mcg_set_error("mcg_clip_forward: workspace too small (%zu < %zu)", ws_bytes, need); return MCG_ERR_WORKSPACE; }
   char* base = (char*)ws;
   const size_t trunk_bytes = mcg_trunk_workspace_bytes(e, N, H, W, chunk);
-  void* pyr[4];
-  size_t off = trunk_bytes;
-  for (int i = 0; i < 4; ++i) { pyr[i] = base + off; off += pyramid_bytes(e->dt, N, H, W, i); }
-  MCG_TRY(mcg_backbone_fpn_forward(e, s_, img, N, H, W, chunk, pyr, base, trunk_bytes));
-  return mcg_decoder_forward(e, s_, pyr, N, clip_length, H, W, img_hw, gaze_out, boxes_out, scores_out, base + off, ws_bytes - off);
-}
+  const size_t slot_bytes = defer_layout(e, N, H, W, nullptr).total;
+  const size_t off = trunk_bytes + slot_bytes;
+  MCG_TRY(mcg_backbone_fpn_forward_deferred(e, s_, img, N, H, W, chunk, base + trunk_bytes, slot_bytes, base, trunk_bytes));
+  return mcg_decoder_forward_deferred(e, s_, base + trunk_bytes, slot_bytes, N, clip_length, H, W, img_hw, gaze_out, boxes_out, scores_out,
+                                      base + off, ws_bytes - off);
+}
diff --git a/mcgaze_amd/csrc/roi_align.hip b/mcgaze_amd/csrc/roi_align.hip
--- a/mcgaze_amd/csrc/roi_align.hip
+++ b/mcgaze_amd/csrc/roi_align.hip
@@ -1,4 +1,5 @@
 #include "common.hpp"
+#include "roi_sample.hpp"
 
 struct RoiLevels {
   const void* feat[4];
@@ -17,28 +18,15 @@
   __shared__ int s_valid[2][NS];
   const int box = blockIdx.x, tid = threadIdx.x;
   const float x1 = boxes[box * 4 + 0], y1 = boxes[box * 4 + 1], x2 = boxes[box * 4 + 2], y2 = boxes[box * 4 + 3];
-  const float sc = sqrtf((x2 - x1) * (y2 - y1));
-  int level = (int)fminf(fmaxf(floorf(log2f(sc / finest_scale + 1e-6f)), 0.f), 3.f);
-  if (!(sc == sc)) level = 0;
+  const int level = roi_level(x1, y1, x2, y2, finest_scale);
   const int H = lv.h[level], W = lv.w[level];
   const float ss = lv.scale[level];
   if (tid < 2 * NS) {
     const int axis = tid / NS, i = tid % NS;
-    const float start = (axis == 0 ? y1 : x1) * ss - 0.5f, end = (axis == 0 ? y2 : x2) * ss - 0.5f;
-    const float bin = (end - start) / (float)P;
-    const int L = axis == 0 ? H : W;
-    float c = start + (float)(i / S) * bin + ((float)(i % S) + 0.5f) * bin / (float)S;
-    const int valid = !(c < -1.0f || c > (float)L);
-    c = fmaxf(c, 0.f);
-    int lo = (int)c, hi;
-    if (lo >= L - 1) {
-      lo = hi = L - 1;
-      c = (float)lo;
-    } else {
-      hi = lo + 1;
-    }
-    const float l = c - (float)lo;
-    s_lo[axis][i] = lo; s_hi[axis][i] = hi; s_l[axis][i] = l; s_h[axis][i] = 1.f - l; s_valid[axis][i] = valid && (c == c);
+    int lo, hi, valid;
+    float l;
+    roi_axis_sample<P, S>(axis == 0 ? y1 : x1, axis == 0 ? y2 : x2, ss, axis == 0 ? H : W, i, lo, hi, l, valid);
+    s_lo[axis][i] = lo; s_hi[axis][i] = hi; s_l[axis][i] = l; s_h[axis][i] = 1.f - l; s_valid[axis][i] = valid;
   }
   if (tid == 0) {
     if (levels_out) levels_out[box] = level;
@@ -92,6 +80,54 @@
   }
 }
 
+constexpr int kMarkMaxBlocks = 64;
+__global__ __launch_bounds__(256) void roi_mark_kernel(const float* __restrict__ boxes, int boxes_per_frame, int level_deferred, int H, int W,
+                                                       float ss, int* __restrict__ state, int* __restrict__ list, int* __restrict__ count,
+                                                       float finest_scale) {
+  constexpr int P = 7, S = 2, NS = P * S;
+  __shared__ int s_hit[2][kMarkMaxBlocks];
+  const int box = blockIdx.x, tid = threadIdx.x;
+  const float x1 = boxes[box * 4 + 0], y1 = boxes[box * 4 + 1], x2 = boxes[box * 4 + 2], y2 = boxes[box * 4 + 3];
+  if (roi_level(x1, y1, x2, y2, finest_scale) != level_deferred) return;
+  const int by_n = (H + 7) / 8, bx_n = (W + 7) / 8;
+  if (tid < 2 * kMarkMaxBlocks) s_hit[tid / kMarkMaxBlocks][tid % kMarkMaxBlocks] = 0;
+  __syncthreads();
+  if (tid < 2 * NS) {
+    const int axis = tid / NS, i = tid % NS;
+    int lo, hi, valid;
+    float l;
+    roi_axis_sample<P, S>(axis == 0 ? y1 : x1, axis == 0 ? y2 : x2, ss, axis == 0 ? H : W, i, lo, hi, l, valid);
+    if (valid) { s_hit[axis][lo >> 3] = 1; s_hit[axis][hi >> 3] = 1; }
+  }
+  __syncthreads();
+  const int frame = box / boxes_per_frame;
+  for (int t = tid; t < by_n * bx_n; t += 256) {
+    const int by = t / bx_n, bx = t - by * bx_n;
+    if (s_hit[0][by] && s_hit[1][bx]) {
+      const int id = frame * (by_n * bx_n) + t;
+      if (atomicCAS(&state[id], 0, 1) == 0) list[atomicAdd(count, 1)] = id;
+    }
+  }
+}
+__global__ void defer_clear_kernel(int* __restrict__ p, int n) {
+  for (int i = blockIdx.x * blockDim.x + threadIdx.x; i < n; i += gridDim.x * blockDim.x) p[i] = 0;
+}
+bool roi_mark_supported(int H, int W) { return (H + 7) / 8 <= kMarkMaxBlocks && (W + 7) / 8 <= kMarkMaxBlocks; }
+int launch_defer_clear(hipStream_t s, int* p, int n) {
+  const int blocks = (n + 255) / 256 < 1024 ? (n + 255) / 256 : 1024;
+  hipLaunchKernelGGL(defer_clear_kernel, dim3(blocks > 0 ? blocks : 1), dim3(256), 0, s, p, n);
+  MCG_CHECK_LAUNCH("defer_clear");
+  return MCG_OK;
+}
+int launch_roi_mark(hipStream_t s, const float* boxes, int num_boxes, int boxes_per_frame, int level, int H, int W, int stride, int* state,
+                    int* list, int* count) {
+  MCG_CHECK_ARG(roi_mark_supported(H, W), "roi_mark: deferred level of %dx%d pixels exceeds %d blocks per axis", H, W, kMarkMaxBlocks);
+  hipLaunchKernelGGL(roi_mark_kernel, dim3(num_boxes), dim3(256), 0, s, boxes, boxes_per_frame, level, H, W, 1.0f / (float)stride, state, list,
+                     count, 56.f);
+  MCG_CHECK_LAUNCH("roi_mark");
+  return MCG_OK;
+}
+
 int launch_roi_align(hipStream_t s, mcg_dtype dt, const void* const feats[4], const int feat_h[4], const int feat_w[4],
                      const int strides[4], int C, const float* boxes, int num_boxes, int boxes_per_frame, const int32_t* frame_of,
                      int pyramid_frames, void* out, int32_t* levels_out) {
diff --git a/mcgaze_amd/csrc/roi_sample.hpp b/mcgaze_amd/csrc/roi_sample.hpp
--- /dev/null
+++ b/mcgaze_amd/csrc/roi_sample.hpp
@@ -0,0 +1,25 @@
+#pragma once
+
+__device__ __forceinline__ int roi_level(float x1, float y1, float x2, float y2, float finest_scale) {
+  const float sc = sqrtf((x2 - x1) * (y2 - y1));
+  int level = (int)fminf(fmaxf(floorf(log2f(sc / finest_scale + 1e-6f)), 0.f), 3.f);
+  if (!(sc == sc)) level = 0;
+  return level;
+}
+
+template <int P, int S>
+__device__ __forceinline__ void roi_axis_sample(float a1, float a2, float ss, int L, int i, int& lo_out, int& hi_out, float& l_out, int& valid_out) {
+  const float start = a1 * ss - 0.5f, end = a2 * ss - 0.5f;
+  const float bin = (end - start) / (float)P;
+  float c = start + (float)(i / S) * bin + ((float)(i % S) + 0.5f) * bin / (float)S;
+  const int valid = !(c < -1.0f || c > (float)L);
+  c = fmaxf(c, 0.f);
+  int lo = (int)c, hi;
+  if (lo >= L - 1) {
+    lo = hi = L - 1;
+    c = (float)lo;
+  } else {
+    hi = lo + 1;
+  }
+  lo_out = lo; hi_out = hi; l_out = c - (float)lo; valid_out = valid && (c == c);
+}
diff --git a/mcgaze_amd/csrc/wino_x3.hpp b/mcgaze_amd/csrc/wino_x3.hpp
--- a/mcgaze_amd/csrc/wino_x3.hpp
+++ b/mcgaze_amd/csrc/wino_x3.hpp
@@ -17,6 +17,9 @@
   int total_pairs, n_tiles;
   int tpf, gpf;
   float wscale;
+  const int* blk_list;
+  const int* blk_count;
+  int bxn, bpf;
 };
 
 template <int NB, int RH, int RT, int CT, int G>
@@ -299,34 +302,50 @@
 __device__ __forceinline__ void buf_load16(u32x4v& dst, uint32_t voffset, const u32x4& srd, uint32_t soffset_uniform) {
   asm volatile("buffer_load_dwordx4 %0, %1, %2, %3 offen offset:%4" : "=&v"(dst) : "v"(voffset), "s"(srd), "s"(soffset_uniform), "n"(IMM) : "memory");
 }
-template <int NB>
-__global__ __launch_bounds__(256, 1) void wino_x3w_kernel(const WinoParams p) {
+template <int NB, bool BLK>
+__device__ __forceinline__ void wino_x3w_tile(const WinoParams& p, const int logical) {
   using namespace wnx;
   constexpr int G = 2, NV = 4, NW = 4, RT = 4, CT = 4, MT = 128, NT = 128;
   constexpr int ROWB = NB * 1024, WIN_CAP = 48 * 1024, USTAGE = ustage(2);
   constexpr int MAXP = WIN_CAP / 1024 / NW;
   constexpr int HB = MAXP / 2;
+  constexpr int BWR = 10;
+  static_assert(!BLK || (NB == 1 && RT * BWR <= NW * MAXP), "block tile: one piece per window row, every block's rows in the window");
   extern __shared__ __attribute__((aligned(16))) char smem[];
   char* const s_win = smem;
   const int tid = threadIdx.x, lane = tid & 63;
   const int wave = __builtin_amdgcn_readfirstlane(tid >> 6);
   const int nu = wave;
-  const int logical = xcd_remap(blockIdx.x, gridDim.x);
   const int mt = logical / p.n_tiles, ntile = logical - mt * p.n_tiles;
-  int q0, q_end;
-  if (p.tpf > 0) {
-    const int f = mt / p.tpf, t = mt - f * p.tpf;
-    q0 = f * p.gpf + t * MT;
-    q_end = min(q0 + MT, (f + 1) * p.gpf);
+  int q0 = 0, q_end = 0;
+  int bf[RT], by0[RT], bxg[RT];
+  uint32_t bokm = 0;
+  if constexpr (BLK) {
+    const int cnt = __builtin_amdgcn_readfirstlane(*p.blk_count);
+#pragma unroll
+    for (int rt = 0; rt < RT; ++rt) {
+      const int e = RT * mt + rt;
+      if (e < cnt) bokm |= 1u << rt;
+      const int id = __builtin_amdgcn_readfirstlane(p.blk_list[e < cnt ? e : RT * mt]);
+      const int f = id / p.bpf, r = id - f * p.bpf, by = r / p.bxn;
+      bf[rt] = f; by0[rt] = 8 * by; bxg[rt] = 4 * (r - by * p.bxn);
+    }
   } else {
-    q0 = mt * MT;
-    q_end = min(q0 + MT, p.total_pairs);
-  }
+    if (p.tpf > 0) {
+      const int f = mt / p.tpf, t = mt - f * p.tpf;
+      q0 = f * p.gpf + t * MT;
+      q_end = min(q0 + MT, (f + 1) * p.gpf);
+    } else {
+      q0 = mt * MT;
+      q_end = min(q0 + MT, p.total_pairs);
+    }
+  }
+  auto pick = [&](const int (&a)[RT], int i) { return i == 0 ? a[0] : (i == 1 ? a[1] : (i == 2 ? a[2] : a[3])); };
   const int q_last = q_end - 1;
   const int H1 = p.H + 1;
   auto slot_of = [&](int q) { const int R = q / p.PW; return R + R / p.H + 1; };
-  const int sig_b = __builtin_amdgcn_readfirstlane(slot_of(q0) - 1);
-  const int NP = __builtin_amdgcn_readfirstlane((slot_of(q_last) - sig_b + 2) * NB);
+  const int sig_b = BLK ? 0 : __builtin_amdgcn_readfirstlane(slot_of(q0) - 1);
+  const int NP = BLK ? RT * BWR : __builtin_amdgcn_readfirstlane((slot_of(q_last) - sig_b + 2) * NB);
   const int NSL = p.Cin / KS, KT = 3 * NSL;
   const int n0 = ntile * NT;
   const u32x4 srd_x = make_srd(p.x);
@@ -334,30 +353,54 @@
   const uint32_t lds_win = (uint32_t)(uintptr_t)(__attribute__((address_space(3))) char*)s_win;
 
   uint32_t prow[MAXP];
+  int pxo[MAXP];
   uint32_t pokm = 0, prowokm = 0;
   static_for<MAXP>([&](auto nc) {
     constexpr int n = decltype(nc)::value;
-    const int pi = wave + NW * n, j = pi / NB;
-    const int sg = sig_b + j, f = sg / H1, r = sg - f * H1;
-    if (pi < NP) pokm |= 1u << n;
-    if (r != 0 && f < p.frames) prowokm |= 1u << n;
-    prow[n] = __builtin_amdgcn_readfirstlane((uint32_t)(((long long)(f * p.H + r - 1) * p.W) * p.Cin * 4));
+    const int pi = wave + NW * n;
+    if constexpr (BLK) {
+      const int rb = min(pi / BWR, RT - 1), y = pick(by0, rb) + pi - BWR * rb - 1, f = pick(bf, rb);
+      const bool rowok = y >= 0 && y < p.H;
+      if (pi < NP && ((bokm >> rb) & 1)) pokm |= 1u << n;
+      if (rowok) prowokm |= 1u << n;
+      prow[n] = __builtin_amdgcn_readfirstlane((uint32_t)(((long long)(f * p.H + (rowok ? y : 0)) * p.W) * p.Cin * 4));
+      pxo[n] = __builtin_amdgcn_readfirstlane(2 * pick(bxg, rb));
+    } else {
+      const int j = pi / NB;
+      const int sg = sig_b + j, f = sg / H1, r = sg - f * H1;
+      if (pi < NP) pokm |= 1u << n;
+      if (r != 0 && f < p.frames) prowokm |= 1u << n;
+      prow[n] = __builtin_amdgcn_readfirstlane((uint32_t)(((long long)(f * p.H + r - 1) * p.W) * p.Cin * 4));
+      pxo[n] = 0;
+    }
   });
   pokm = __builtin_amdgcn_readfirstlane(pokm);
   prowokm = __builtin_amdgcn_readfirstlane(prowokm);
   uint32_t w_voff;
+  int l_x;
   {
     const int l_ph = lane >> 5, l_i = (lane >> 2) & 7, l_cs = lane & 3, b = wave & (NB - 1);
     const int x = (8 * b + l_i) * G + l_ph - 1;
     const int c = l_cs ^ ((2 * b + (l_i >> 2)) & 3);
-    w_voff = (unsigned)x < (unsigned)p.W ? (uint32_t)((x * p.Cin + 4 * c) * 4) : MCG_OOB_OFFSET;
-  }
+    l_x = x;
+    w_voff = BLK ? (uint32_t)(4 * c * 4) : ((unsigned)x < (unsigned)p.W ? (uint32_t)((x * p.Cin + 4 * c) * 4) : MCG_OOB_OFFSET);
+  }
+  auto piece_voff = [&](auto nc) -> uint32_t {
+    constexpr int n = decltype(nc)::value;
+    if (!(prowokm & (1u << n))) return MCG_OOB_OFFSET;
+    if constexpr (BLK) {
+      const int x = pxo[n] + l_x;
+      return (unsigned)x < (unsigned)p.W ? (uint32_t)(x * p.Cin * 4) + w_voff : MCG_OOB_OFFSET;
+    } else {
+      return w_voff;
+    }
+  };
   auto issue_window = [&](auto hc, int cs, uint32_t dst) {
     constexpr int h0 = decltype(hc)::value * HB;
     static_for<HB>([&](auto nc) {
       constexpr int n = h0 + decltype(nc)::value;
       if (pokm & (1u << n)) {
-        const uint32_t v = (prowokm & (1u << n)) ? w_voff : MCG_OOB_OFFSET;
+        const uint32_t v = piece_voff(std::integral_constant<int, n>{});
         lds_dma16<0>(v, srd_x, prow[n] + (uint32_t)cs * (KS * 4), dst + (uint32_t)(wave + NW * n) * 1024u);
       }
     });
@@ -376,9 +419,16 @@
   const char* ap[RT][2][2];
 #pragma unroll
   for (int rt = 0; rt < RT; ++rt) {
-    const int q = min(q0 + rt * 32 + pl, q_last);
-    const int R = q / p.PW, xg = q - R * p.PW;
-    const int jrow = (R + R / p.H + 1) - sig_b - 1;
+    int jrow, xg;
+    if constexpr (BLK) {
+      jrow = BWR * rt + (pl >> 2);
+      xg = pl & 3;
+    } else {
+      const int q = min(q0 + rt * 32 + pl, q_last);
+      const int R = q / p.PW;
+      xg = q - R * p.PW;
+      jrow = (R + R / p.H + 1) - sig_b - 1;
+    }
 #pragma unroll
     for (int t = 0; t < 2; ++t) {
       const int wx = G * xg + (t == 0 ? toff0 : toff1);
@@ -459,7 +509,7 @@
           constexpr int n = (KY == 0 ? HB : 0) + (V - 8);
           const int csn = KY == 0 ? cs + 1 : cs + 2;
           if (csn < NSL && (pokm & (1u << n))) {
-            const uint32_t v = (prowokm & (1u << n)) ? w_voff : MCG_OOB_OFFSET;
+            const uint32_t v = piece_voff(std::integral_constant<int, n>{});
             lds_dma16<0>(v, srd_x, prow[n] + (uint32_t)csn * (KS * 4), lds_win + (KY == 0 ? (WB ^ 1) : WB) * WIN_CAP + (uint32_t)(wave + NW * n) * 1024u);
           }
         }
@@ -527,8 +577,18 @@
     __syncthreads();
     for (int item = tid; item < PP * CPR; item += 256) {
       const int prl = item / CPR, ch4 = (item - prl * CPR) * 4;
-      const int q = q0 + pass * PP + prl;
-      if (q >= q_end) continue;
+      int R, xo;
+      if constexpr (BLK) {
+        const int rt = 2 * pass + (prl >> 5), pl = prl & 31;
+        const int y = pick(by0, rt) + (pl >> 2);
+        xo = G * (pick(bxg, rt) + (pl & 3));
+        if (!((bokm >> rt) & 1) || y >= p.H || xo >= p.W) continue;
+        R = pick(bf, rt) * p.H + y;
+      } else {
+        const int q = q0 + pass * PP + prl;
+        if (q >= q_end) continue;
+        R = q / p.PW; xo = G * (q - R * p.PW);
+      }
       float4 bv = make_float4(0.f, 0.f, 0.f, 0.f);
       if (p.bias) bv = *(const float4*)(p.bias + n0 + ch4);
       float4 m[NV];
@@ -537,7 +597,6 @@
       float4 y[2];
       y[0] = make_float4(((m[0].x + m[1].x) + m[2].x) * wsc + bv.x, ((m[0].y + m[1].y) + m[2].y) * wsc + bv.y, ((m[0].z + m[1].z) + m[2].z) * wsc + bv.z, ((m[0].w + m[1].w) + m[2].w) * wsc + bv.w);
       y[1] = make_float4(((m[1].x - m[2].x) - m[3].x) * wsc + bv.x, ((m[1].y - m[2].y) - m[3].y) * wsc + bv.y, ((m[1].z - m[2].z) - m[3].z) * wsc + bv.z, ((m[1].w - m[2].w) - m[3].w) * wsc + bv.w);
-      const int R = q / p.PW, xo = G * (q - R * p.PW);
       float* yp = p.y + ((long long)R * p.W + xo) * p.Cout + n0 + ch4;
 #pragma unroll
       for (int j = 0; j < 2; ++j) {
@@ -548,6 +607,19 @@
       }
     }
     __syncthreads();
+  }
+}
+template <int NB>
+__global__ __launch_bounds__(256, 1) void wino_x3w_kernel(const WinoParams p) {
+  wino_x3w_tile<NB, false>(p, xcd_remap(blockIdx.x, gridDim.x));
+}
+__global__ __launch_bounds__(256, 1) void wino_x3w_blocks_kernel(const WinoParams p) {
+  const int units = __builtin_amdgcn_readfirstlane(((*p.blk_count + 3) >> 2) * p.n_tiles);
+  const int padded = p.n_tiles == 2 ? (units + 15) & ~15 : units;
+  for (int u = blockIdx.x; u < padded; u += gridDim.x) {
+    int logical = u;
+    if (p.n_tiles == 2) { const int x = u & 7, j = u >> 3; logical = (j & 1) + 2 * (x + 8 * (j >> 1)); }
+    if (logical < units) wino_x3w_tile<1, true>(p, logical);
   }
 }
 
@@ -612,6 +684,35 @@
   if (shape == 1) return launch_wino_x3_t<NB, 2, 1, 2, 2>(s, p, grid);
   return launch_wino_x3_t<NB, 1, 1, 2, 2>(s, p, grid);
 }
+static inline bool wino_x3_blocks_applicable(int frames, int H, int W, int Cin, int Cout) {
+  const long long px = (long long)frames * H * W;
+  return Cin % 32 == 0 && Cout % wnx::UNT == 0 && H >= 1 && W >= 2 && frames >= 1 && px * Cin * 4 < MCG_DMA_MAX_BYTES &&
+         px * Cout * 4 < MCG_DMA_MAX_BYTES && px < 0x7fffffffLL;
+}
+static inline int wino_x3_blocks_per_frame(int H, int W) { return ((H + 7) / 8) * ((W + 7) / 8); }
+static inline int launch_wino_x3_blocks(hipStream_t s, WinoParams p, const int* list, const int* count, int max_blocks) {
+  constexpr int kLds = 4 * 64 * 128 * 4;
+  static bool raised[MCG_MAX_DEVICES] = {false};
+  static int cus[MCG_MAX_DEVICES] = {0};
+  int dev = 0;
+  if (hipGetDevice(&dev) != hipSuccess || dev < 0 || dev >= MCG_MAX_DEVICES) dev = 0;
+  if (!raised[dev]) {
+    if (hipFuncSetAttribute((const void*)wino_x3w_blocks_kernel, hipFuncAttributeMaxDynamicSharedMemorySize, kLds) != hipSuccess) return 1;
+    int n = 0;
+    if (hipDeviceGetAttribute(&n, hipDeviceAttributeMultiprocessorCount, dev) != hipSuccess || n <= 0) n = 256;
+    cus[dev] = n;
+    raised[dev] = true;
+  }
+  p.PW = (p.W + 1) / 2;
+  p.n_tiles = p.Cout / 128;
+  p.bxn = (p.W + 7) / 8;
+  p.bpf = wino_x3_blocks_per_frame(p.H, p.W);
+  p.blk_list = list; p.blk_count = count;
+  const int units = (max_blocks + 3) / 4 * p.n_tiles;
+  const int grid = units < cus[dev] ? units : cus[dev] / 16 * 16;
+  hipLaunchKernelGGL(wino_x3w_blocks_kernel, dim3(grid > 0 ? grid : 1), dim3(256), kLds, s, p);
+  return hipGetLastError() == hipSuccess ? 0 : 1;
+}
 static const int kWinoMinGrid = 130;
 static inline int launch_wino_x3(hipStream_t s, WinoParams p, int shape = -1, int g = 2) {
   const int mode = wino_x3_mode(p.frames, p.H, p.W, p.Cin, p.Cout, g);
diff --git a/mcgaze_amd/engine.py b/mcgaze_amd/engine.py
--- a/mcgaze_amd/engine.py
+++ b/mcgaze_amd/engine.py
@@ -444,8 +444,7 @@
         self.e, self.N, self.H, self.W, self.T, self.chunk = engine, num_frames, H, W, clip_length, chunk_frames
         dev, lib, h = engine.device, engine.lib, engine._handle
         self.sa, self.sb = pipeline_streams(dev, decoder_priority)
-        self.pyr = [[torch.empty(num_frames, (H // 4) >> i, (W // 4) >> i, 256, dtype=engine.dtype, device=dev) for i in range(4)] for _ in range(2)]
-        self.tabs = [(C.c_void_p * 4)(*[p.data_ptr() for p in lvl]) for lvl in self.pyr]
+        self.slots = [_ws(lib.mcg_deferred_pyramid_bytes(h, num_frames, H, W), dev) for _ in range(2)]
         self.trunk_ws = _ws(lib.mcg_trunk_workspace_bytes(h, num_frames, H, W, chunk_frames), dev)
         self.dec_ws = _ws(lib.mcg_decoder_workspace_bytes(h, num_frames), dev)
         self.trunk_done = [torch.cuda.Event() for _ in range(2)]
@@ -469,13 +468,14 @@
         self.sa.wait_stream(cur)
         if self.used[slot]:
             self.sa.wait_event(self.dec_done[slot])
-        L.check(lib.mcg_backbone_fpn_forward(e._handle, C.c_void_p(self.sa.cuda_stream), _ptr(img), self.N, self.H, self.W, self.chunk,
-                                             self.tabs[slot], _ptr(self.trunk_ws), self.trunk_ws.numel()), 'mcg_backbone_fpn_forward')
+        L.check(lib.mcg_backbone_fpn_forward_deferred(e._handle, C.c_void_p(self.sa.cuda_stream), _ptr(img), self.N, self.H, self.W, self.chunk,
+                                                      _ptr(self.slots[slot]), self.slots[slot].numel(), _ptr(self.trunk_ws), self.trunk_ws.numel()),
+                'mcg_backbone_fpn_forward_deferred')
         self.trunk_done[slot].record(self.sa)
         self.sb.wait_event(self.trunk_done[slot])
-        L.check(lib.mcg_decoder_forward(e._handle, C.c_void_p(self.sb.cuda_stream), self.tabs[slot], self.N, self.T, self.H, self.W,
-                                        _ptr(img_hw), _ptr(out['gaze']), _ptr(out['boxes']), _ptr(out['scores']),
-                                        _ptr(self.dec_ws), self.dec_ws.numel()), 'mcg_decoder_forward')
+        L.check(lib.mcg_decoder_forward_deferred(e._handle, C.c_void_p(self.sb.cuda_stream), _ptr(self.slots[slot]), self.slots[slot].numel(),
+                                                 self.N, self.T, self.H, self.W, _ptr(img_hw), _ptr(out['gaze']), _ptr(out['boxes']),
+                                                 _ptr(out['scores']), _ptr(self.dec_ws), self.dec_ws.numel()), 'mcg_decoder_forward_deferred')
         self.dec_done[slot].record(self.sb)
         self.used[slot] = True
         self.k += 1
diff --git a/mcgaze_amd/lib.py b/mcgaze_amd/lib.py
--- a/mcgaze_amd/lib.py
+++ b/mcgaze_amd/lib.py
@@ -6,7 +6,7 @@
 
 MCG_OK = 0
 MCG_F32, MCG_BF16, MCG_F16X3, MCG_F16 = 0, 1, 2, 3
-ABI_VERSION = 14
+ABI_VERSION = 15
 RES_NONE, RES_ADD, RES_UPSAMPLE_ADD = 0, 1, 2
 FLAG_STAGED_GEMM, FLAG_NO_SPECIALISED, FLAG_NO_ATTN_BLOCK = 1, 2, 4
 
@@ -24,7 +24,8 @@
            'mcg_engine_workspace_bytes', 'mcg_trunk_workspace_bytes', 'mcg_decoder_workspace_bytes', 'mcg_backbone_fpn_forward',
            'mcg_decoder_forward', 'mcg_clip_forward', 'mcg_preprocess_frames', 'mcg_engine_set_option', 'mcg_engine_profile_start',
            'mcg_engine_profile_stop', 'mcg_bench_backbone_forward', 'mcg_bottleneck_x3', 'mcg_bench_backbone_levels', 'mcg_conv3x3_wino_x3',
-           'mcg_conv3x3_wino_x3_weight_bytes', 'mcg_engine_range_audit', 'mcg_roi_align_indexed', 'mcg_decoder_forward_indexed']
+           'mcg_conv3x3_wino_x3_weight_bytes', 'mcg_engine_range_audit', 'mcg_roi_align_indexed', 'mcg_decoder_forward_indexed',
+           'mcg_deferred_pyramid_bytes', 'mcg_deferred_pyramid_levels', 'mcg_backbone_fpn_forward_deferred', 'mcg_decoder_forward_deferred']
 
 
 class ConvDesc(C.Structure):
@@ -103,6 +104,11 @@
     lib.mcg_decoder_forward.argtypes = [vp, vp, C.POINTER(vp), i, i, i, i, vp, vp, vp, vp, vp, sz]
     lib.mcg_decoder_forward_indexed.argtypes = [vp, vp, C.POINTER(vp), i, vp, i, i, i, i, vp, vp, vp, vp, vp, sz]
     lib.mcg_backbone_fpn_forward.argtypes = [vp, vp, vp, i, i, i, i, C.POINTER(vp), vp, sz]
+    lib.mcg_deferred_pyramid_bytes.restype = sz
+    lib.mcg_deferred_pyramid_bytes.argtypes = [vp, i, i, i]
+    lib.mcg_deferred_pyramid_levels.argtypes = [vp, vp, i, i, i, C.POINTER(vp), C.POINTER(i)]
+    lib.mcg_backbone_fpn_forward_deferred.argtypes = [vp, vp, vp, i, i, i, i, vp, sz, vp, sz]
+    lib.mcg_decoder_forward_deferred.argtypes = [vp, vp, vp, sz, i, i, i, i, vp, vp, vp, vp, vp, sz]
     lib.mcg_clip_forward.argtypes = [vp, vp, vp, i, i, i, i, vp, i, vp, vp, vp, vp, sz]
     lib.mcg_preprocess_frames.argtypes = [vp, vp, i, vp, i, i, C.POINTER(C.c_float), C.POINTER(C.c_float), i]
     lib.mcg_engine_set_option.argtypes = [vp, C.c_char_p, i]
```

Result: faster. 3606 clips/s (median of 6 runs) (+8.5%).
